# mycrazycracy/speaker-embedding-with-phonetic-information

Measured on AMD Instinct MI355X. Metric: utterance-embeddings/sec (400-frame chunks), higher is better.
Workload: dtype fp16mx; 1 GPU; v2_xvector TDNN, 256 chunks x 400 frames per GPU per step, utterance-sharded, weights broadcast once over RCCL; topology=v2_xvector, batch_chunks_per_gpu=256, frames_per_chunk=400, precision=default, arithmetic=fp16mx, lanes=2, output_node=embedding, chunk_lengths=400, library=xvec_hip 0.4 (gfx950; kernels 1123b5fc04a88fd3)

## Files before the change

### include/xvec_hip.h

```cpp
#ifndef XVEC_HIP_H_
#define XVEC_HIP_H_

#include <stddef.h>
#include <stdint.h>

#ifdef __cplusplus
extern "C" {
#endif

typedef enum {
  XV_OK = 0,
  XV_ERR_IO = 1,
  XV_ERR_MODEL = 2,
  XV_ERR_DEVICE = 3,
  XV_ERR_ARG = 4,
  XV_ERR_INTERNAL = 5
} xv_status;

typedef enum {
  XV_PREC_DEFAULT = -1,
  XV_PREC_BF16X3 = 0,
  XV_PREC_BF16 = 1,
  XV_PREC_FP16 = 2,
  XV_PREC_FP16X3 = 3,
// ... 118 lines not shown
  float sample_frequency, frame_length_ms, frame_shift_ms, dither, preemphasis_coefficient, blackman_coeff;
  int32_t remove_dc_offset, window_type, round_to_power_of_two, snip_edges;
  int32_t num_mel_bins;
  float low_freq, high_freq;
  int32_t num_ceps;
  float cepstral_lifter;
  int32_t use_energy, raw_energy;
  float energy_floor;
} xv_mfcc_options;
typedef struct {
  float vad_energy_threshold, vad_energy_mean_scale, vad_proportion_threshold;
  int32_t vad_frames_context;
} xv_vad_options;
void xv_mfcc_options_default(xv_mfcc_options* opts);
int64_t xv_mfcc_num_frames(const xv_mfcc_options* opts, int64_t n_samples);
uint64_t xv_mfcc_utt_seed(const char* key);
xv_status xv_mfcc_compute(int device, const xv_mfcc_options* opts, const float* samples, const int64_t* sample_offsets,
                          int32_t n_utts, const uint64_t* utt_seeds, float* out, int32_t* out_row_offsets);
xv_status xv_mfcc_compute_i16(int device, const xv_mfcc_options* opts, const int16_t* samples, const int64_t* sample_offsets,
                              int32_t n_utts, const uint64_t* utt_seeds, float* out, int32_t* out_row_offsets);
xv_status xv_mfcc_kernel_time(int device, const xv_mfcc_options* opts, const int16_t* samples, const int64_t* sample_offsets,
                              int32_t n_utts, int32_t reps, float* kernel_ms);
xv_status xv_vad_energy(int device, const xv_vad_options* vad_opts, const float* feats, const int32_t* row_offsets,
                        int32_t n_utts, int32_t dim, float* out);
xv_status xv_wave_read(const char* rxfilename, int32_t channel, int32_t* rate, int16_t** samples, int64_t* n);
void xv_wave_free(int16_t* samples);

typedef struct {
  int32_t shift_output, normalize_output;
  float duration, volume;
  int32_t input_wave_channel, rir_channel, noise_channel;
} xv_reverb_options;
void xv_reverb_options_default(xv_reverb_options* opts);
int64_t xv_reverb_output_length(const xv_reverb_options* opts, float sample_rate, int64_t n_samples, int64_t rir_len);
xv_status xv_wav_reverberate(int device, const xv_reverb_options* opts, float sample_rate, const void* samples,
                             int32_t samples_are_i16, const int64_t* sample_offsets, int32_t n_utts, const float* rirs,
                             const int64_t* rir_offsets, int32_t n_rirs, const int32_t* utt_rir, const float* noises,
                             const int64_t* noise_offsets, int32_t n_noises, const int32_t* utt_add_offsets,
                             const int32_t* add_noise, const float* add_snr, const float* add_start, int64_t* out_offsets,
                             float* out_f32, int16_t* out_i16, int64_t* clipped);
xv_status xv_reverb_kernel_time(int device, const xv_reverb_options* opts, float sample_rate, const void* samples,
                                int32_t samples_are_i16, const int64_t* sample_offsets, int32_t n_utts, const float* rirs,
                                const int64_t* rir_offsets, int32_t n_rirs, const int32_t* utt_rir, const float* noises,
                                const int64_t* noise_offsets, int32_t n_noises, const int32_t* utt_add_offsets,
                                const int32_t* add_noise, const float* add_snr, const float* add_start, int32_t reps,
                                float* kernel_ms);
xv_status xv_recognize_wav_pipeline(const char* rxfilename, int32_t* found, char* description, size_t description_cap);
xv_status xv_wave_write(const char* wxfilename, int32_t rate, const float* samples, int64_t n, int64_t* clipped);

typedef struct {
  const void* hi;
  const void* lo;
  int32_t ld;
  int32_t row_shift;
  int32_t k_len;
  const void* gmax;
  const void* lo4; const void* lo4_scale;
} xv_seg_desc;
typedef struct {
  int32_t precision, epilogue;
  int32_t nseg;
  xv_seg_desc seg[8];
  const void* w_hi; const void* w_lo; int32_t ldw;
  int32_t rows;
  int32_t n_pad;
  const float* bias; const float* scale; const float* offset;
  int32_t relu, bn;
  void* out_hi; void* out_lo; int32_t ldo;
  float* out_f32; int32_t ldf; int32_t m_valid;
  float* partial; int32_t ldp; const int8_t* grp_range;
  void* hip_stream;
  const void* w4; int32_t ldw4; const void* w4_scale;
  void* gmax_out;
  const void* w4b; int32_t ldw4b; const void* w4b_scale;
  void* out_lo4; void* out_lo4_scale;
  int32_t p8;
  const int8_t* out_range;
  int32_t ksplit;
} xv_gemm_desc;
xv_status xv_pack_mx_residual(const float* w, const uint16_t* w_hi_f16, int32_t n_pad, int32_t nseg,
                              const int32_t* seg_src, const int32_t* seg_shift, const int32_t* seg_klen, uint8_t* w4,
                              uint8_t* w4_scale);
xv_status xv_pack_mx_residual64(const float* w, const uint16_t* w_hi_f16, int32_t n_pad, int32_t nseg, const int32_t* seg_src,
                                const int32_t* seg_shift, const int32_t* seg_klen, uint8_t* w4, uint8_t* w4_scale);
xv_status xv_pack_mx_weights(const float* w, int32_t n_pad, int32_t nseg, const int32_t* seg_src, const int32_t* seg_shift,
                             const int32_t* seg_klen, uint8_t* w4b, uint8_t* w4b_scale);
xv_status xv_pack_mx_weights64(const float* w, int32_t n_pad, int32_t nseg, const int32_t* seg_src, const int32_t* seg_shift,
                               const int32_t* seg_klen, uint8_t* w4b, uint8_t* w4b_scale);
xv_status xv_tile_mx_scales(const uint8_t* natural, int32_t n_pad, int32_t k_len, int32_t epilogue, uint8_t* tiled);
xv_status xv_kernel_tdnn_gemm(const xv_gemm_desc* d);

xv_status xv_compressed_size(int32_t rows, int32_t cols, int32_t method, size_t* nbytes, const char** format);
xv_status xv_compress_matrices(int device, const float* feats, const int32_t* row_off, int32_t n, int32_t cols, int32_t method,
                               uint8_t* out_bytes, int64_t* out_off, int32_t* nonfinite_flags);
xv_status xv_compress_kernel_time(int device, const float* feats, const int32_t* row_off, int32_t n, int32_t cols, int32_t method,
                                  int32_t reps, float* kernel_ms);
xv_status xv_cmvn_sliding(int device, const float* raw, const int32_t* raw_off, int32_t n, int32_t cols, int32_t cmn_window,
                          int32_t min_cmn_window, int32_t center, float* out);

xv_status xv_cmvn_stats(int device, const float* feats, const int32_t* row_off, int32_t n_utts, int32_t cols, double* stats,
                        float* device_ms);
xv_status xv_cmvn_norm(const double* stats, int32_t cols, int32_t norm_means, int32_t norm_vars, int32_t reverse,
                       const int32_t* skip_dims, int32_t n_skip, float* norm, int32_t* num_floored);
xv_status xv_cmvn_apply(int device, const float* feats, const int32_t* row_off, int32_t n_utts, int32_t cols, const float* norms,
                        const int32_t* utt_norm, float* out);
xv_status xv_cmvn_kernel_time(int device, const float* feats, const int32_t* row_off, int32_t n_utts, int32_t cols, int32_t reps,
                              float* stats_ms, float* apply_ms);

typedef struct {
  const float* feats;
  const int32_t* row_offsets;
  const int32_t* dev_off;
  int32_t B;
  int32_t rows;
  int32_t pad_left, pad_right;
  int32_t dim, noff;
  int32_t off[8];
  const void* w_hi; const void* w_lo;
  int32_t ldw, seg_pad;
  int32_t n_pad;
  int32_t epi_prec;
  const float* bias; const float* scale; const float* offset;
  int32_t relu, bn;
  void* out_hi; void* out_lo; int32_t ldo;
  void* out_lo4; void* out_lo4_scale;
  void* gmax_out; const int8_t* out_range;
  int32_t row0, nrows;
  int32_t max_wgs;
  void* hip_stream;
} xv_first_layer_desc;
xv_status xv_kernel_first_layer(const xv_first_layer_desc* d);
typedef struct {
  int32_t precision;
  const float* feats; const int32_t* src_off; const int32_t* dev_off; const int32_t* grp_utt;
  int32_t rows;
  int32_t dim, ld;
  void* out_hi; void* out_lo;
  int32_t pad_left, pad_right;
  void* zero_words; int32_t n_zero_words;
  void* hip_stream;
} xv_prep_input_desc;
xv_status xv_kernel_prep_input(const xv_prep_input_desc* d);
typedef struct {
  int32_t precision;
  const float* partial; int32_t ldp;
  const int32_t* utt_grp0; const int32_t* utt_grp1; const int32_t* utt_count;
  int32_t B, dim;
  float var_floor;
  void* out_hi; void* out_lo; int32_t ld;
  void* hip_stream;
} xv_pool_finalise_desc;
xv_status xv_kernel_pool_finalise(const xv_pool_finalise_desc* d);
typedef struct {
  const float* src; const void* src16; int32_t ld;
  const int32_t* out_row; int32_t n_out;
  int32_t dim, log_softmax;
  float* out; int32_t out_ld;
  void* hip_stream;
} xv_frame_output_desc;
xv_status xv_kernel_frame_output(const xv_frame_output_desc* d);

#ifdef __cplusplus
}
#endif
#endif
```

### speaker-embedding-with-phonetic-information_amd/__init__.py

```python
import ctypes
import os
import subprocess
import sys

_HERE = os.path.dirname(os.path.abspath(__file__))
CSRC = os.path.join(_HERE, "csrc")
LIB_PATH = os.environ.get("XVEC_LIB") or os.path.join(_HERE, "libxvec_hip.so")
BIN_DIR = os.path.join(_HERE, "bin")

XV_OK = 0
XV_ERR_IO, XV_ERR_MODEL, XV_ERR_DEVICE, XV_ERR_ARG, XV_ERR_INTERNAL = 1, 2, 3, 4, 5
PREC_BF16X3, PREC_BF16, PREC_FP16, PREC_FP16X3, PREC_FP16X2, PREC_AUTO, PREC_FP16MX, PREC_FP16MX2, PREC_FP16X3E = range(9)
PREC_DEFAULT = -1
PRECISIONS = {"default": PREC_DEFAULT, "bf16x3": PREC_BF16X3, "bf16": PREC_BF16, "fp16": PREC_FP16, "fp16x3": PREC_FP16X3,
              "fp16x2": PREC_FP16X2, "auto": PREC_AUTO, "fp16mx": PREC_FP16MX, "fp16mx2": PREC_FP16MX2}
PRECISION_NAMES = {v: k for k, v in PRECISIONS.items()}
MFMA_PASSES = {"bf16x3": 3, "bf16": 1, "fp16": 1, "fp16x3": 3, "fp16x2": 2, "fp16mx": 1.25}
EPI_ACT, EPI_F32, EPI_STATS = 0, 1, 2


class XvError(RuntimeError):
    def __init__(self, status, msg):
        super().__init__("xvec_hip status %d: %s" % (status, msg))
        self.status = status


class ModelInfo(ctypes.Structure):
    _fields_ = [(n, ctypes.c_int32) for n in ("input_dim", "output_dim", "left_context", "right_context",
                                              "min_frames", "num_layers", "output_is_segment", "reserved")]


class SegDesc(ctypes.Structure):
    _fields_ = [("hi", ctypes.c_void_p), ("lo", ctypes.c_void_p), ("ld", ctypes.c_int32),
                ("row_shift", ctypes.c_int32), ("k_len", ctypes.c_int32), ("gmax", ctypes.c_void_p),
                ("lo4", ctypes.c_void_p), ("lo4_scale", ctypes.c_void_p)]


class GemmDesc(ctypes.Structure):
    _fields_ = [("precision", ctypes.c_int32), ("epilogue", ctypes.c_int32), ("nseg", ctypes.c_int32),
                ("seg", SegDesc * 8),
                ("w_hi", ctypes.c_void_p), ("w_lo", ctypes.c_void_p), ("ldw", ctypes.c_int32),
                ("rows", ctypes.c_int32), ("n_pad", ctypes.c_int32),
                ("bias", ctypes.c_void_p), ("scale", ctypes.c_void_p), ("offset", ctypes.c_void_p),
                ("relu", ctypes.c_int32), ("bn", ctypes.c_int32),
                ("out_hi", ctypes.c_void_p), ("out_lo", ctypes.c_void_p), ("ldo", ctypes.c_int32),
                ("out_f32", ctypes.c_void_p), ("ldf", ctypes.c_int32), ("m_valid", ctypes.c_int32),
                ("partial", ctypes.c_void_p), ("ldp", ctypes.c_int32), ("grp_range", ctypes.c_void_p),
                ("hip_stream", ctypes.c_void_p),
                ("w4", ctypes.c_void_p), ("ldw4", ctypes.c_int32), ("w4_scale", ctypes.c_void_p),
                ("gmax_out", ctypes.c_void_p),
                ("w4b", ctypes.c_void_p), ("ldw4b", ctypes.c_int32), ("w4b_scale", ctypes.c_void_p),
                ("out_lo4", ctypes.c_void_p), ("out_lo4_scale", ctypes.c_void_p),
                ("p8", ctypes.c_int32),
                ("out_range", ctypes.c_void_p), ("ksplit", ctypes.c_int32)]


class FirstLayerDesc(ctypes.Structure):
    _fields_ = [("feats", ctypes.c_void_p), ("row_offsets", ctypes.c_void_p), ("dev_off", ctypes.c_void_p), ("B", ctypes.c_int32),
                ("rows", ctypes.c_int32), ("pad_left", ctypes.c_int32), ("pad_right", ctypes.c_int32),
                ("dim", ctypes.c_int32), ("noff", ctypes.c_int32), ("off", ctypes.c_int32 * 8),
                ("w_hi", ctypes.c_void_p), ("w_lo", ctypes.c_void_p), ("ldw", ctypes.c_int32), ("seg_pad", ctypes.c_int32),
                ("n_pad", ctypes.c_int32), ("epi_prec", ctypes.c_int32),
                ("bias", ctypes.c_void_p), ("scale", ctypes.c_void_p), ("offset", ctypes.c_void_p),
                ("relu", ctypes.c_int32), ("bn", ctypes.c_int32),
                ("out_hi", ctypes.c_void_p), ("out_lo", ctypes.c_void_p), ("ldo", ctypes.c_int32),
                ("out_lo4", ctypes.c_void_p), ("out_lo4_scale", ctypes.c_void_p),
                ("gmax_out", ctypes.c_void_p), ("out_range", ctypes.c_void_p),
                ("row0", ctypes.c_int32), ("nrows", ctypes.c_int32), ("max_wgs", ctypes.c_int32),
                ("hip_stream", ctypes.c_void_p)]


class PrepInputDesc(ctypes.Structure):
    _fields_ = [("precision", ctypes.c_int32), ("feats", ctypes.c_void_p), ("src_off", ctypes.c_void_p), ("dev_off", ctypes.c_void_p),
                ("grp_utt", ctypes.c_void_p), ("rows", ctypes.c_int32), ("dim", ctypes.c_int32), ("ld", ctypes.c_int32),
                ("out_hi", ctypes.c_void_p), ("out_lo", ctypes.c_void_p), ("pad_left", ctypes.c_int32), ("pad_right", ctypes.c_int32),
                ("zero_words", ctypes.c_void_p), ("n_zero_words", ctypes.c_int32), ("hip_stream", ctypes.c_void_p)]


class PoolFinaliseDesc(ctypes.Structure):
    _fields_ = [("precision", ctypes.c_int32), ("partial", ctypes.c_void_p), ("ldp", ctypes.c_int32),
                ("utt_grp0", ctypes.c_void_p), ("utt_grp1", ctypes.c_void_p), ("utt_count", ctypes.c_void_p),
                ("B", ctypes.c_int32), ("dim", ctypes.c_int32), ("var_floor", ctypes.c_float),
                ("out_hi", ctypes.c_void_p), ("out_lo", ctypes.c_void_p), ("ld", ctypes.c_int32), ("hip_stream", ctypes.c_void_p)]


class FrameOutputDesc(ctypes.Structure):
    _fields_ = [("src", ctypes.c_void_p), ("src16", ctypes.c_void_p), ("ld", ctypes.c_int32),
                ("out_row", ctypes.c_void_p), ("n_out", ctypes.c_int32), ("dim", ctypes.c_int32), ("log_softmax", ctypes.c_int32),
                ("out", ctypes.c_void_p), ("out_ld", ctypes.c_int32), ("hip_stream", ctypes.c_void_p)]


class Calibration(ctypes.Structure):
    _fields_ = [("chosen", ctypes.c_int32), ("checked", ctypes.c_int32), ("err_mx", ctypes.c_float), ("err_mx2", ctypes.c_float),
                ("checked_mx", ctypes.c_int32), ("err_lite", ctypes.c_float), ("lite_mask", ctypes.c_uint64),
                ("err_holdout", ctypes.c_float), ("checked_holdout", ctypes.c_int32), ("lite_dropped", ctypes.c_int32),
                ("tail", ctypes.c_float)]

    def as_dict(self):
        d = {"chosen": PRECISION_NAMES.get(self.chosen, str(self.chosen)), "checked": self.checked, "checked_mx": self.checked_mx,
             "err_mx": self.err_mx, "err_mx2": self.err_mx2, "tail": self.tail}
        if self.lite_mask:
            d["lite_mask"] = int(self.lite_mask)
            d["err_lite"] = self.err_lite
            d["err_holdout"] = self.err_holdout
            d["checked_holdout"] = self.checked_holdout
        if self.lite_dropped:
            d["lite_dropped"] = self.lite_dropped
        return d


ABI_SYMBOLS = [
    "xv_last_error", "xv_version", "xv_model_load", "xv_model_load_rxfilename", "xv_model_free", "xv_model_info",
    "xv_model_macs", "xv_model_describe", "xv_model_pack", "xv_ctx_create", "xv_ctx_create_from_blob",
    "xv_ctx_create_from_device_blob", "xv_ctx_free",
    "xv_ctx_info", "xv_forward_batch", "xv_forward_batch_device", "xv_ctx_synchronize", "xv_ctx_set_profiling",
    "xv_ctx_profile_report", "xv_extract_utterances", "xv_ctx_calibrate", "xv_ctx_set_fast_mode", "xv_ctx_fast_mode",
    "xv_calibrate_table", "xv_ctx_set_calibration", "xv_ctx_model_fingerprint", "xv_ctx_share_calibration",
    "xv_ctx_set_calibration_file", "xv_calibration_file_read", "xv_calibration_file_publish", "xv_recognize_feature_pipeline", "xv_ctx_set_lite_layers", "xv_ctx_lite_layers",
    "xv_extract_table", "xv_frontend_cmvn_select", "xv_plan_chunks", "xv_ctx_create_broadcast", "xv_kernel_tdnn_gemm",
    "xv_backend_apply", "xv_segment_mean", "xv_scatter_stats", "xv_plda_transform", "xv_plda_score", "xv_lda_estimate",
    "xv_plda_estimate", "xv_plda_adapt",
    "xv_mfcc_options_default", "xv_mfcc_num_frames", "xv_mfcc_utt_seed", "xv_mfcc_compute", "xv_mfcc_compute_i16", "xv_mfcc_kernel_time", "xv_vad_energy",
    "xv_reverb_options_default", "xv_reverb_output_length", "xv_wav_reverberate", "xv_reverb_kernel_time", "xv_wave_write", "xv_recognize_wav_pipeline",
    "xv_compressed_size", "xv_compress_matrices", "xv_compress_kernel_time", "xv_cmvn_sliding",
    "xv_cmvn_stats", "xv_cmvn_norm", "xv_cmvn_apply", "xv_cmvn_kernel_time",
    "xv_kernel_first_layer", "xv_kernel_prep_input", "xv_kernel_pool_finalise", "xv_kernel_frame_output",
    "xv_wave_read", "xv_wave_free", "xv_pack_mx_residual", "xv_pack_mx_residual64", "xv_tile_mx_scales", "xv_pack_mx_weights", "xv_pack_mx_weights64",
]

_lib = None


def build(verbose=False):
    cmd = ["make", "-C", CSRC, "-j8"]
    res = subprocess.run(cmd, stdout=subprocess.PIPE, stderr=subprocess.STDOUT, text=True)
    if verbose or res.returncode != 0:
        print(res.stdout)
    if res.returncode != 0:
        raise RuntimeError("building libxvec_hip.so failed")
    return LIB_PATH


def lib():
    global _lib
    if _lib is not None:
        return _lib
    if not os.path.exists(LIB_PATH):
        raise ImportError("%s is missing - run `python -c 'import __graft_entry__ as g; g.build()'` "
                          "(there is no Python/CPU fallback for the HIP path)" % LIB_PATH)
    if os.environ.get("XVEC_NO_TORCH_PRELOAD", "") != "1":
        try:
            import torch
        except Exception:
            pass
    L = ctypes.CDLL(LIB_PATH)
    L.xv_last_error.restype = ctypes.c_char_p
    L.xv_version.restype = ctypes.c_char_p
    L.xv_model_macs.restype = ctypes.c_double
    L.xv_model_macs.argtypes = [ctypes.c_void_p, ctypes.c_int32]
    L.xv_model_describe.restype = ctypes.c_size_t
    L.xv_model_describe.argtypes = [ctypes.c_void_p, ctypes.c_char_p, ctypes.c_size_t]
    L.xv_model_load.argtypes = [ctypes.c_void_p, ctypes.c_size_t, ctypes.c_char_p, ctypes.c_char_p,
                                ctypes.POINTER(ctypes.c_void_p)]
    L.xv_model_load_rxfilename.argtypes = [ctypes.c_char_p, ctypes.c_char_p, ctypes.c_char_p,
                                           ctypes.POINTER(ctypes.c_void_p)]
    L.xv_model_free.argtypes = [ctypes.c_void_p]
    L.xv_model_free.restype = None
    L.xv_model_info.argtypes = [ctypes.c_void_p, ctypes.POINTER(ModelInfo)]
    L.xv_model_pack.argtypes = [ctypes.c_void_p, ctypes.c_int, ctypes.c_void_p, ctypes.POINTER(ctypes.c_size_t)]
    L.xv_ctx_create.argtypes = [ctypes.c_void_p, ctypes.c_int, ctypes.c_int, ctypes.POINTER(ctypes.c_void_p)]
    L.xv_ctx_create_from_blob.argtypes = [ctypes.c_void_p, ctypes.c_size_t, ctypes.c_int,
                                          ctypes.POINTER(ctypes.c_void_p)]
    L.xv_ctx_create_from_device_blob.argtypes = [ctypes.c_void_p, ctypes.c_size_t, ctypes.c_int,
                                                 ctypes.POINTER(ctypes.c_void_p)]
    L.xv_pack_mx_residual.argtypes = [ctypes.c_void_p, ctypes.c_void_p, ctypes.c_int32, ctypes.c_int32, ctypes.c_void_p,
                                      ctypes.c_void_p, ctypes.c_void_p, ctypes.c_void_p, ctypes.c_void_p]
    L.xv_pack_mx_residual64.argtypes = L.xv_pack_mx_residual.argtypes
    L.xv_pack_mx_weights.argtypes = [ctypes.c_void_p, ctypes.c_int32, ctypes.c_int32, ctypes.c_void_p, ctypes.c_void_p,
                                     ctypes.c_void_p, ctypes.c_void_p, ctypes.c_void_p]
    L.xv_pack_mx_weights64.argtypes = L.xv_pack_mx_weights.argtypes
    L.xv_tile_mx_scales.argtypes = [ctypes.c_void_p, ctypes.c_int32, ctypes.c_int32, ctypes.c_int32, ctypes.c_void_p]
    L.xv_ctx_free.argtypes = [ctypes.c_void_p]
    L.xv_ctx_free.restype = None
    L.xv_ctx_info.argtypes = [ctypes.c_void_p, ctypes.POINTER(ModelInfo), ctypes.POINTER(ctypes.c_int32),
                              ctypes.POINTER(ctypes.c_int32)]
    L.xv_forward_batch.argtypes = [ctypes.c_void_p, ctypes.c_void_p, ctypes.c_void_p, ctypes.c_int32, ctypes.c_void_p]
    L.xv_forward_batch_device.argtypes = [ctypes.c_void_p, ctypes.c_void_p, ctypes.c_void_p, ctypes.c_int32,
                                          ctypes.c_void_p, ctypes.c_int32, ctypes.c_void_p]
    L.xv_ctx_synchronize.argtypes = [ctypes.c_void_p]
    L.xv_ctx_set_profiling.argtypes = [ctypes.c_void_p, ctypes.c_int32]
    L.xv_ctx_profile_report.argtypes = [ctypes.c_void_p, ctypes.c_char_p, ctypes.c_size_t]
    L.xv_ctx_profile_report.restype = ctypes.c_size_t
    L.xv_extract_utterances.argtypes = [ctypes.c_void_p, ctypes.c_void_p, ctypes.c_void_p, ctypes.c_int32,
                                        ctypes.c_int32, ctypes.c_int32, ctypes.c_int32, ctypes.c_void_p, ctypes.c_void_p]
    L.xv_ctx_create_broadcast.argtypes = [ctypes.c_void_p, ctypes.POINTER(ctypes.c_int), ctypes.c_int, ctypes.c_int,
                                          ctypes.POINTER(ctypes.c_void_p)]
    L.xv_kernel_tdnn_gemm.argtypes = [ctypes.POINTER(GemmDesc)]
    L.xv_kernel_first_layer.argtypes = [ctypes.POINTER(FirstLayerDesc)]
    L.xv_kernel_prep_input.argtypes = [ctypes.POINTER(PrepInputDesc)]
    L.xv_kernel_pool_finalise.argtypes = [ctypes.POINTER(PoolFinaliseDesc)]
    L.xv_kernel_frame_output.argtypes = [ctypes.POINTER(FrameOutputDesc)]
    L.xv_ctx_calibrate.argtypes = [ctypes.c_void_p, ctypes.c_void_p, ctypes.c_void_p, ctypes.c_int32, ctypes.c_float,
                                   ctypes.POINTER(Calibration)]
    L.xv_ctx_set_fast_mode.argtypes = [ctypes.c_void_p, ctypes.c_int32]
    L.xv_ctx_fast_mode.argtypes = [ctypes.c_void_p, ctypes.POINTER(ctypes.c_int32)]
    L.xv_ctx_set_lite_layers.argtypes = [ctypes.c_void_p, ctypes.c_uint64]
    L.xv_ctx_lite_layers.argtypes = [ctypes.c_void_p, ctypes.POINTER(ctypes.c_uint64)]
    L.xv_calibrate_table.argtypes = [ctypes.c_void_p, ctypes.c_char_p, ctypes.c_int32, ctypes.c_int32, ctypes.c_int32,
                                     ctypes.c_int32, ctypes.c_float, ctypes.POINTER(Calibration)]
    L.xv_ctx_set_calibration.argtypes = [ctypes.c_void_p, ctypes.c_int32, ctypes.c_float]
    L.xv_ctx_model_fingerprint.argtypes = [ctypes.c_void_p, ctypes.POINTER(ctypes.c_uint64)]
    L.xv_ctx_share_calibration.argtypes = [ctypes.c_void_p, ctypes.c_char_p, ctypes.c_float, ctypes.c_char_p,
                                           ctypes.POINTER(ctypes.c_int32)]
    L.xv_ctx_set_calibration_file.argtypes = [ctypes.c_void_p, ctypes.c_char_p]
    L.xv_calibration_file_read.argtypes = [ctypes.c_char_p, ctypes.POINTER(ctypes.c_int32), ctypes.POINTER(ctypes.c_uint64),
                                           ctypes.POINTER(ctypes.c_int32), ctypes.POINTER(ctypes.c_uint64)]
    L.xv_calibration_file_publish.argtypes = [ctypes.c_char_p, ctypes.c_uint64, ctypes.c_int32, ctypes.c_uint64, ctypes.c_float,
                                              ctypes.c_char_p, ctypes.POINTER(ctypes.c_int32), ctypes.POINTER(ctypes.c_uint64),
                                              ctypes.POINTER(ctypes.c_int32), ctypes.POINTER(ctypes.c_uint64)]
    _lib = L
    return L


def _check(status):
    if status != XV_OK:
        raise XvError(status, lib().xv_last_error().decode(errors="replace"))


class Model:

    def __init__(self, raw=None, rxfilename=None, nnet_config=None, output_node=None):
        L = lib()
        self._h = ctypes.c_void_p()
        cfg = nnet_config.encode() if nnet_config else None
        node = output_node.encode() if output_node else None
        if raw is not None:
            buf = ctypes.create_string_buffer(bytes(raw), len(raw))
            _check(L.xv_model_load(buf, len(raw), cfg, node, ctypes.byref(self._h)))
        else:
            _check(L.xv_model_load_rxfilename(rxfilename.encode(), cfg, node, ctypes.byref(self._h)))

    def __del__(self):
        if getattr(self, "_h", None) and self._h.value and lib is not None:
            lib().xv_model_free(self._h)
            self._h = ctypes.c_void_p()

    @property
    def info(self):
        mi = ModelInfo()
        _check(lib().xv_model_info(self._h, ctypes.byref(mi)))
        return mi

    def macs(self, frames):
        return lib().xv_model_macs(self._h, int(frames))

    def describe(self):
        n = lib().xv_model_describe(self._h, None, 0)
        buf = ctypes.create_string_buffer(n)
        lib().xv_model_describe(self._h, buf, n)
        return buf.value.decode()

    def pack(self, precision=PREC_DEFAULT):
        n = ctypes.c_size_t(0)
        _check(lib().xv_model_pack(self._h, precision, None, ctypes.byref(n)))
        buf = ctypes.create_string_buffer(n.value)
        _check(lib().xv_model_pack(self._h, precision, buf, ctypes.byref(n)))
        return buf.raw[:n.value]


class Context:

    def __init__(self, model=None, blob=None, device=0, precision=PREC_DEFAULT, device_blob=None):
        L = lib()
        self._h = ctypes.c_void_p()
        if device_blob is not None:
            _check(L.xv_ctx_create_from_device_blob(ctypes.c_void_p(int(device_blob[0])), int(device_blob[1]), device,
                                                    ctypes.byref(self._h)))
        elif blob is not None:
            self._blob = ctypes.create_string_buffer(bytes(blob), len(blob))
            _check(L.xv_ctx_create_from_blob(self._blob, len(blob), device, ctypes.byref(self._h)))
        else:
            _check(L.xv_ctx_create(model._h, device, precision, ctypes.byref(self._h)))
        mi = ModelInfo()
        p, d = ctypes.c_int32(), ctypes.c_int32()
        _check(L.xv_ctx_info(self._h, ctypes.byref(mi), ctypes.byref(p), ctypes.byref(d)))
        self.info, self.precision, self.device = mi, p.value, d.value

    def close(self):
        if getattr(self, "_h", None) and self._h.value and lib is not None:
            lib().xv_ctx_free(self._h)
            self._h = ctypes.c_void_p()

    def __del__(self):
        self.close()

    def forward_batch(self, feats, row_offsets):
        import numpy as np
        feats = np.ascontiguousarray(feats, dtype=np.float32)
        offs = np.ascontiguousarray(row_offsets, dtype=np.int32)
        B = len(offs) - 1
        n_out = B if self.info.output_is_segment else int(offs[-1] - offs[0])
        out = np.empty((n_out, self.info.output_dim), dtype=np.float32)
        _check(lib().xv_forward_batch(self._h, feats.ctypes.data, offs.ctypes.data, B, out.ctypes.data))
        return out

    def forward_batch_device(self, feats_ptr, row_offsets, out_ptr, out_ld, stream=None):
        import numpy as np
        offs = np.ascontiguousarray(row_offsets, dtype=np.int32)
        _check(lib().xv_forward_batch_device(self._h, feats_ptr, offs.ctypes.data, len(offs) - 1, out_ptr, out_ld,
                                             stream))

    def synchronize(self):
        _check(lib().xv_ctx_synchronize(self._h))

    def set_profiling(self, on):
        _check(lib().xv_ctx_set_profiling(self._h, 1 if on else 0))

    def profile_report(self):
        buf = ctypes.create_string_buffer(1 << 18)
        lib().xv_ctx_profile_report(self._h, buf, len(buf))
        rows = []
        for line in buf.value.decode().splitlines():
            label, calls, ms = line.split("\t")
            rows.append((label, int(calls), float(ms)))
        return rows

    def frontend(self, raw, raw_offsets, vad=None, cmn_window=300, center=True):
        import numpy as np
        raw = np.ascontiguousarray(raw, dtype=np.float32)
        offs = np.ascontiguousarray(raw_offsets, dtype=np.int32)
        n = len(offs) - 1
        out = np.empty_like(raw)
        out_off = np.zeros(n + 1, dtype=np.int32)
        v = None if vad is None else np.ascontiguousarray(vad, dtype=np.float32)
        L = lib()
        L.xv_frontend_cmvn_select.argtypes = [ctypes.c_void_p, ctypes.c_void_p, ctypes.c_void_p, ctypes.c_int32, ctypes.c_void_p,
                                              ctypes.c_int32, ctypes.c_int32, ctypes.c_void_p, ctypes.c_void_p]
        _check(L.xv_frontend_cmvn_select(self._h, raw.ctypes.data, offs.ctypes.data, n, None if v is None else v.ctypes.data,
                                         cmn_window, 1 if center else 0, out.ctypes.data, out_off.ctypes.data))
        return out[:out_off[-1]], out_off

    def extract_table(self, feature_rspecifier, vector_wspecifier, chunk_size=-1, min_chunk_size=100, pad_input=True,
                      batch_frames=0):
        L = lib()
        L.xv_extract_table.argtypes = [ctypes.c_void_p, ctypes.c_char_p, ctypes.c_char_p, ctypes.c_int32, ctypes.c_int32,
                                       ctypes.c_int32, ctypes.c_int32, ctypes.POINTER(ctypes.c_int64),
                                       ctypes.POINTER(ctypes.c_int64)]
        done, failed = ctypes.c_int64(0), ctypes.c_int64(0)
        _check(L.xv_extract_table(self._h, feature_rspecifier.encode(), vector_wspecifier.encode(), chunk_size,
                                  min_chunk_size, 1 if pad_input else 0, batch_frames, ctypes.byref(done),
                                  ctypes.byref(failed)))
        return done.value, failed.value

    def calibrate(self, feats, row_offsets, tol=7.5e-5):
# ... 538 lines not shown
              rir_flat.ctypes.data, rir_off.ctypes.data, len(rir_list), utt_rir.ctypes.data,
              noise_flat.ctypes.data, noise_off.ctypes.data, len(noise_list), add_off.ctypes.data if additive is not None else None,
              add_noise.ctypes.data, add_snr.ctypes.data, add_start.ctypes.data)
    if kernel_time_reps > 0:
        L.xv_reverb_kernel_time.argtypes = _REVERB_ARGTYPES + [ctypes.c_int32, ctypes.POINTER(ctypes.c_float)]
        ms = ctypes.c_float(0)
        _check(L.xv_reverb_kernel_time(*common, int(kernel_time_reps), ctypes.byref(ms)))
        return ms.value
    out = np.empty(total, dtype=np.float32)
    out16 = np.empty(total, dtype=np.int16) if return_int16 else None
    clipped = np.zeros(max(1, n), dtype=np.int64)
    out_off = np.zeros(n + 1, dtype=np.int64)
    L.xv_wav_reverberate.argtypes = _REVERB_ARGTYPES + [ctypes.c_void_p, ctypes.c_void_p, ctypes.c_void_p, ctypes.c_void_p]
    _check(L.xv_wav_reverberate(*common, out_off.ctypes.data, out.ctypes.data, out16.ctypes.data if return_int16 else None,
                                clipped.ctypes.data))
    assert list(np.diff(out_off)) == [max(0, x) for x in lens]
    if return_int16:
        return [(out[out_off[u]:out_off[u + 1]].copy(), out16[out_off[u]:out_off[u + 1]].copy(), int(clipped[u])) for u in range(n)]
    return [out[out_off[u]:out_off[u + 1]].copy() for u in range(n)]


def _pack_matrices(mats, what):
    import numpy as np
    ms = [np.ascontiguousarray(m, dtype=np.float32) for m in mats]
    if any(m.ndim != 2 for m in ms):
        raise XvError(XV_ERR_ARG, "%s: every matrix must be two-dimensional" % what)
    widths = {m.shape[1] for m in ms if m.shape[0] > 0}
    if len(widths) > 1:
        raise XvError(XV_ERR_ARG, "%s: the matrices of one call share their column count" % what)
    cols = widths.pop() if widths else 0
    off = np.zeros(len(ms) + 1, dtype=np.int32)
    off[1:] = np.cumsum([m.shape[0] if cols else 0 for m in ms])
    rows = [m for m in ms if m.shape[0] > 0 and cols]
    packed = np.concatenate(rows, axis=0) if rows else np.zeros((0, max(cols, 1)), np.float32)
    return np.ascontiguousarray(packed), off, cols


def compressed_size(rows, cols, method=1):
    L = lib()
    n, fmt = ctypes.c_size_t(0), ctypes.c_char_p()
    L.xv_compressed_size.argtypes = [ctypes.c_int32, ctypes.c_int32, ctypes.c_int32, ctypes.POINTER(ctypes.c_size_t),
                                     ctypes.POINTER(ctypes.c_char_p)]
    _check(L.xv_compressed_size(rows, cols, method, ctypes.byref(n), ctypes.byref(fmt)))
    return int(n.value), fmt.value.decode()


def compress(mats, method=1, device=0, return_flags=False, kernel_time_reps=0):
    import numpy as np
    L = lib()
    packed, off, cols = _pack_matrices(mats, "compress")
    n = len(off) - 1
    common = [device, packed.ctypes.data if packed.size else None, off.ctypes.data, n, cols, method]
    types = [ctypes.c_int, ctypes.c_void_p, ctypes.c_void_p, ctypes.c_int32, ctypes.c_int32, ctypes.c_int32]
    if kernel_time_reps > 0:
        ms = ctypes.c_float(0)
        L.xv_compress_kernel_time.argtypes = types + [ctypes.c_int32, ctypes.POINTER(ctypes.c_float)]
        _check(L.xv_compress_kernel_time(*common, int(kernel_time_reps), ctypes.byref(ms)))
        return ms.value
    total = sum(compressed_size(int(off[u + 1] - off[u]), cols, method)[0] for u in range(n))
    out = np.zeros(max(1, total), dtype=np.uint8)
    out_off = np.zeros(n + 1, dtype=np.int64)
    flags = np.zeros(max(1, n), dtype=np.int32)
    L.xv_compress_matrices.argtypes = types + [ctypes.c_void_p, ctypes.c_void_p, ctypes.c_void_p]
    _check(L.xv_compress_matrices(*common, out.ctypes.data, out_off.ctypes.data, flags.ctypes.data))
    assert int(out_off[n]) == total
    objs = [out[out_off[u]:out_off[u + 1]].tobytes() for u in range(n)]
    return (objs, [bool(f) for f in flags[:n]]) if return_flags else objs


def cmvn_sliding(mats, cmn_window=600, min_cmn_window=100, center=False, device=0):
    import numpy as np
    L = lib()
    packed, off, cols = _pack_matrices(mats, "cmvn_sliding")
    n = len(off) - 1
    out = np.empty_like(packed)
    L.xv_cmvn_sliding.argtypes = [ctypes.c_int, ctypes.c_void_p, ctypes.c_void_p, ctypes.c_int32, ctypes.c_int32, ctypes.c_int32,
                                  ctypes.c_int32, ctypes.c_int32, ctypes.c_void_p]
    _check(L.xv_cmvn_sliding(device, packed.ctypes.data if packed.size else None, off.ctypes.data, n, max(cols, 1), cmn_window,
                             min_cmn_window, 1 if center else 0, out.ctypes.data if out.size else None))
    return [out[off[u]:off[u + 1]].copy() for u in range(n)]


def cmvn_stats(feats_list, device=0, kernel_time_reps=0):
    import numpy as np
    L = lib()
    packed, off, cols = _pack_matrices(feats_list, "cmvn_stats")
    n = len(off) - 1
    if cols < 1:
        raise XvError(XV_ERR_ARG, "cmvn_stats: no matrix with rows and columns")
    if kernel_time_reps > 0:
        a, b = ctypes.c_float(0), ctypes.c_float(0)
        L.xv_cmvn_kernel_time.argtypes = [ctypes.c_int, ctypes.c_void_p, ctypes.c_void_p, ctypes.c_int32, ctypes.c_int32, ctypes.c_int32,
                                          ctypes.POINTER(ctypes.c_float), ctypes.POINTER(ctypes.c_float)]
        _check(L.xv_cmvn_kernel_time(device, packed.ctypes.data, off.ctypes.data, n, cols, int(kernel_time_reps), ctypes.byref(a),
                                     ctypes.byref(b)))
        return a.value, b.value
    stats = np.zeros((n, 2, cols + 1), dtype=np.float64)
    L.xv_cmvn_stats.argtypes = [ctypes.c_int, ctypes.c_void_p, ctypes.c_void_p, ctypes.c_int32, ctypes.c_int32, ctypes.c_void_p,
                                ctypes.c_void_p]
    _check(L.xv_cmvn_stats(device, packed.ctypes.data if packed.size else None, off.ctypes.data, n, cols, stats.ctypes.data, None))
    return stats


def cmvn_norm(stats, norm_means=True, norm_vars=False, reverse=False, skip_dims=(), return_floored=False):
    import numpy as np
    L = lib()
    st = np.ascontiguousarray(stats, dtype=np.float64)
    if st.ndim != 2 or st.shape[0] != 2 or st.shape[1] < 2:
        raise XvError(XV_ERR_ARG, "cmvn_norm: the statistics are a [2][cols + 1] matrix")
    cols = st.shape[1] - 1
    skip = np.ascontiguousarray(list(skip_dims), dtype=np.int32)
    norm = np.zeros((2, cols), dtype=np.float32)
    floored = ctypes.c_int32(0)
    L.xv_cmvn_norm.argtypes = [ctypes.c_void_p, ctypes.c_int32, ctypes.c_int32, ctypes.c_int32, ctypes.c_int32, ctypes.c_void_p,
                               ctypes.c_int32, ctypes.c_void_p, ctypes.POINTER(ctypes.c_int32)]
    _check(L.xv_cmvn_norm(st.ctypes.data, cols, int(bool(norm_means)), int(bool(norm_vars)), int(bool(reverse)),
                          skip.ctypes.data if skip.size else None, int(skip.size), norm.ctypes.data, ctypes.byref(floored)))
    return (norm, int(floored.value)) if return_floored else norm


def apply_cmvn(feats_list, norms, utt_norm, device=0):
    import numpy as np
    L = lib()
    packed, off, cols = _pack_matrices(feats_list, "apply_cmvn")
    n = len(off) - 1
    nm = np.ascontiguousarray(norms, dtype=np.float32)
    un = np.ascontiguousarray(utt_norm, dtype=np.int32)
    if un.shape != (n,) or nm.ndim != 3 or nm.shape[1:] != (2, max(cols, 1)) or (n and (un.min() < 0 or un.max() >= nm.shape[0])):
        raise XvError(XV_ERR_ARG, "apply_cmvn: norms are [n_norms][2][cols] and utt_norm names one of them per matrix")
    out = np.empty_like(packed)
    L.xv_cmvn_apply.argtypes = [ctypes.c_int, ctypes.c_void_p, ctypes.c_void_p, ctypes.c_int32, ctypes.c_int32, ctypes.c_void_p,
                                ctypes.c_void_p, ctypes.c_void_p]
    _check(L.xv_cmvn_apply(device, packed.ctypes.data if packed.size else None, off.ctypes.data, n, max(cols, 1), nm.ctypes.data,
                           un.ctypes.data, out.ctypes.data if out.size else None))
    return [out[off[u]:off[u + 1]].copy() for u in range(n)]


def kernel_tdnn_gemm(desc):
    _check(lib().xv_kernel_tdnn_gemm(ctypes.byref(desc)))


def kernel_first_layer(desc):
    _check(lib().xv_kernel_first_layer(ctypes.byref(desc)))


def kernel_prep_input(desc):
    _check(lib().xv_kernel_prep_input(ctypes.byref(desc)))


def kernel_pool_finalise(desc):
    _check(lib().xv_kernel_pool_finalise(ctypes.byref(desc)))


def kernel_frame_output(desc):
    _check(lib().xv_kernel_frame_output(ctypes.byref(desc)))


def pack_mx_residual(w, w_hi_f16, segs, walk64=False):
    import numpy as np
    w = np.ascontiguousarray(w, dtype=np.float32)
    hi = np.ascontiguousarray(w_hi_f16, dtype=np.uint16)
    n_pad, K = w.shape
    src = np.array([s[0] for s in segs], dtype=np.int32)
    shift = np.array([s[1] for s in segs], dtype=np.int32)
    klen = np.array([s[2] for s in segs], dtype=np.int32)
    assert int(klen.sum()) == K and K % 128 == 0
    w4 = np.zeros((n_pad, K // 128 * 64), dtype=np.uint8)
    sc = np.zeros((n_pad, K // 32), dtype=np.uint8)
    fn = lib().xv_pack_mx_residual64 if walk64 else lib().xv_pack_mx_residual
    _check(fn(w.ctypes.data, hi.ctypes.data, n_pad, len(segs), src.ctypes.data, shift.ctypes.data,
              klen.ctypes.data, w4.ctypes.data, sc.ctypes.data))
    return w4, sc


def pack_mx_weights(w, segs, walk64=False):
    import numpy as np
    w = np.ascontiguousarray(w, dtype=np.float32)
    n_pad, K = w.shape
    src = np.array([s[0] for s in segs], dtype=np.int32)
    shift = np.array([s[1] for s in segs], dtype=np.int32)
    klen = np.array([s[2] for s in segs], dtype=np.int32)
    assert int(klen.sum()) == K and np.all(klen % (256 if walk64 else 128) == 0)
    w4b = np.zeros((n_pad, 2 * K if walk64 else K // 2), dtype=np.uint8)
    sc = np.zeros((n_pad, K // 32), dtype=np.uint8)
    fn = lib().xv_pack_mx_weights64 if walk64 else lib().xv_pack_mx_weights
    _check(fn(w.ctypes.data, n_pad, len(segs), src.ctypes.data, shift.ctypes.data, klen.ctypes.data, w4b.ctypes.data, sc.ctypes.data))
    return w4b, sc


def tile_mx_scales(scales, epilogue):
    import numpy as np
    sc = np.ascontiguousarray(scales, dtype=np.uint8)
    out = np.zeros(sc.size, dtype=np.uint8)
    _check(lib().xv_tile_mx_scales(sc.ctypes.data, sc.shape[0], sc.shape[1] * 32, int(epilogue), out.ctypes.data))
    return out
```

### speaker-embedding-with-phonetic-information_amd/csrc/capi.cc

```cpp
#include <dlfcn.h>
#include <stdlib.h>
#include <string.h>

#include <algorithm>
#include <memory>
#include <string>
#include <vector>

#include "../../include/xvec_hip.h"
#include "backend.h"
#include "cmvn.h"
#include "compress.h"
#include "engine.h"
#include "extractor.h"
#include "feat.h"
#include "reverb.h"
#include "wave.h"
#include "kernels.h"
#include "calib_file.h"
#include "fuse_pipe.h"
#include "fuse_wav.h"
#include "multi_gpu.h"
#include "nnet3_raw.h"
#include "plda.h"
// ... 1066 lines not shown
    if (p) (void)hipFree(p);
  }
  hipError_t Alloc(size_t n) { return hipMalloc(&p, n ? n : 1); }
};
}

xv_status xv_kernel_first_layer(const xv_first_layer_desc* d) {
  if (!d) return Fail(XV_ERR_ARG, "xv_kernel_first_layer: null descriptor");
  return Guard([&] {
    const char* who = "xv_kernel_first_layer: ";
    if (!d->feats || !d->row_offsets || !d->dev_off || !d->w_hi || !d->w_lo || !d->bias || !d->out_hi || (d->bn && (!d->scale || !d->offset)))
      return Fail(XV_ERR_ARG, std::string(who) + "a required pointer is null");
    const int p = d->epi_prec;
    if (p != xv::kPrecBf16x3 && p != xv::kPrecFp16x3 && p != xv::kPrecFp16x2 && p != xv::kPrecFp16x3E)
      return Fail(XV_ERR_ARG, std::string(who) + "epi_prec must be XV_PREC_BF16X3, XV_PREC_FP16X3, XV_PREC_FP16X2 or XV_PREC_FP16X3E");
    if ((p == xv::kPrecBf16x3 || p == xv::kPrecFp16x3) && !d->out_lo) return Fail(XV_ERR_ARG, std::string(who) + "the split planes need out_lo");
    if (p == xv::kPrecFp16x3E && (!d->out_lo4 || !d->out_lo4_scale))
      return Fail(XV_ERR_ARG, std::string(who) + "XV_PREC_FP16X3E needs out_lo4 and out_lo4_scale");
    if (d->B < 1 || d->rows < xv::kFirstRows || d->rows % xv::kFirstRows || d->n_pad < xv::kBN || d->n_pad % xv::kBN ||
        d->ldo < d->n_pad || d->ldo % 64 || d->pad_left < 0 || d->pad_right < 0)
      return Fail(XV_ERR_ARG, std::string(who) + "bad geometry (rows: multiple of 64, n_pad: multiple of 128, ldo: multiple of 64, >= n_pad)");
    if (d->nrows < xv::kFirstRows || d->nrows % xv::kFirstRows || d->row0 < 0 || d->row0 % xv::kFirstRows || d->row0 + (long)d->nrows > d->rows)
      return Fail(XV_ERR_ARG, std::string(who) + "row0 and nrows must be multiples of 64 inside [0, rows]");
    if (d->dim < 1 || d->noff < 1 || d->noff > 8) return Fail(XV_ERR_ARG, std::string(who) + "dim >= 1 and 1 .. 8 offsets");
    int off[8];
    for (int j = 0; j < d->noff; ++j) {
      off[j] = d->off[j];
      if (off[j] < -15 || off[j] > 15) return Fail(XV_ERR_ARG, std::string(who) + "time offsets beyond +-15 frames");
    }
    if (!xv::FirstLayerApplicable(d->dim, d->noff, off))
      return Fail(XV_ERR_ARG, std::string(who) + "tdnn_first_kernel cannot run this shape (dim rounded up to 8 must be <= 24, noff x that <= 128, "
                                                 "and (64 + offset span) x that <= 2048)");
    if (d->seg_pad < d->dim || (long)(d->noff - 1) * d->seg_pad + d->dim > d->ldw)
      return Fail(XV_ERR_ARG, std::string(who) + "the weight planes do not hold noff segments of dim columns");
    const int ngrp = d->rows / xv::kRowAlign;
    std::vector<int32_t> grp_utt(ngrp, -1);
    long next_free = 0;
    if (d->row_offsets[0] < 0) return Fail(XV_ERR_ARG, std::string(who) + "negative row offset");
    for (int b = 0; b < d->B; ++b) {
      const long len = (long)d->row_offsets[b + 1] - d->row_offsets[b];
      const long span = (len + d->pad_left + d->pad_right + xv::kRowAlign - 1) / xv::kRowAlign * xv::kRowAlign;
      if (len < 1 || d->dev_off[b] % xv::kRowAlign || d->dev_off[b] < next_free || d->dev_off[b] + span > d->rows)
        return Fail(XV_ERR_ARG, std::string(who) + "chunk " + std::to_string(b) + ": empty, not on a 16-row boundary, overlapping or beyond rows");
      next_free = d->dev_off[b] + span;
      for (long g = d->dev_off[b] / xv::kRowAlign; g < next_free / xv::kRowAlign; ++g) grp_utt[g] = b;
    }
    std::vector<int32_t> grp_src((size_t)ngrp * 4);
    xv::FillFirstGroupSources(ngrp, grp_utt.data(), d->dev_off, d->row_offsets, d->pad_left, d->pad_right, grp_src.data());
    hipStream_t s = (hipStream_t)d->hip_stream;
    DevMem tab, wch, wcl;
    const size_t wc_bytes = (size_t)d->n_pad * xv::kFirstK * 2;
    hipError_t e = tab.Alloc(grp_src.size() * 4);
    if (e == hipSuccess) e = wch.Alloc(wc_bytes);
    if (e == hipSuccess) e = wcl.Alloc(wc_bytes);
    if (e == hipSuccess) e = hipMemcpy(tab.p, grp_src.data(), grp_src.size() * 4, hipMemcpyHostToDevice);
    if (e != hipSuccess) return Fail(XV_ERR_DEVICE, std::string("first_layer tables: ") + hipGetErrorString(e));
    xv::FirstArgs fa;
    memset(&fa, 0, sizeof fa);
    fa.g.n_tiles = d->n_pad / xv::kBN;
    fa.g.m_tiles = d->rows / xv::kBM;
    fa.g.relu = d->relu;
    fa.g.bn = d->bn;
    fa.g.bias = d->bias;
    fa.g.scale = d->scale;
    fa.g.offset = d->offset;
    fa.g.out_hi = (uint16_t*)d->out_hi;
    fa.g.out_lo = (uint16_t*)d->out_lo;
    fa.g.ldo = d->ldo;
    fa.g.out_lo4 = (uint8_t*)d->out_lo4;
    fa.g.out_lo4s = (uint8_t*)d->out_lo4_scale;
    fa.g.gmax_out = (unsigned*)d->gmax_out;
    fa.g.out_range = d->out_range;
    fa.feats = d->feats;
    fa.feats_valid_idx = (long)d->row_offsets[0] * d->dim;
    fa.grp_src = (const int4*)tab.p;
    fa.rows = d->rows;
    fa.dim = d->dim;
    fa.row0 = d->row0;
    fa.nrows = d->nrows;
    fa.noff = d->noff;
    for (int j = 0; j < d->noff; ++j) fa.off[j] = off[j];
    fa.wc_hi = (const uint16_t*)wch.p;
    fa.wc_lo = (const uint16_t*)wcl.p;
    fa.max_wgs = d->max_wgs > 0 ? d->max_wgs : 0;
    e = xv::launch_compact_first((const uint16_t*)d->w_hi, d->ldw, d->seg_pad, d->n_pad, d->noff, d->dim, (uint16_t*)wch.p, s);
    if (e == hipSuccess) e = xv::launch_compact_first((const uint16_t*)d->w_lo, d->ldw, d->seg_pad, d->n_pad, d->noff, d->dim, (uint16_t*)wcl.p, s);
    if (e == hipSuccess) e = xv::launch_tdnn_first(fa, p, s);
    const hipError_t e2 = hipStreamSynchronize(s);
    if (e != hipSuccess || e2 != hipSuccess)
      return Fail(XV_ERR_DEVICE, std::string("tdnn_first launch: ") + hipGetErrorString(e != hipSuccess ? e : e2));
    return XV_OK;
  });
}

xv_status xv_kernel_prep_input(const xv_prep_input_desc* d) {
  if (!d) return Fail(XV_ERR_ARG, "xv_kernel_prep_input: null descriptor");
  return Guard([&] {
    if (d->precision < xv::kPrecBf16x3 || d->precision > xv::kPrecFp16x3) return Fail(XV_ERR_ARG, "xv_kernel_prep_input: precision must be 0 .. 3");
    const bool split = xv::PrecXPlanes(d->precision) == 2;
    if (!d->feats || !d->src_off || !d->dev_off || !d->grp_utt || !d->out_hi || (split && !d->out_lo))
      return Fail(XV_ERR_ARG, "xv_kernel_prep_input: a required pointer is null");
    if (d->rows < xv::kBM || d->rows % xv::kBM || d->ld < xv::kBK || d->ld % xv::kBK || d->dim < 1 || d->dim > d->ld || d->pad_left < 0 ||
        d->pad_right < 0 || d->n_zero_words < 0 || (d->n_zero_words > 0 && !d->zero_words))
      return Fail(XV_ERR_ARG, "xv_kernel_prep_input: bad geometry (rows: multiple of 128, ld: multiple of 32, >= dim)");
    xv::PrepArgs a;
    memset(&a, 0, sizeof a);
    a.feats = d->feats;
    a.src_off = d->src_off;
    a.dev_off = d->dev_off;
    a.grp_utt = d->grp_utt;
    a.rows = d->rows;
    a.dim = d->dim;
    a.ld = d->ld;
    a.out_hi = (uint16_t*)d->out_hi;
    a.out_lo = (uint16_t*)d->out_lo;
    a.pad_left = d->pad_left;
    a.pad_right = d->pad_right;
    a.zero_words = (unsigned*)d->zero_words;
    a.n_zero_words = d->n_zero_words;
    const hipError_t e = xv::launch_prep_input(a, d->precision, (hipStream_t)d->hip_stream);
    if (e != hipSuccess) return Fail(XV_ERR_DEVICE, std::string("prep_input launch: ") + hipGetErrorString(e));
    return XV_OK;
  });
}

xv_status xv_kernel_pool_finalise(const xv_pool_finalise_desc* d) {
  if (!d) return Fail(XV_ERR_ARG, "xv_kernel_pool_finalise: null descriptor");
  return Guard([&] {
    if (d->precision < xv::kPrecBf16x3 || d->precision > xv::kPrecFp16x3) return Fail(XV_ERR_ARG, "xv_kernel_pool_finalise: precision must be 0 .. 3");
    const bool split = xv::PrecXPlanes(d->precision) == 2;
    if (!d->partial || !d->utt_grp0 || !d->utt_grp1 || !d->utt_count || !d->out_hi || (split && !d->out_lo))
      return Fail(XV_ERR_ARG, "xv_kernel_pool_finalise: a required pointer is null");
    if (d->B < 1 || d->dim < 1 || d->ldp < d->dim || d->ld < 2 * d->dim)
      return Fail(XV_ERR_ARG, "xv_kernel_pool_finalise: bad geometry (ldp >= dim, ld >= 2 dim)");
    xv::PoolArgs a;
    memset(&a, 0, sizeof a);
    a.partial = d->partial;
    a.ldp = d->ldp;
    a.utt_grp0 = d->utt_grp0;
    a.utt_grp1 = d->utt_grp1;
    a.utt_count = d->utt_count;
    a.B = d->B;
    a.dim = d->dim;
    a.var_floor = d->var_floor;
    a.out_hi = (uint16_t*)d->out_hi;
    a.out_lo = (uint16_t*)d->out_lo;
    a.ld = d->ld;
    const hipError_t e = xv::launch_pool_finalise(a, d->precision, (hipStream_t)d->hip_stream);
    if (e != hipSuccess) return Fail(XV_ERR_DEVICE, std::string("pool_finalise launch: ") + hipGetErrorString(e));
    return XV_OK;
  });
}

xv_status xv_kernel_frame_output(const xv_frame_output_desc* d) {
  if (!d) return Fail(XV_ERR_ARG, "xv_kernel_frame_output: null descriptor");
  return Guard([&] {
    if ((!d->src && !d->src16) || !d->out) return Fail(XV_ERR_ARG, "xv_kernel_frame_output: a required pointer is null");
    if (d->n_out < 1 || d->dim < 1 || d->ld < d->dim || d->out_ld < d->dim) return Fail(XV_ERR_ARG, "xv_kernel_frame_output: bad geometry");
    if (d->src16 && (!d->log_softmax || d->dim > 256 * 64))
      return Fail(XV_ERR_ARG, "xv_kernel_frame_output: fp16 logits are read by the log-softmax kernels only, rows of up to 16384 columns");
    xv::FrameOutArgs a;
    memset(&a, 0, sizeof a);
    a.src = d->src;
    a.src16 = (const uint16_t*)d->src16;
    a.ld = d->ld;
    a.out_row = d->out_row;
    a.n_out = d->n_out;
    a.dim = d->dim;
    a.log_softmax = d->log_softmax;
    a.out = d->out;
    a.out_ld = d->out_ld;
    const hipError_t e = xv::launch_frame_output(a, (hipStream_t)d->hip_stream);
    if (e != hipSuccess) return Fail(XV_ERR_DEVICE, std::string("frame_output launch: ") + hipGetErrorString(e));
    return XV_OK;
  });
}

static xv_status PackMxResidualImpl(bool walk64, const float* w, const uint16_t* w_hi_f16, int32_t n_pad, int32_t nseg,
                                    const int32_t* seg_src, const int32_t* seg_shift, const int32_t* seg_klen, uint8_t* w4,
                                    uint8_t* w4_scale) {
  if (!w || !w_hi_f16 || !seg_src || !seg_shift || !seg_klen || !w4 || !w4_scale || nseg < 1 || nseg > xv::kMaxSeg || n_pad < 1)
    return Fail(XV_ERR_ARG, "xv_pack_mx_residual: bad argument");
  return Guard([&] {
    long key[xv::kMaxSeg];
    int shift[xv::kMaxSeg], ksteps[xv::kMaxSeg], k_pad = 0;
    for (int j = 0; j < nseg; ++j) {
      if (seg_klen[j] % xv::kBK) return Fail(XV_ERR_ARG, "xv_pack_mx_residual: k_len must be a multiple of 32");
      key[j] = seg_src[j];
      shift[j] = seg_shift[j];
      ksteps[j] = seg_klen[j] / xv::kBK;
      k_pad += seg_klen[j];
    }
    xv::WalkGroup wg[xv::kMaxSeg];
    const int ng = xv::PlanWalkGroups(nseg, key, shift, ksteps, wg);
    std::vector<int> step_wcol(k_pad / xv::kBK);
    bool ok = false;
    if (walk64) xv::PlanWalkSteps64(ng, wg, step_wcol.data(), (int)step_wcol.size(), &ok);
    else xv::PlanWalkSteps(ng, wg, step_wcol.data(), (int)step_wcol.size(), &ok);
    if (!ok) return Fail(XV_ERR_ARG, "xv_pack_mx_residual: a K group is not a multiple of four steps");
    const int ldw4 = k_pad / xv::kBK / 4 * 64;
    std::vector<float> res(k_pad);
    for (int n = 0; n < n_pad; ++n) {
      for (int k = 0; k < k_pad; ++k) res[k] = w[(size_t)n * k_pad + k] - xv::host_f16_to_f32(w_hi_f16[(size_t)n * k_pad + k]);
      xv::PackMxRow(res.data(), k_pad, step_wcol.data(), w4 + (size_t)n * ldw4, w4_scale + (size_t)n * (k_pad / xv::kBK));
    }
    return XV_OK;
  });
}

xv_status xv_pack_mx_residual(const float* w, const uint16_t* w_hi_f16, int32_t n_pad, int32_t nseg, const int32_t* seg_src,
                              const int32_t* seg_shift, const int32_t* seg_klen, uint8_t* w4, uint8_t* w4_scale) {
  return PackMxResidualImpl(false, w, w_hi_f16, n_pad, nseg, seg_src, seg_shift, seg_klen, w4, w4_scale);
}

xv_status xv_pack_mx_residual64(const float* w, const uint16_t* w_hi_f16, int32_t n_pad, int32_t nseg, const int32_t* seg_src,
                                const int32_t* seg_shift, const int32_t* seg_klen, uint8_t* w4, uint8_t* w4_scale) {
  return PackMxResidualImpl(true, w, w_hi_f16, n_pad, nseg, seg_src, seg_shift, seg_klen, w4, w4_scale);
}

static xv_status PackMxWeightsImpl(bool walk64, const float* w, int32_t n_pad, int32_t nseg, const int32_t* seg_src,
                                   const int32_t* seg_shift, const int32_t* seg_klen, uint8_t* w4b, uint8_t* w4b_scale) {
  if (!w || !seg_src || !seg_shift || !seg_klen || !w4b || !w4b_scale || nseg < 1 || nseg > xv::kMaxSeg || n_pad < 1)
    return Fail(XV_ERR_ARG, "xv_pack_mx_weights: bad argument");
  return Guard([&] {
    long key[xv::kMaxSeg];
    int shift[xv::kMaxSeg], ksteps[xv::kMaxSeg], k_pad = 0;
    for (int j = 0; j < nseg; ++j) {
      if (seg_klen[j] % (walk64 ? 256 : 128)) return Fail(XV_ERR_ARG, "xv_pack_mx_weights: k_len must be a multiple of 128 (256 for the p8 order)");
      key[j] = seg_src[j];
      shift[j] = seg_shift[j];
      ksteps[j] = seg_klen[j] / xv::kBK;
      k_pad += seg_klen[j];
    }
    xv::WalkGroup wg[xv::kMaxSeg];
    const int ng = xv::PlanWalkGroups(nseg, key, shift, ksteps, wg);
    std::vector<int> lo_wcol(k_pad / 128);
    const int n_lo = walk64 ? xv::PlanWalkLoSteps64(ng, wg, lo_wcol.data(), (int)lo_wcol.size())
                            : xv::PlanWalkLoSteps(ng, wg, lo_wcol.data(), (int)lo_wcol.size());
    if (n_lo != (int)lo_wcol.size()) return Fail(XV_ERR_ARG, "xv_pack_mx_weights: inconsistent walk");
    const size_t pitch = walk64 ? (size_t)k_pad * 2 : (size_t)n_lo * 64;
    if (walk64) memset(w4b, 0, pitch * n_pad);
    for (int n = 0; n < n_pad; ++n)
      xv::PackMxWeightsRow(w + (size_t)n * k_pad, lo_wcol.data(), n_lo, w4b + (size_t)n * pitch, w4b_scale + (size_t)n * n_lo * 4);
    return XV_OK;
  });
}

xv_status xv_pack_mx_weights(const float* w, int32_t n_pad, int32_t nseg, const int32_t* seg_src, const int32_t* seg_shift,
                             const int32_t* seg_klen, uint8_t* w4b, uint8_t* w4b_scale) {
  return PackMxWeightsImpl(false, w, n_pad, nseg, seg_src, seg_shift, seg_klen, w4b, w4b_scale);
}

xv_status xv_pack_mx_weights64(const float* w, int32_t n_pad, int32_t nseg, const int32_t* seg_src, const int32_t* seg_shift,
                               const int32_t* seg_klen, uint8_t* w4b, uint8_t* w4b_scale) {
  return PackMxWeightsImpl(true, w, n_pad, nseg, seg_src, seg_shift, seg_klen, w4b, w4b_scale);
}

xv_status xv_tile_mx_scales(const uint8_t* natural, int32_t n_pad, int32_t k_len, int32_t epilogue, uint8_t* tiled) {
  if (!natural || !tiled || n_pad < 1 || n_pad % xv::kBN || k_len < 128 || k_len % 128)
    return Fail(XV_ERR_ARG, "xv_tile_mx_scales: bad argument");
  return Guard([&] {
    xv::TileMxScales(natural, n_pad, k_len / xv::kBK, epilogue != xv::kEpiStats, tiled);
    return XV_OK;
  });
}

}
```

### speaker-embedding-with-phonetic-information_amd/csrc/engine.cc

```cpp
#include "engine.h"
#include "knobs.h"

#include <stddef.h>
#include <time.h>
#include <stdlib.h>
#include <string.h>

#include <algorithm>
#include <atomic>
#include <cmath>
#include <exception>
#include <sstream>
#include <thread>

namespace xv {

namespace {

constexpr int kDefaultFastMinPooledMx2 = 160;
constexpr int kHalo = 32;
constexpr uint32_t kBlobVersion = 8;
constexpr uint64_t kNone = ~0ull;

uint64_t Hash64(const uint8_t* p, size_t n) {
// ... 486 lines not shown
      if (b.w4p != kNone)
        ok = ok && b.w4 != kNone && b.n_pad % 256 == 0 && inside(b.w4p, (uint64_t)b.n_pad * b.ldw4) && b.w4p_scale != kNone &&
             inside(b.w4p_scale, sc_bytes);
      else
        ok = ok && b.w4p_scale == kNone;
      if (b.w4bp != kNone)
        ok = ok && b.w4p != kNone && b.w4b != kNone && inside(b.w4bp, (uint64_t)b.n_pad * b.k_pad * 2) && b.w4bp_scale != kNone &&
             inside(b.w4bp_scale, sc_bytes);
      else
        ok = ok && b.w4bp_scale == kNone;
      if (!ok) throw EngineError("model blob: layer " + std::to_string(i) + " is inconsistent");
    }
    BlobLayerInfo li;
    li.name = b.name;
    li.in_dim = b.in_dim;
    li.out_dim = b.out_dim;
    li.k_pad = b.k_pad;
    li.n_pad = b.n_pad;
    li.relu = b.relu;
    li.bn = b.bn;
    li.log_softmax = b.log_softmax;
    li.segment_level = b.segment_level;
    li.left = b.left;
    li.right = b.right;
    li.has_w4 = b.w4 != kNone;
    li.has_w4b = b.w4b != kNone;
    li.has_w4p = b.w4p != kNone;
    for (int j = 0; j < b.nsrc; ++j) {
      LayerSource s;
      s.layer = b.src_layer[j];
      s.offset = b.src_offset[j];
      s.dim = b.src_dim[j];
      li.src.push_back(s);
    }
    info.layers.push_back(li);
  }
  return info;
}

double BlobInfo::Macs(int T) const {
  const int n = (int)layers.size();
  std::vector<int> nl(n, 1 << 30), nr(n, 1 << 30);
  const int root = output_is_segment ? pooled_layer : output_layer;
  nl[root] = layers[root].left;
  nr[root] = layers[root].right;
  for (int i = n - 1; i >= 0; --i) {
    if (layers[i].segment_level || nl[i] == (1 << 30)) continue;
    for (const LayerSource& s : layers[i].src)
      if (s.layer >= 0) {
        nl[s.layer] = std::min(nl[s.layer], nl[i] + s.offset);
        nr[s.layer] = std::min(nr[s.layer], nr[i] - s.offset);
      }
  }
  double macs = 0;
  for (int i = 0; i < n; ++i) {
    if (layers[i].segment_level) macs += (double)layers[i].in_dim * layers[i].out_dim;
    else if (nl[i] != (1 << 30)) macs += (double)layers[i].in_dim * layers[i].out_dim * std::max(0, T - nl[i] - nr[i]);
  }
  return macs;
}

void Engine::Check(hipError_t e, const char* what) const {
  if (e != hipSuccess) {
    std::ostringstream m;
    m << what << ": " << hipGetErrorString(e) << " (HIP error " << (int)e << ", device " << device_ << ")";
    throw EngineError(m.str());
  }
}

Engine::Engine(const uint8_t* blob, size_t n, int device, const void* device_image) : device_(device) {
  info_ = ParseBlobInfo(blob, n);
  int count = 0;
  hipError_t e = hipGetDeviceCount(&count);
  if (e != hipSuccess || count <= 0)
    throw EngineError("no HIP device available: this library has no CPU path (hipGetDeviceCount: " +
                      std::string(hipGetErrorString(e)) + ")");
  if (device < 0 || device >= count) throw EngineError("HIP device index out of range");
  Check(hipSetDevice(device_), "hipSetDevice");
  hipDeviceProp_t prop;
  Check(hipGetDeviceProperties(&prop, device_), "hipGetDeviceProperties");
  if (strncmp(prop.gcnArchName, "gfx950", 6) != 0)
    throw EngineError(std::string("kernels are built for gfx950 (MI355X) only; device is ") + prop.gcnArchName);
  frame_mode_ = !info_.output_is_segment;
  if (frame_mode_) {
    if (info_.pooled_layer >= 0) throw EngineError("a frame-level output that depends on statistics pooling is not supported");
    pad_left_ = info_.left_context;
    pad_right_ = info_.right_context;
  } else {
    if (info_.pooled_layer < 0) throw EngineError("model has no statistics pooling");
    for (size_t i = 0; i < info_.layers.size(); ++i)
      for (const LayerSource& s : info_.layers[i].src)
        if (s.layer == info_.pooled_layer)
          throw EngineError("the pooled layer must feed only the statistics pooling");
  }
  nplanes_ = PrecWPlanes(info_.precision);
  fast_mode_ = info_.precision;
  if (info_.precision == kPrecAuto || info_.precision == kPrecFp16Mx2) {
    const char* e = getenv("XVEC_FAST_MIN_POOLED");
    fast_min_pooled_ = (e && *e) ? atoi(e) : (info_.precision == kPrecAuto ? kDefaultFastMinPooled : kDefaultFastMinPooledMx2);
    mx2_min_pooled_ = (e && *e) ? atoi(e) : kDefaultFastMinPooledMx2;
    mx_min_pooled_ = (e && *e) ? atoi(e) : kDefaultFastMinPooled;
  }
  Check(hipStreamCreateWithFlags(&stream_, hipStreamNonBlocking), "hipStreamCreate");
  {
    const char* e = getenv("XVEC_LANES");
    int nl = e && *e ? atoi(e) : 2;
    if (nl < 1) nl = 1;
    if (nl > kMaxLanes) nl = kMaxLanes;
    lanes_.resize(nl);
    for (Lane& L : lanes_) {
      Check(hipStreamCreateWithFlags(&L.stream, hipStreamNonBlocking), "hipStreamCreate(lane)");
      Check(hipEventCreateWithFlags(&L.done, hipEventDisableTiming), "hipEventCreate(lane)");
      L.act.resize(info_.layers.size());
    }
  }

  BlobHeader h;
  memcpy(&h, blob, sizeof h);
  blob_data_bytes_ = (size_t)(h.total_bytes - h.data_offset);
  Check(hipMalloc(&d_blob_, blob_data_bytes_), "hipMalloc(weights)");
  if (device_image)
    Check(hipMemcpy(d_blob_, (const uint8_t*)device_image + h.data_offset, blob_data_bytes_, hipMemcpyDeviceToDevice),
          "hipMemcpy(weights, device to device)");
  else
    Check(hipMemcpy(d_blob_, blob + h.data_offset, blob_data_bytes_, hipMemcpyHostToDevice), "hipMemcpy(weights)");
  layers_.resize(info_.layers.size());
  for (size_t i = 0; i < layers_.size(); ++i) {
    BlobLayer b;
    memcpy(&b, blob + sizeof h + i * sizeof(BlobLayer), sizeof b);
    const uint8_t* base = (const uint8_t*)d_blob_;
    layers_[i].w_hi = (const uint16_t*)(base + b.w_hi);
    layers_[i].w_lo = b.w_lo == kNone ? nullptr : (const uint16_t*)(base + b.w_lo);
    layers_[i].bias = (const float*)(base + b.bias);
    layers_[i].scale = (const float*)(base + b.scale);
    layers_[i].offset = (const float*)(base + b.offset);
    layers_[i].w4 = b.w4 == kNone ? nullptr : base + b.w4;
    layers_[i].w4_scale = b.w4_scale == kNone ? nullptr : base + b.w4_scale;
    layers_[i].ldw4 = b.ldw4;
    layers_[i].w4b = b.w4b == kNone ? nullptr : base + b.w4b;
    layers_[i].w4b_scale = b.w4b_scale == kNone ? nullptr : base + b.w4b_scale;
    layers_[i].ldw4b = b.ldw4b;
    layers_[i].w4p = b.w4p == kNone ? nullptr : base + b.w4p;
    layers_[i].w4p_scale = b.w4p_scale == kNone ? nullptr : base + b.w4p_scale;
    layers_[i].w4bp = b.w4bp == kNone ? nullptr : base + b.w4bp;
    layers_[i].w4bp_scale = b.w4bp_scale == kNone ? nullptr : base + b.w4bp_scale;
  }
  Check(hipStreamSynchronize(nullptr), "hipStreamSynchronize(weights)");
  {
    use_p8_ = DebugKnobInt("p8", 1) != 0;
    p8_whole_ = DebugKnobInt("p8_whole", 0);
  }
  in_ld_ = RoundUp(info_.input_dim, kBK);
  stats_ld_ = RoundUp(2 * info_.pool_dim, kBK);
  {
    const bool allow = DebugKnobInt("first_kernel", 1) != 0 && nplanes_ == 2;
    need_prep_ = false;
    for (size_t i = 0; i < layers_.size(); ++i) {
      const BlobLayerInfo& li = info_.layers[i];
      bool reads_input = false, only_input = !li.segment_level && !li.src.empty();
      int off[kMaxSeg] = {0};
      for (size_t j = 0; j < li.src.size(); ++j) {
        if (li.src[j].layer == kSrcInput) reads_input = true;
        if (li.src[j].layer != kSrcInput || li.src[j].dim != info_.input_dim) only_input = false;
        off[j] = li.src[j].offset;
      }
      const bool planes_out = (int)i != info_.pooled_layer && !(frame_mode_ && (int)i == info_.output_layer);
      if (allow && only_input && planes_out && layers_[i].w_lo && FirstLayerApplicable(info_.input_dim, (int)li.src.size(), off)) {
        first_buf_.emplace_back();
        first_buf_.emplace_back();
        Buf& bh = first_buf_[first_buf_.size() - 2];
        Buf& bl = first_buf_[first_buf_.size() - 1];
        Ensure(&bh, (size_t)li.n_pad * kFirstK * 2, false);
        Ensure(&bl, (size_t)li.n_pad * kFirstK * 2, false);
        const int seg_pad = SrcKPad(info_.input_dim, kSrcInput, false, info_.precision);
        Check(launch_compact_first(layers_[i].w_hi, li.k_pad, seg_pad, li.n_pad, (int)li.src.size(), info_.input_dim, (uint16_t*)bh.p, stream_),
              "compact_first launch");
        Check(launch_compact_first(layers_[i].w_lo, li.k_pad, seg_pad, li.n_pad, (int)li.src.size(), info_.input_dim, (uint16_t*)bl.p, stream_),
              "compact_first launch");
        layers_[i].first = true;
        layers_[i].wc_hi = (const uint16_t*)bh.p;
        layers_[i].wc_lo = (const uint16_t*)bl.p;
      } else if (reads_input) {
        need_prep_ = true;
      }
    }
    Check(hipStreamSynchronize(stream_), "hipStreamSynchronize(compact_first)");
  }
}

Engine::~Engine() {
  (void)hipSetDevice(device_);
  if (stream_) (void)hipStreamSynchronize(stream_);
  plan_cache_.clear();
  auto fr = [](Buf& b) {
    if (b.p) (void)hipFree(b.p);
    b.p = nullptr;
  };
  if (stream_) release_stream_workspace(stream_);
  for (Lane& L : lanes_) {
    if (L.stream) (void)hipStreamSynchronize(L.stream);
    if (L.stream) release_stream_workspace(L.stream);
    fr(L.gmax);
    for (ActBuf& a : L.act) {
      fr(a.act_hi);
      fr(a.act_lo);
      fr(a.act_lo4);
      fr(a.act_lo4s);
    }
    fr(L.in_hi);
    fr(L.in_lo);
    fr(L.partial);
    fr(L.stats_hi);
    fr(L.stats_lo);
    fr(L.out_f32);
    fr(L.splitk_ws);
    fr(L.frame_f32);
    if (L.done) (void)hipEventDestroy(L.done);
    if (L.stream) (void)hipStreamDestroy(L.stream);
  }
  for (HostSlot& S : host_slots_) {
    if (S.done) {
      (void)hipEventSynchronize(S.done);
      (void)hipEventDestroy(S.done);
    }
    if (S.h2d_done) (void)hipEventDestroy(S.h2d_done);
    S.plan.reset();
    fr(S.d_feats);
    fr(S.d_out);
    fr(S.d_tables);
    fr(S.d_raw);
    fr(S.d_prefix);
    fr(S.d_fetab);
    fr(S.d_cm);
    if (S.h_fetab) (void)hipHostFree(S.h_fetab);
    if (S.h_feats) (void)hipHostFree(S.h_feats);
    if (S.h_out) (void)hipHostFree(S.h_out);
    if (S.h_tables) (void)hipHostFree(S.h_tables);
  }
  for (Buf& b : first_buf_) fr(b);
  fr(feats_stage_);
  fr(fe_raw_);
  fr(fe_tab_);
  fr(fe_prefix_);
  fr(fe_out_);
  fr(out_stage_);
  if (d_blob_) (void)hipFree(d_blob_);
  if (copy_stream_) (void)hipStreamDestroy(copy_stream_);
  if (stream_) (void)hipStreamDestroy(stream_);
}

void Engine::Ensure(Buf* b, size_t bytes, bool zero, hipStream_t consumer) {
  if (b->bytes >= bytes && b->p) return;
  if (b->p) Check(hipFree(b->p), "hipFree");
  b->p = nullptr;
  Check(hipMalloc(&b->p, bytes), "hipMalloc");
  b->bytes = bytes;
  if (zero) {
    Check(hipMemsetAsync(b->p, 0, bytes, consumer), "hipMemsetAsync");
  }
}

void Engine::EnsureCapacity(Lane& L, int rows, int b_pad, hipStream_t s) {
  bool grew = false;
  if (rows > L.cap_rows) {
    grew = true;
    if (L.busy) Check(hipEventSynchronize(L.done), "hipEventSynchronize(lane)");
    const size_t r = (size_t)rows + 2 * kHalo;
    Ensure(&L.in_hi, r * in_ld_ * 2, true, s);
    if (nplanes_ == 2) Ensure(&L.in_lo, r * in_ld_ * 2, true, s);
    for (size_t i = 0; i < layers_.size(); ++i) {
      const BlobLayerInfo& li = info_.layers[i];
      if (li.segment_level) continue;
      if ((int)i == info_.pooled_layer) {
        Ensure(&L.partial, (size_t)(rows / kRowAlign) * 2 * li.n_pad * 4, true, s);
        continue;
      }
      if (frame_mode_ && (int)i == info_.output_layer) {
        Ensure(&L.frame_f32, (size_t)rows * li.n_pad * (logits16() ? 2 : 4), false);
        continue;
      }
      Ensure(&L.act[i].act_hi, r * li.n_pad * 2, true, s);
      if (nplanes_ == 2) Ensure(&L.act[i].act_lo, r * li.n_pad * 2, true, s);
      if (info_.precision == kPrecFp16Mx2 && !frame_mode_) {
        Ensure(&L.act[i].act_lo4, r * (li.n_pad / 2), true, s);
        Ensure(&L.act[i].act_lo4s, r * Lo4ScalePitch(li.n_pad), true, s);
      }
    }
    if (fast_mx() || can_switch_fast_mode()) Ensure(&L.gmax, layers_.size() * (size_t)(rows / kRowAlign) * 4, true, s);
    L.gmax_stride = rows / kRowAlign;
    L.cap_rows = rows;
  }
  if (!frame_mode_ && b_pad > L.cap_b) {
    if (L.busy) Check(hipEventSynchronize(L.done), "hipEventSynchronize(lane)");
    Ensure(&L.stats_hi, (size_t)b_pad * stats_ld_ * 2, true, s);
    if (nplanes_ == 2) Ensure(&L.stats_lo, (size_t)b_pad * stats_ld_ * 2, true, s);
    for (size_t i = 0; i < layers_.size(); ++i) {
      const BlobLayerInfo& li = info_.layers[i];
      if (!li.segment_level) continue;
      if ((int)i == info_.output_layer) {
        Ensure(&L.out_f32, (size_t)b_pad * li.n_pad * 4, true, s);
      } else {
        Ensure(&L.act[i].act_hi, (size_t)b_pad * li.n_pad * 2, true, s);
        if (nplanes_ == 2) Ensure(&L.act[i].act_lo, (size_t)b_pad * li.n_pad * 2, true, s);
      }
    }
    L.cap_b = b_pad;
    grew = true;
  }
  if (grew) Check(hipStreamSynchronize(s), "hipStreamSynchronize(fills)");
}

uint16_t* Engine::ActBase(const Buf& b, int ld) const {
  return b.p ? (uint16_t*)b.p + (size_t)kHalo * ld : nullptr;
}

Engine::Plan::~Plan() {
  if (d_tables && !borrowed_tables) (void)hipFree(d_tables);
}

void Engine::FillPlan(const int32_t* row_offsets, int B, Plan* plan, std::vector<uint8_t>* tables) const {
  if (B <= 0) throw EngineError("empty batch");
  std::vector<int32_t> key(B);
  for (int b = 0; b < B; ++b) {
    key[b] = row_offsets[b + 1] - row_offsets[b];
    if (frame_mode_ ? key[b] < 1 : key[b] < info_.min_frames) {
      std::ostringstream m;
      m << "chunk " << b << " has " << key[b] << " frames; the network needs at least " << info_.min_frames;
      throw EngineError(m.str());
    }
  }
  plan->B = B;
  plan->b_pad = RoundUp(B, kBM);
  plan->src_off.assign(row_offsets, row_offsets + B + 1);
  plan->src_rows = row_offsets[B];
  const BlobLayerInfo& pl = info_.layers[frame_mode_ ? 0 : info_.pooled_layer];
  const int pool_first = std::max(pl.left, -info_.pool_left);
  std::vector<int32_t> dev_off(B), cnt(B, 0);
  std::vector<char> fast(B, 0);
  for (int b = 0; b < B && !frame_mode_; ++b) {
    const int last = std::min(key[b] - 1 - pl.right, info_.pool_right);
    if (last < pool_first) throw EngineError("chunk has no frame inside the pooling window");
    cnt[b] = last - pool_first + 1;
    fast[b] = has_fast() && cnt[b] >= fast_min_pooled_;
  }
  long off = 0;
  for (int pass = 0; pass < 2; ++pass) {
    for (int b = 0; b < B; ++b) {
      if ((pass == 0) != (fast[b] != 0)) continue;
      dev_off[b] = (int32_t)off;
      off += RoundUp(key[b] + pad_left_ + pad_right_, kRowAlign);
      if (off > (1l << 30)) throw EngineError("batch too large (more than 2^30 device rows)");
    }
    off = RoundUp((int)off, (pass == 0 && has_fast()) ? 4 * kBM : 2 * kBM);
    if (pass == 0) plan->rows_fast = (int)off;
  }
  plan->rows = (int)off;
  const int ngrp = plan->rows / kRowAlign;
  std::vector<int32_t> grp_utt(ngrp, -1), g0(B), g1(B);
  std::vector<int8_t> grp_range((size_t)ngrp * 2, 0);
  std::vector<int32_t> out_row;
  if (frame_mode_) {
    plan->out_off.assign(1, 0);
    for (int b = 0; b < B; ++b) {
      const int Td = key[b] + pad_left_ + pad_right_;
      const int ga = dev_off[b] / kRowAlign, gb = (dev_off[b] + RoundUp(Td, kRowAlign)) / kRowAlign;
      for (int g = ga; g < gb; ++g) grp_utt[g] = b;
      for (int i = 0; i < key[b]; ++i) out_row.push_back(dev_off[b] + pad_left_ + i);
      plan->out_off.push_back((int32_t)out_row.size());
    }
    plan->n_out = (int)out_row.size();
  }
  for (int b = 0; b < B && !frame_mode_; ++b) {
    const int T = key[b];
    const int first = pool_first;
    const int last = first + cnt[b] - 1;
    g0[b] = dev_off[b] / kRowAlign;
    g1[b] = (dev_off[b] + RoundUp(T, kRowAlign)) / kRowAlign;
    for (int g = g0[b]; g < g1[b]; ++g) {
      grp_utt[g] = b;
      const int t0 = (g - g0[b]) * kRowAlign;
      grp_range[2 * g] = (int8_t)std::min(std::max(first - t0, 0), kRowAlign);
      grp_range[2 * g + 1] = (int8_t)std::min(std::max(last + 1 - t0, 0), kRowAlign);
    }
  }
  const int nlay = (int)info_.layers.size();
  std::vector<int8_t> act_range;
  if (fast_mx() && !frame_mode_) {
    act_range.assign((size_t)nlay * ngrp * 2, 0);
    for (int i = 0; i < nlay; ++i) {
      const BlobLayerInfo& li = info_.layers[i];
      if (li.segment_level) continue;
      int8_t* t = act_range.data() + (size_t)i * ngrp * 2;
      for (int b = 0; b < B; ++b) {
        const int lo = li.left, hi = key[b] - li.right;
        for (int g = g0[b]; g < g1[b]; ++g) {
          const int t0 = (g - g0[b]) * kRowAlign;
          t[2 * g] = (int8_t)std::min(std::max(lo - t0, 0), kRowAlign);
          t[2 * g + 1] = (int8_t)std::min(std::max(hi - t0, 0), kRowAlign);
        }
      }
    }
  }
  plan->ngrp = ngrp;
  plan->o_src = 0;
  plan->o_dev = Align256(plan->o_src + (size_t)(B + 1) * 4);
  plan->o_gu = Align256(plan->o_dev + (size_t)B * 4);
  plan->o_gr = Align256(plan->o_gu + (size_t)ngrp * 4);
  plan->o_g0 = Align256(plan->o_gr + (size_t)ngrp * 2);
  plan->o_g1 = Align256(plan->o_g0 + (size_t)B * 4);
  plan->o_cn = Align256(plan->o_g1 + (size_t)B * 4);
  plan->o_or = Align256(plan->o_cn + (size_t)B * 4);
  plan->o_ar = Align256(plan->o_or + out_row.size() * 4);
  plan->o_gs = Align256(plan->o_ar + act_range.size());
  std::vector<int32_t> grp_src((size_t)ngrp * 4, 0);
  FillFirstGroupSources(ngrp, grp_utt.data(), dev_off.data(), row_offsets, pad_left_, pad_right_, grp_src.data());
  const size_t total = Align256(plan->o_gs + grp_src.size() * 4);
  std::vector<uint8_t>& host = *tables;
  host.assign(total, 0);
  if (!act_range.empty()) memcpy(host.data() + plan->o_ar, act_range.data(), act_range.size());
  memcpy(host.data() + plan->o_gs, grp_src.data(), grp_src.size() * 4);
  if (!out_row.empty()) memcpy(host.data() + plan->o_or, out_row.data(), out_row.size() * 4);
  memcpy(host.data() + plan->o_src, plan->src_off.data(), (size_t)(B + 1) * 4);
  memcpy(host.data() + plan->o_dev, dev_off.data(), (size_t)B * 4);
  memcpy(host.data() + plan->o_gu, grp_utt.data(), (size_t)ngrp * 4);
  memcpy(host.data() + plan->o_gr, grp_range.data(), (size_t)ngrp * 2);
  memcpy(host.data() + plan->o_g0, g0.data(), (size_t)B * 4);
  memcpy(host.data() + plan->o_g1, g1.data(), (size_t)B * 4);
  memcpy(host.data() + plan->o_cn, cnt.data(), (size_t)B * 4);
}

void Engine::BindPlan(Plan* plan, const void* device_tables) {
  const uint8_t* d = (const uint8_t*)device_tables;
  plan->d_src_off = (const int32_t*)(d + plan->o_src);
  plan->d_dev_off = (const int32_t*)(d + plan->o_dev);
  plan->d_grp_utt = (const int32_t*)(d + plan->o_gu);
  plan->d_grp_range = (const int8_t*)(d + plan->o_gr);
  plan->d_utt_grp0 = (const int32_t*)(d + plan->o_g0);
  plan->d_utt_grp1 = (const int32_t*)(d + plan->o_g1);
  plan->d_utt_count = (const int32_t*)(d + plan->o_cn);
  plan->d_out_row = (const int32_t*)(d + plan->o_or);
  plan->d_act_range = (const int8_t*)(d + plan->o_ar);
  plan->d_grp_src = d + plan->o_gs;
}

std::shared_ptr<Engine::Plan> Engine::MakePlan(const int32_t* row_offsets, int B) {
  if (B <= 0) throw EngineError("empty batch");
  std::vector<int32_t> key(B + 1);
// ... 102 lines not shown
      ga.ldo = li.n_pad;
      if (fast_mx2()) {
        ga.out_lo4 = (uint8_t*)L.act[i].act_lo4.p + (size_t)kHalo * (li.n_pad / 2);
        ga.out_lo4s = (uint8_t*)L.act[i].act_lo4s.p + (size_t)kHalo * Lo4ScalePitch(li.n_pad);
      }
      if (mx_pass) {
        ga.gmax_out = gmax_of((int)i);
        ga.out_range = plan.d_act_range + (size_t)i * plan.ngrp * 2;
      }
    }
  } else {
    ga.m_tiles = plan.b_pad / kBM;
    const int per = SplitKStepsPerSlice(ksteps);
    ga.ksteps_per_slice = per;
    ga.ksplit = (ksteps + per - 1) / per;
    if (ga.ksplit > 1) {
      Ensure(&L.splitk_ws, (size_t)ga.ksplit * plan.b_pad * li.n_pad * 4, false);
      ga.splitk_ws = (float*)L.splitk_ws.p;
    }
    if ((int)i == info_.output_layer) {
      epi = kEpiF32;
      ga.out_f32 = direct_out ? out_dev : (float*)L.out_f32.p;
      ga.ldf = direct_out ? out_ld : li.n_pad;
      ga.m_valid = plan.B;
    } else {
      epi = kEpiAct;
      ga.out_hi = (uint16_t*)L.act[i].act_hi.p;
      ga.out_lo = (uint16_t*)L.act[i].act_lo.p;
      ga.ldo = li.n_pad;
    }
  }
  if (ga.w4_scale && epi == kEpiStats) ga.w4_scale += (size_t)li.n_pad * (li.k_pad / kBK);
  if (ga.w4b_scale && epi == kEpiStats) ga.w4b_scale += (size_t)li.n_pad * (li.k_pad / kBK);
  return epi;
}

FirstArgs Engine::FirstLayerArgs(const Plan& plan, size_t i, const GemmArgs& ga, const float* feats_dev, int r0, int r1) const {
  const BlobLayerInfo& li = info_.layers[i];
  FirstArgs fa;
  memset(&fa, 0, sizeof fa);
  fa.g = ga;
  fa.feats = feats_dev;
  fa.feats_valid_idx = (long)plan.src_off[0] * info_.input_dim;
  fa.grp_src = (const int4*)plan.d_grp_src;
  fa.rows = plan.rows;
  fa.dim = info_.input_dim;
  fa.noff = (int)li.src.size();
  for (int j = 0; j < fa.noff; ++j) fa.off[j] = li.src[j].offset;
  fa.wc_hi = layers_[i].wc_hi;
  fa.wc_lo = layers_[i].wc_lo;
  fa.row0 = r0;
  fa.nrows = r1 - r0;
  return fa;
}

static GemmArgs SliceRows(GemmArgs g, long r0, long r1) {
  g.m_tiles = (int)((r1 - r0) / kBM);
  g.m_valid = (int)(r1 - r0);
  for (int j = 0; j < g.nseg; ++j) {
    Seg& sg = g.seg[j];
    sg.hi += r0 * sg.ld;
    if (sg.lo) sg.lo += r0 * sg.ld;
    if (sg.lo4) sg.lo4 += r0 * (sg.ld / 2);
    if (sg.lo4s) sg.lo4s += r0 * Lo4ScalePitch(sg.ld);
  }
  if (g.out_hi) g.out_hi += r0 * g.ldo;
  if (g.out_lo) g.out_lo += r0 * g.ldo;
  if (g.out_lo4) g.out_lo4 += r0 * (g.ldo / 2);
  if (g.out_lo4s) g.out_lo4s += r0 * Lo4ScalePitch(g.ldo);
  if (g.out_f32) g.out_f32 += r0 * g.ldf;
  if (g.partial) g.partial += (r0 / kRowAlign) * 2 * g.ldp;
  if (g.grp_range) g.grp_range += (r0 / kRowAlign) * 2;
  return g;
}

int Engine::LaunchPrec(size_t i, int epi, bool fast, GemmArgs* g) const {
  const BlobLayerInfo& li = info_.layers[i];
  const DevLayer& dl = layers_[i];
  int p = slow_prec();
  if (!fast) {
    g->gmax_out = nullptr;
    g->out_range = nullptr;
    for (int j = 0; j < g->nseg; ++j) g->seg[j].gmax = nullptr;
    if (dl.first || p != kPrecFp16 || li.segment_level) return p;
  } else if (dl.first) {
    return (fast_mx2() && (!lite_mask_ || lite_emits_[i])) ? (int)kPrecFp16x3E : (int)kPrecFp16x2;
  } else if (fast_mx2() && lite_mask_ && lite_[i] && gemm_mx_applicable(*g)) {
    p = (lite_emits_[i] && epi == kEpiAct) ? (int)kPrecFp16MxE : (int)kPrecFp16Mx;
    if (p == kPrecFp16Mx) {
      g->out_lo4 = nullptr;
      g->out_lo4s = nullptr;
    }
  } else if (fast_mx2()) {
    p = gemm_mx2_applicable(*g) ? (int)kPrecFp16Mx2 : (int)kPrecFp16x3E;
    if (p == kPrecFp16x3E && epi != kEpiAct) throw EngineError("fp16mx2: layer " + li.name + " cannot run the mode");
    if (p == kPrecFp16x3E) return p;
  } else {
    p = (fast_mx() && gemm_mx_applicable(*g)) ? (int)kPrecFp16Mx : (int)kPrecFp16x2;
    if (p == kPrecFp16x2) return p;
  }
  const bool mx = p != kPrecFp16, mx2 = p == kPrecFp16Mx2;
  if (!use_p8_ || (epi != kEpiAct && epi != kEpiStats) || (mx && !dl.w4p) || (mx2 && !dl.w4bp)) return p;
  const size_t so = epi == kEpiStats ? (size_t)li.n_pad * (li.k_pad / kBK) : 0;
  GemmArgs g8 = *g;
  g8.p8 = 1;
  g8.p8_whole = p8_whole_;
  if (mx) {
    g8.w4 = dl.w4p;
    g8.w4_scale = dl.w4p_scale + so;
  }
  if (mx2) {
    g8.w4b = dl.w4bp;
    g8.ldw4b = li.k_pad * 2;
    g8.w4b_scale = dl.w4bp_scale + so;
  }
  if (gemm_p8_applicable(g8, p)) *g = g8;
  return p;
}

PrepArgs Engine::PrepInputArgs(const Lane& L, const Plan& plan, const float* feats_dev, bool mx_pass) const {
  PrepArgs pa;
  pa.feats = feats_dev;
  pa.src_off = plan.d_src_off;
  pa.dev_off = plan.d_dev_off;
  pa.grp_utt = plan.d_grp_utt;
  pa.rows = plan.rows;
  pa.dim = info_.input_dim;
  pa.ld = in_ld_;
  pa.out_hi = ActBase(L.in_hi, in_ld_);
  pa.out_lo = ActBase(L.in_lo, in_ld_);
  pa.pad_left = pad_left_;
  pa.pad_right = pad_right_;
  pa.zero_words = mx_pass ? (unsigned*)L.gmax.p : nullptr;
  pa.n_zero_words = mx_pass ? (int)(layers_.size() * (size_t)L.gmax_stride) : 0;
  return pa;
}

PoolArgs Engine::PoolingArgs(const Lane& L, const Plan& plan) const {
  PoolArgs po;
  po.partial = (const float*)L.partial.p;
  po.ldp = info_.layers[info_.pooled_layer].n_pad;
  po.utt_grp0 = plan.d_utt_grp0;
  po.utt_grp1 = plan.d_utt_grp1;
  po.utt_count = plan.d_utt_count;
  po.B = plan.B;
  po.dim = info_.pool_dim;
  po.var_floor = info_.variance_floor;
  po.out_hi = (uint16_t*)L.stats_hi.p;
  po.out_lo = (uint16_t*)L.stats_lo.p;
  po.ld = stats_ld_;
  return po;
}

FrameOutArgs Engine::OutputArgs(const Lane& L, const Plan& plan, float* out_dev, int out_ld) const {
  const BlobLayerInfo& ol = info_.layers[info_.output_layer];
  FrameOutArgs fo;
  fo.src = logits16() ? nullptr : (const float*)(frame_mode_ ? L.frame_f32.p : L.out_f32.p);
  fo.src16 = logits16() ? (const uint16_t*)L.frame_f32.p : nullptr;
  fo.ld = ol.n_pad;
  fo.out_row = frame_mode_ ? plan.d_out_row : nullptr;
  fo.n_out = frame_mode_ ? plan.n_out : plan.B;
  fo.dim = info_.output_dim;
  fo.log_softmax = ol.log_softmax;
  fo.out = out_dev;
  fo.out_ld = out_ld;
  return fo;
}

void Engine::ForwardOnLane(size_t lane, const Plan& plan, const float* feats_dev, float* out_dev, int out_ld,
                           hipStream_t stream) {
  Check(hipSetDevice(device_), "hipSetDevice");
  Lane& L = lanes_[lane % lanes_.size()];
  hipStream_t s = stream ? stream : L.stream;
  if (stream && stream != stream_ && std::find(ext_streams_.begin(), ext_streams_.end(), stream) == ext_streams_.end()) {
    bool own = false;
    for (const Lane& l : lanes_) own = own || l.stream == stream;
    if (!own) ext_streams_.push_back(stream);
  }
  if (L.busy) Check(hipStreamWaitEvent(s, L.done, 0), "hipStreamWaitEvent(lane)");
  EnsureCapacity(L, plan.rows, plan.b_pad, s);
  const bool mx_pass = fast_mx() && plan.rows_fast > 0;
  std::vector<hipEvent_t> prof_run;
  const bool first_prof = prof_on_ && prof_labels_.empty();
  auto arm = [&](const std::string& label) {
    if (!prof_on_) return;
    hipEvent_t e0, e1;
    Check(hipEventCreate(&e0), "hipEventCreate");
    Check(hipEventCreate(&e1), "hipEventCreate");
    prof_run.push_back(e0);
    prof_run.push_back(e1);
    if (first_prof) prof_labels_.push_back(label);
    set_launch_events(e0, e1);
  };
  auto disarm = [&]() {
    if (prof_on_) set_launch_events(nullptr, nullptr);
  };
  const PrepArgs pa = PrepInputArgs(L, plan, feats_dev, mx_pass);
  if (need_prep_) {
    arm("prep_input");
    Check(launch_prep_input(pa, slow_prec(), s), "prep_input launch");
    disarm();
  } else if (pa.n_zero_words > 0) {
    Check(hipMemsetAsync(pa.zero_words, 0, (size_t)pa.n_zero_words * 4, s), "hipMemsetAsync(group maxima)");
  }

  const BlobLayerInfo& ol = info_.layers[info_.output_layer];
  const bool direct_out = ol.segment_level && !ol.log_softmax && ol.n_pad == info_.output_dim && (out_ld & 3) == 0 &&
                          out_ld >= ol.n_pad && ((uintptr_t)out_dev & 15) == 0;
  for (size_t i = 0; i < layers_.size(); ++i) {
    const BlobLayerInfo& li = info_.layers[i];
    GemmArgs ga;
    const int epi = LayerArgs(L, plan, i, mx_pass, out_dev, out_ld, direct_out, &ga);
    arm(std::string("tdnn_gemm<") + (epi == kEpiAct ? "act" : epi == kEpiF32 ? "f32" : "stats") + ">:" + li.name);
    if (!layers_[i].first && (li.segment_level || plan.rows_fast == 0)) {
      const int p = LaunchPrec(i, epi, false, &ga);
      Check(launch_tdnn_gemm(ga, p, epi, s), "tdnn_gemm launch");
      if (first_prof) prof_labels_.back() += std::string(" ") + last_gemm_kernel();
    } else {
      for (int region = 0; region < 2; ++region) {
        const int r0 = region == 0 ? 0 : plan.rows_fast, r1 = region == 0 ? plan.rows_fast : plan.rows;
        if (r1 <= r0) continue;
        if (layers_[i].first) {
          FirstArgs fa = FirstLayerArgs(plan, i, ga, feats_dev, r0, r1);
          const int p = LaunchPrec(i, epi, region == 0, &fa.g);
          Check(launch_tdnn_first(fa, p, s), "tdnn_first launch");
        } else {
          GemmArgs gr = SliceRows(ga, r0, r1);
          const int p = LaunchPrec(i, epi, region == 0, &gr);
          Check(launch_tdnn_gemm(gr, p, epi, s), "tdnn_gemm launch");
        }
        if (first_prof) prof_labels_.back() += std::string(" ") + last_gemm_kernel();
      }
    }
    disarm();

    if ((int)i == info_.pooled_layer) {
      arm("pool_finalise");
      Check(launch_pool_finalise(PoolingArgs(L, plan), slow_prec(), s), "pool_finalise launch");
      disarm();
    }
  }
  if (frame_mode_ || ol.log_softmax) {
    arm("frame_output");
    Check(launch_frame_output(OutputArgs(L, plan, out_dev, out_ld), s), "frame_output launch");
    disarm();
  } else if (!direct_out) {
    Check(hipMemcpy2DAsync(out_dev, (size_t)out_ld * 4, L.out_f32.p, (size_t)ol.n_pad * 4, (size_t)info_.output_dim * 4,
                           (size_t)plan.B, hipMemcpyDeviceToDevice, s),
          "hipMemcpy2DAsync(out)");
  }
  Check(hipEventRecord(L.done, s), "hipEventRecord(lane)");
  L.busy = true;
  if (prof_on_) prof_runs_.push_back(std::move(prof_run));
}

void Engine::SetFastMode(int mode) {
  if (!can_switch_fast_mode()) throw EngineError("this context cannot switch its arithmetic (it was not packed as fp16mx2 with a pooled output)");
  if (mode != kPrecFp16Mx2 && mode != kPrecFp16Mx && mode != kPrecFp16x3) throw EngineError("SetFastMode: fp16mx2, fp16mx or fp16x3");
  if (mode == fast_mode_ && lite_mask_ == 0) return;
  Check(hipSetDevice(device_), "hipSetDevice");
  Check(hipDeviceSynchronize(), "hipDeviceSynchronize");
  for (const HostSlot& S : host_slots_)
    if (S.pending) throw EngineError("SetFastMode with a batch in flight");
  fast_mode_ = mode;
  fast_min_pooled_ = mode == kPrecFp16Mx2 ? mx2_min_pooled_ : mx_min_pooled_;
  lite_mask_ = 0;
  lite_.assign(layers_.size(), 0);
  lite_emits_.assign(layers_.size(), 0);
  plan_cache_.clear();
}

void Engine::SetLiteMask(uint64_t mask) {
  if (!can_switch_fast_mode() || fast_mode_ != kPrecFp16Mx2) throw EngineError("SetLiteMask: the context must be running fp16mx2");
  Check(hipSetDevice(device_), "hipSetDevice");
  Check(hipDeviceSynchronize(), "hipDeviceSynchronize");
  for (const HostSlot& S : host_slots_)
    if (S.pending) throw EngineError("SetLiteMask with a batch in flight");
  const size_t nl = layers_.size();
  lite_.assign(nl, 0);
  lite_emits_.assign(nl, 0);
  uint64_t kept = 0;
  for (size_t i = 0; i < nl && i < (size_t)kMaxLiteLayers; ++i) {
    const BlobLayerInfo& li = info_.layers[i];
    bool ok = ((mask >> i) & 1) && !li.segment_level && li.has_w4 && !layers_[i].first;
    for (const LayerSource& src : li.src) ok = ok && src.layer >= 0 && !info_.layers[src.layer].segment_level;
    if (ok) {
      lite_[i] = 1;
      kept |= 1ull << i;
    }
  }
  for (size_t c = 0; c < nl; ++c) {
    if (info_.layers[c].segment_level || lite_[c]) continue;
    for (const LayerSource& src : info_.layers[c].src)
      if (src.layer >= 0) lite_emits_[src.layer] = 1;
  }
  lite_mask_ = kept;
  fast_min_pooled_ = kept ? std::max(mx2_min_pooled_, mx_min_pooled_) : mx2_min_pooled_;
  plan_cache_.clear();
}

Engine::Calibration Engine::Calibrate(const float* feats, const int32_t* row_offsets, int B, float tol) {
  Calibration c;
  c.chosen = fast_mode();
  if (!can_switch_fast_mode() || B <= 0) return c;
  {
    static std::atomic<int> calls{0};
    const int inject = DebugKnobInt("calib_fail", 0);
    if ((inject == 1 && calls.fetch_add(1) == 0) || inject == 2) throw EngineError("injected failure (XVEC_DEBUG=calib_fail)");
  }
  static std::atomic<int> perturb_calls{0};
  const bool perturb = DebugKnobInt("calib_fail", 0) == 3 && perturb_calls.fetch_add(1) == 0;
  const BlobLayerInfo& pl = info_.layers[info_.pooled_layer];
  const int pool_first = std::max(pl.left, -info_.pool_left);
  std::vector<int32_t> offs(1, row_offsets[0]);
  std::vector<int> pick;
  std::vector<char> runs_mx;
  for (int b = 0; b < B; ++b) {
    const int T = row_offsets[b + 1] - row_offsets[b];
    const int cnt = std::min(T - 1 - pl.right, info_.pool_right) - pool_first + 1;
    if (T >= info_.min_frames && cnt >= std::min(mx_min_pooled_, mx2_min_pooled_)) {
      pick.push_back(b);
      runs_mx.push_back(cnt >= mx_min_pooled_);
    }
  }
  if (pick.empty()) return c;
  const int D = info_.input_dim, E = info_.output_dim;
  std::vector<float> f;
  offs.assign(1, 0);
  for (int b : pick) {
    f.insert(f.end(), feats + (size_t)row_offsets[b] * D, feats + (size_t)row_offsets[b + 1] * D);
    offs.push_back(offs.back() + (row_offsets[b + 1] - row_offsets[b]));
  }
  const int n = (int)pick.size();
  const int before = fast_mode_;
  const uint64_t lite_before = lite_mask_;
  std::vector<float> ref((size_t)n * E), mx((size_t)n * E), mx2((size_t)n * E);
  try {
    SetFastMode(kPrecFp16x3);
    ForwardHost(f.data(), offs.data(), n, ref.data());
    SetFastMode(kPrecFp16Mx);
    ForwardHost(f.data(), offs.data(), n, mx.data());
    SetFastMode(kPrecFp16Mx2);
    ForwardHost(f.data(), offs.data(), n, mx2.data());
    if (perturb) mx2[0] = std::nextafterf(mx2[0], INFINITY);
    std::vector<float> again((size_t)n * E);
    for (int pass = 0; pass < 2; ++pass) {
      const std::vector<float>& first = pass == 0 ? mx2 : ref;
      if (pass == 1) SetFastMode(kPrecFp16x3);
      ForwardHost(f.data(), offs.data(), n, again.data());
      if (memcmp(again.data(), first.data(), again.size() * sizeof(float)) != 0) {
        int bad = 0;
        double worst = 0.0;
        for (int i = 0; i < n; ++i) {
          bool differs = false;
          for (int k = 0; k < E; ++k) {
            const float a = again[(size_t)i * E + k], b = first[(size_t)i * E + k];
            if (memcmp(&a, &b, 4) != 0) {
              differs = true;
              const double r = std::fabs((double)a - b) / std::max(1e-30, (double)std::fabs(b));
              if (!(r <= worst)) worst = r;
            }
          }
          bad += differs ? 1 : 0;
        }
        std::ostringstream m;
        m << "calibration: two runs of the " << PrecisionName(pass == 0 ? (int)kPrecFp16Mx2 : (int)kPrecFp16x3) << " arithmetic on the same "
          << n << " chunks differ in " << bad << " of them (largest relative difference of an element " << worst
          << "): the device does not reproduce its own results";
        throw EngineError(m.str());
      }
    }
  } catch (...) {
    SetFastMode(before);
    if (before == kPrecFp16Mx2 && lite_before) SetLiteMask(lite_before);
    throw;
  }
  struct ErrStat {
    float worst = 0.f, tail = 0.f;
    int n = 0;
  };
  auto stat = [&](const std::vector<float>& got, bool only_mx, int half) {
    ErrStat st;
    double sum = 0.0, sum2 = 0.0;
    for (int i = 0; i < n; ++i) {
      if (only_mx && !runs_mx[i]) continue;
      if (half >= 0 && (i & 1) != half) continue;
      float d = 0.f, m = 0.f;
      for (int k = 0; k < E; ++k) {
        d = std::max(d, std::fabs(got[(size_t)i * E + k] - ref[(size_t)i * E + k]));
// ... 362 lines not shown
```

### speaker-embedding-with-phonetic-information_amd/csrc/engine.h

```cpp
#pragma once
#include <hip/hip_runtime_api.h>
#include <stdint.h>

#include <map>
#include <memory>
#include <stdexcept>
#include <string>
#include <vector>

#include "kernels.h"
#include "program.h"

namespace xv {

struct EngineError : public std::runtime_error {
  explicit EngineError(const std::string& m) : std::runtime_error(m) {}
};

std::vector<uint8_t> PackModel(const TdnnProgram& prog, int precision);
constexpr int kPrecDefault = -1;
std::vector<uint8_t> PackModelPolicy(const TdnnProgram& prog, int precision, int* resolved = nullptr);
const char* PrecisionName(int precision);

void PackMxRow(const float* res, int k_pad, const int* step_wcol, uint8_t* row, uint8_t* scales);
void PackMxWeightsRow(const float* w, const int* lo_wcol, int n_lo, uint8_t* row, uint8_t* scales);
void TileMxScales(const uint8_t* natural, int n_pad, int nsteps, bool weights_are_operand_a, uint8_t* tiled);

struct BlobLayerInfo {
  std::string name;
  int in_dim, out_dim, k_pad, n_pad, relu, bn, log_softmax, segment_level, left, right;
  bool has_w4 = false;
  bool has_w4b = false;
  bool has_w4p = false;
  std::vector<LayerSource> src;
};

struct BlobInfo {
  int precision, input_dim, pooled_layer, pool_dim, pool_left, pool_right, output_layer, output_dim,
      output_is_segment, left_context, right_context, min_frames;
  float variance_floor;
  uint64_t fingerprint = 0;
  std::vector<BlobLayerInfo> layers;
  double Macs(int T) const;
};
BlobInfo ParseBlobInfo(const uint8_t* blob, size_t n);
std::vector<uint8_t> ReadBlobHead(const void* device_blob, size_t n);

class Engine {
 public:
  struct Plan;
  Engine(const uint8_t* blob, size_t n, int device, const void* device_image = nullptr);
  ~Engine();
  Engine(const Engine&) = delete;
  Engine& operator=(const Engine&) = delete;

  const BlobInfo& info() const { return info_; }
  int device() const { return device_; }

  std::shared_ptr<Plan> MakePlan(const int32_t* row_offsets, int B);
  void Forward(const Plan& plan, const float* feats_dev, float* out_dev, int out_ld, hipStream_t stream);
  void ForwardHost(const float* feats, const int32_t* row_offsets, int B, float* out);
  static constexpr int kNumHostSlots = 3;
  float* HostFeats(int slot, size_t rows);
  struct FrontEndJob {
    const int32_t* raw_off;
    int n_utts;
    const int32_t* sel_row;
    const int32_t* sel_utt;
    int n_out;
    int cmn_window;
    bool center;
    int min_window;
    const int64_t* cm_off = nullptr;
    size_t cm_bytes = 0;
    int max_rows = 0;
  };
  void SubmitHost(int slot, long seq, const int32_t* row_offsets, int B, const FrontEndJob* fe = nullptr);
  const float* WaitHost(int slot);
  bool frame_mode() const { return frame_mode_; }
  void FrontEndHost(const float* raw, const int32_t* raw_off, int n_utts, const int32_t* sel_row, const int32_t* sel_utt,
                    int n_out, int cmn_window, bool center, int min_window, float* out);

  struct Calibration {
    int chosen = 0;
    int checked = 0;
    float err_mx = 0.f;
    float err_mx2 = 0.f;
    int checked_mx = 0;
    uint64_t lite_mask = 0;
    float err_lite = 0.f;
    int checked_holdout = 0;
    float err_holdout = 0.f;
    int lite_dropped = 0;
    float tail = 0.f;
    float tail_mx = 0.f;
  };
  static constexpr int kCalibMinChunks = 16;
  static constexpr double kTailSigmas = 6.0;
  static constexpr float kTailOverTol = 1.10f;
  static constexpr float kTailOverTolPacked = 1.20f;
  static constexpr int kMaxLanes = 4;
  static constexpr int kMaxLiteLayers = 64;
  bool can_switch_fast_mode() const { return info_.precision == kPrecFp16Mx2 && !frame_mode_; }
  int fast_mode() const { return can_switch_fast_mode() ? fast_mode_ : info_.precision; }
  void SetFastMode(int mode);
  void SetLiteMask(uint64_t mask);
  uint64_t lite_mask() const { return lite_mask_; }
  Calibration Calibrate(const float* feats, const int32_t* row_offsets, int B, float tol);

  hipStream_t stream() const { return stream_; }
  int num_lanes() const { return (int)lanes_.size(); }
  size_t weight_bytes() const { return blob_data_bytes_; }
  void SetProfiling(bool on) { prof_on_ = on; }
  std::string ProfileReport();

 private:
  struct Buf {
    void* p = nullptr;
    size_t bytes = 0;
  };
  struct DevLayer {
    const uint16_t* w_hi;
    const uint16_t* w_lo;
    const float* bias;
    const float* scale;
    const float* offset;
    const uint8_t* w4;
    const uint8_t* w4_scale;
    int ldw4;
    const uint8_t* w4b;
    const uint8_t* w4b_scale;
    int ldw4b;
    const uint8_t* w4p = nullptr;
    const uint8_t* w4p_scale = nullptr;
    const uint8_t* w4bp = nullptr;
    const uint8_t* w4bp_scale = nullptr;
    bool first = false;
    const uint16_t* wc_hi = nullptr;
    const uint16_t* wc_lo = nullptr;
  };
  struct ActBuf {
    Buf act_hi, act_lo;
    Buf act_lo4, act_lo4s;
  };
  struct Lane {
    hipStream_t stream = nullptr;
    hipEvent_t done = nullptr;
    bool busy = false;
    std::vector<ActBuf> act;
    Buf in_hi, in_lo, partial, stats_hi, stats_lo, out_f32, splitk_ws, frame_f32;
    Buf gmax;
    int gmax_stride = 0;
    int cap_rows = 0, cap_b = 0;
  };
  struct HostSlot {
    void* h_feats = nullptr;
    size_t h_feats_bytes = 0;
    void* h_out = nullptr;
    size_t h_out_bytes = 0;
    void* h_tables = nullptr;
    size_t h_tables_bytes = 0;
    Buf d_feats, d_out, d_tables;
    Buf d_raw, d_prefix, d_fetab;
    Buf d_cm;
    void* h_fetab = nullptr;
    size_t h_fetab_bytes = 0;
    hipEvent_t done = nullptr;
    hipEvent_t h2d_done = nullptr;
    bool pending = false;
    int lane = 0;
    std::unique_ptr<Plan> plan;
  };
  HostSlot host_slots_[kNumHostSlots];
  void EnsurePinned(void** p, size_t* have, size_t bytes);
  void FillPlan(const int32_t* row_offsets, int B, Plan* plan, std::vector<uint8_t>* tables) const;
  static void BindPlan(Plan* plan, const void* device_tables);
  void ForwardOnLane(size_t lane, const Plan& plan, const float* feats_dev, float* out_dev, int out_ld, hipStream_t stream);
  int LayerArgs(Lane& L, const Plan& plan, size_t i, bool mx_pass, float* out_dev, int out_ld, bool direct_out, GemmArgs* args);
  FirstArgs FirstLayerArgs(const Plan& plan, size_t i, const GemmArgs& ga, const float* feats_dev, int r0, int r1) const;
  int LaunchPrec(size_t i, int epi, bool fast, GemmArgs* g) const;
  PrepArgs PrepInputArgs(const Lane& L, const Plan& plan, const float* feats_dev, bool mx_pass) const;
  PoolArgs PoolingArgs(const Lane& L, const Plan& plan) const;
  FrameOutArgs OutputArgs(const Lane& L, const Plan& plan, float* out_dev, int out_ld) const;
  void Check(hipError_t e, const char* what) const;
 public:
  void CheckKernelFaults(int lane = -1) const;
  mutable unsigned fault_mask_ = 0;
  std::vector<hipStream_t> ext_streams_;
 private:
  void Ensure(Buf* b, size_t bytes, bool zero, hipStream_t consumer = nullptr);
  void EnsureCapacity(Lane& L, int rows, int b_pad, hipStream_t s);
  uint16_t* ActBase(const Buf& b, int ld) const;

  BlobInfo info_;
  int device_ = 0;
  bool frame_mode_ = false;
  int pad_left_ = 0, pad_right_ = 0;
  int nplanes_ = 1;
  static constexpr int kDefaultFastMinPooled = 300;
  static bool fast_family(int p) { return p == kPrecFp16x2 || p == kPrecAuto || p == kPrecFp16Mx || p == kPrecFp16Mx2; }
  int slow_prec() const { return fast_family(info_.precision) ? (int)kPrecFp16x3 : info_.precision; }
  bool has_fast() const { return !frame_mode_ && fast_family(fast_mode_); }
  bool fast_mx() const { return has_fast() && fast_mode_ != kPrecFp16x2; }
  bool fast_mx2() const { return has_fast() && fast_mode_ == kPrecFp16Mx2; }
  int p8_whole_ = 0;
  bool use_p8_ = true;
  bool logits16() const { return frame_mode_ && info_.precision == kPrecFp16 && info_.layers[info_.output_layer].log_softmax; }
  int fast_min_pooled_ = 0;
  int fast_mode_ = 0;
  uint64_t lite_mask_ = 0;
  std::vector<char> lite_, lite_emits_;
  int mx2_min_pooled_ = 0, mx_min_pooled_ = 0;
  hipStream_t stream_ = nullptr;
  hipStream_t copy_stream_ = nullptr;
  void* d_blob_ = nullptr;
  size_t blob_data_bytes_ = 0;
  std::vector<DevLayer> layers_;
  std::vector<Buf> first_buf_;
  bool need_prep_ = true;
  int in_ld_ = 0;
  int stats_ld_ = 0;
  std::vector<Lane> lanes_;
  size_t next_lane_ = 0;
  Buf feats_stage_, out_stage_;
  Buf fe_raw_, fe_tab_, fe_prefix_, fe_out_;
  std::map<std::vector<int32_t>, std::shared_ptr<Plan>> plan_cache_;
  bool prof_on_ = false;
  std::vector<std::string> prof_labels_;
  std::vector<std::vector<hipEvent_t>> prof_runs_;
};

struct Engine::Plan {
  int B = 0, b_pad = 0, rows = 0, src_rows = 0;
  int rows_fast = 0;
  std::vector<int32_t> src_off;
  void* d_tables = nullptr;
  bool borrowed_tables = false;
  size_t o_src = 0, o_dev = 0, o_gu = 0, o_gr = 0, o_g0 = 0, o_g1 = 0, o_cn = 0, o_or = 0, o_ar = 0, o_gs = 0;
  int ngrp = 0;
  const int8_t* d_act_range = nullptr;
  const int32_t* d_src_off = nullptr;
  const int32_t* d_dev_off = nullptr;
  const int32_t* d_grp_utt = nullptr;
  const void* d_grp_src = nullptr;
  const int8_t* d_grp_range = nullptr;
  const int32_t* d_utt_grp0 = nullptr;
  const int32_t* d_utt_grp1 = nullptr;
  const int32_t* d_utt_count = nullptr;
  const int32_t* d_out_row = nullptr;
  std::vector<int32_t> out_off;
  int n_out = 0;
  ~Plan();
};

struct FrontEndBuffers {
  void* raw;
  void* prefix;
  void* out;
  void* tab;
};
struct FrontEndBytes {
  size_t raw, prefix, out, tab;
};
FrontEndBytes FrontEndSizes(long raw_rows, int n_utts, int n_out, int dim);
void FrontEndRun(hipStream_t s, const FrontEndBuffers& b, int dim, const float* raw, const int32_t* raw_off, int n_utts,
                 const int32_t* sel_row, const int32_t* sel_utt, int n_out, int cmn_window, bool center, int min_window, float* out);

}
```

### speaker-embedding-with-phonetic-information_amd/csrc/kernels.h

```cpp
#pragma once
#include <hip/hip_runtime.h>
#include <stdint.h>

namespace xv {

constexpr int kBM = 128;
constexpr int kBN = 128;
constexpr int kBK = 32;
constexpr int kMaxSeg = 8;
constexpr int kRowAlign = 16;

enum Precision : int {
  kPrecBf16x3 = 0,
  kPrecBf16 = 1,
  kPrecFp16 = 2,
  kPrecFp16x3 = 3,
  kPrecFp16x2 = 4,
  kPrecAuto = 5,
  kPrecFp16Mx = 6,
  kPrecFp16Mx2 = 7,
  kPrecFp16x3E = 8,
  kPrecFp16MxE = 9,
};
constexpr bool PrecF16(int p) { return p == kPrecFp16 || p == kPrecFp16x3 || p == kPrecFp16x2 || p == kPrecAuto || p == kPrecFp16Mx || p == kPrecFp16Mx2 || p == kPrecFp16x3E || p == kPrecFp16MxE; }
// ... 117 lines not shown
    for (int kq = 0; kq < g[i].ksteps / 4; ++kq)
      for (int ij = 0; ij < g[i].nshift; ++ij) {
        if (n < cap) lo_wcol[n] = g[i].wcol0 + ij * g[i].wstride + kq * 4 * kBK;
        ++n;
      }
  return n;
}

struct GemmArgs {
  Seg seg[kMaxSeg];
  int nseg;
  Grp grp[2 * kMaxSeg];
  int ngrp;
  int total_ksteps;
  int ngrp_lo;
  int lo_ksteps;
  const uint16_t* w_hi;
  const uint16_t* w_lo;
  int ldw;
  const uint8_t* w4;
  int ldw4;
  const uint8_t* w4_scale;
  const uint8_t* w4b;
  int ldw4b;
  const uint8_t* w4b_scale;
  int m_tiles;
  int n_tiles;
  int relu;
  int bn;
  const float* bias;
  const float* scale;
  const float* offset;
  uint16_t* out_hi;
  uint16_t* out_lo;
  int ldo;
  uint8_t* out_lo4;
  uint8_t* out_lo4s;
  unsigned* gmax_out;
  const int8_t* out_range;
  float* out_f32;
  int ldf;
  int m_valid;
  float* partial;
  int ldp;
  const int8_t* grp_range;
  int ksplit;
  int ksteps_per_slice;
  float* splitk_ws;
  int stagger_wgs, stagger_units;
  int sk_mtiles;
  int sk_lanes;
  float* sk_ws;
  unsigned* sk_flags;
  unsigned sk_epoch;
  unsigned* sk_error;
  int p8;
  int p8_ktiles;
  int p8_whole;
  int p8_ktiles_lo;
};

inline int SplitKStepsPerSlice(int ksteps) {
  const int per = (ksteps + 23) / 24;
  return per < 4 ? 4 : per;
}

void set_launch_events(hipEvent_t start, hipEvent_t stop);

hipError_t launch_tdnn_gemm(const GemmArgs& a, int precision, int epilogue, hipStream_t s);
const char* last_gemm_kernel();
bool gemm_mx_applicable(const GemmArgs& a);
bool gemm_mx2_applicable(const GemmArgs& a);
constexpr bool kP8Mx2Built = true;
bool gemm_p8_applicable(const GemmArgs& a, int precision);
void release_stream_workspace(hipStream_t s);
unsigned sk_take_error(hipStream_t s);

constexpr int kFirstK = 128;
constexpr int kFirstRows = 64;
constexpr int kFirstMaxSlots = 4;
inline bool FirstLayerApplicable(int dim, int noff, const int* off) {
  if (noff < 1 || noff > 8 || dim < 1) return false;
  const int dp = (dim + 7) / 8 * 8;
  int lo = off[0], hi = off[0];
  for (int j = 1; j < noff; ++j) {
    lo = off[j] < lo ? off[j] : lo;
    hi = off[j] > hi ? off[j] : hi;
  }
  return dp <= 24 && noff * dp <= kFirstK && hi - lo <= 30 && (kFirstRows + hi - lo) * dp <= 512 * kFirstMaxSlots;
}
struct FirstArgs {
  GemmArgs g;
  const float* feats;
  long feats_valid_idx;
  const int4* grp_src;
  int rows;
  int dim;
  int row0, nrows;
  int noff;
  int off[8];
  const uint16_t* wc_hi;
  const uint16_t* wc_lo;
  int max_wgs;
};
inline void FillFirstGroupSources(int ngrp, const int32_t* grp_utt, const int32_t* dev_off, const int32_t* row_offsets, int pad_left,
                                  int pad_right, int32_t* grp_src) {
  for (int g = 0; g < ngrp; ++g) {
    int32_t* e = grp_src + 4 * (size_t)g;
    e[0] = e[1] = e[2] = e[3] = 0;
    const int b = grp_utt[g];
    if (b < 0) continue;
    const int t0 = g * kRowAlign - dev_off[b];
    const int s0 = row_offsets[b], len = row_offsets[b + 1] - row_offsets[b];
    e[0] = s0 + t0 - pad_left;
    e[1] = len + pad_left + pad_right - t0;
    e[2] = s0;
    e[3] = s0 + len - 1;
  }
}
hipError_t launch_tdnn_first(const FirstArgs& a, int epi_prec, hipStream_t s);
hipError_t launch_compact_first(const uint16_t* src, int ldw, int seg_pad, int n_pad, int noff, int dim, uint16_t* dst, hipStream_t s);

struct PrepArgs {
  const float* feats;
  const int32_t* src_off;
  const int32_t* dev_off;
  const int32_t* grp_utt;
  int rows;
  int dim;
  int ld;
  uint16_t* out_hi;
  uint16_t* out_lo;
  int pad_left, pad_right;
  unsigned* zero_words;
  int n_zero_words;
};
hipError_t launch_prep_input(const PrepArgs& a, int precision, hipStream_t s);

struct PoolArgs {
  const float* partial;
  int ldp;
  const int32_t* utt_grp0;
  const int32_t* utt_grp1;
  const int32_t* utt_count;
  int B;
  int dim;
  float var_floor;
  uint16_t* out_hi;
  uint16_t* out_lo;
  int ld;
};
hipError_t launch_pool_finalise(const PoolArgs& a, int precision, hipStream_t s);

struct FrameOutArgs {
  const float* src;
  const uint16_t* src16;
  int ld;
  const int32_t* out_row;
  int n_out;
  int dim;
  int log_softmax;
  float* out;
  int out_ld;
};
hipError_t launch_frame_output(const FrameOutArgs& a, hipStream_t s);

struct FrontEndArgs {
  const float* raw;
  const int32_t* raw_off;
  double* prefix;
  int n_utts;
  int dim;
  const int32_t* sel_row;
  const int32_t* sel_utt;
  int n_out;
  int cmn_window;
  int center;
  int min_window;
  float* out;
};
hipError_t launch_frontend(const FrontEndArgs& a, hipStream_t s);

struct CmExpandArgs {
  const uint8_t* cm;
  const int64_t* cm_off;
  const int32_t* raw_off;
  int n_utts, dim, max_rows;
  float* out;
};
hipError_t launch_cm_expand(const CmExpandArgs& a, hipStream_t s);

struct BackendArgs {
  const float* x;
  int n, dim, ldx;
  const float* mean;
  const float* t;
  int t_rows, t_cols;
  int normalize, scaleup;
  float* out;
  int ldo;
  float* ratio;
};
hipError_t launch_backend(const BackendArgs& a, hipStream_t s);

struct SegMeanArgs {
  const float* x;
  int dim, ldx;
  const int32_t* seg_off;
  const int32_t* idx;
  int n_seg;
  int acc64;
  float* out;
};
hipError_t launch_segment_mean(const SegMeanArgs& a, hipStream_t s);

uint16_t host_f32_to_bf16(float x);
float host_bf16_to_f32(uint16_t h);
uint16_t host_f32_to_f16(float x);
float host_f16_to_f32(uint16_t h);

}
```

### speaker-embedding-with-phonetic-information_amd/csrc/kernels.hip

```cpp
#include "kernels.h"
#include "knobs.h"

#include <hip/hip_ext.h>

#include <stdlib.h>
#include <string.h>

#include <algorithm>
#include <atomic>
#include <map>
#include <mutex>
#include <type_traits>
#include <utility>

namespace xv {

typedef __attribute__((ext_vector_type(8))) __bf16 bf16x8;
typedef __attribute__((ext_vector_type(8))) _Float16 f16x8;
typedef __attribute__((ext_vector_type(8))) short s16x8;
typedef __attribute__((ext_vector_type(4))) float f32x4;
typedef __attribute__((ext_vector_type(2))) float f32x2;
typedef __attribute__((ext_vector_type(4))) unsigned int u32x4;

#define XV_AS1 __attribute__((address_space(1)))
// ... 2704 lines not shown
    b.sk_mtiles = a.m_tiles * kBM / (64 * MF);
    {
      static const int max_lanes = [] {
        const int x = DebugKnobInt("sk_lanes", 4);
        return (x != 1 && x != 2 && x != 4) ? 4 : x;
      }();
      int l = max_lanes;
      while (l > 1 && (a.n_tiles % l || (grid / 8) % l)) l >>= 1;
      b.sk_lanes = l;
      grid = 8 * l * sk_groups<MF>(a, grid, l);
    }
    SkWorkspace w;
    hipError_t e = sk_workspace(s, grid, (size_t)grid * 64 * MF * kBN * sizeof(float), &w, &b.sk_epoch, &b.sk_error);
    if (e != hipSuccess) return e;
    b.sk_ws = w.ws;
    b.sk_flags = w.flags;
    note_kernel("_sk", PREC, EPI, MF);
    XV_LAUNCH((tdnn_gemm_kernel_sk<PREC, EPI, MF>), dim3(grid), dim3(512), lds, s, b);
    return hipGetLastError();
  }
}


bool gemm_p8_applicable(const GemmArgs& a, int precision) {
  if (precision == kPrecFp16MxE) precision = kPrecFp16Mx;
  if (precision != kPrecFp16 && precision != kPrecFp16Mx && precision != kPrecFp16Mx2) return false;
  if ((a.m_tiles & 1) || (a.n_tiles & 1) || a.ksplit > 1) return false;
  const bool mx = precision != kPrecFp16, mx2 = precision == kPrecFp16Mx2;
  GemmArgs b = a;
  build_groups(&b);
  int t = 0;
  for (int i = 0; i < b.ngrp; ++i) {
    if (b.grp[i].ksteps % (mx2 ? 8 : mx ? 4 : 2) || b.grp[i].ld % (mx2 ? 256 : 64)) return false;
    if (mx && !b.grp[i].gmax) return false;
    t += (b.grp[i].ksteps >> 1) * b.grp[i].nshift;
  }
  if (t < 2 || (t & 1)) return false;
  if (mx && (!a.w4 || !a.w4_scale || a.ldw4 <= 0)) return false;
  if (mx2) {
    if (!a.w4b || !a.w4b_scale || a.ldw4b <= 0) return false;
    for (int j = 0; j < a.nseg; ++j)
      if (!a.seg[j].lo4 || !a.seg[j].lo4s) return false;
  }
  return true;
}

template <int PREC, int EPI>
static hipError_t launch_one_p8(const GemmArgs& a, hipStream_t s) {
  if (!gemm_p8_applicable(a, PREC)) return hipErrorInvalidValue;
  static std::atomic<unsigned long long> attr_done{0};
  int attr_dev = 0;
  if (lds_attr_needed(&attr_done, &attr_dev)) {
    hipError_t e = hipFuncSetAttribute((const void*)tdnn_gemm_kernel_p8<PREC, EPI>, hipFuncAttributeMaxDynamicSharedMemorySize, kP8Lds);
    if (e != hipSuccess) return e;
    attr_done.fetch_or(1ull << (attr_dev & 63), std::memory_order_release);
  }
  GemmArgs b = a;
  build_groups(&b);
  b.p8_ktiles = 0;
  for (int i = 0; i < b.ngrp; ++i) b.p8_ktiles += (b.grp[i].ksteps >> 1) * b.grp[i].nshift;
  b.p8_ktiles_lo = 0;
  if constexpr (PrecMx2(PREC)) {
    build_lo_groups(&b);
    for (int i = 0; i < b.ngrp_lo; ++i) b.p8_ktiles_lo += (b.grp[b.ngrp + i].ksteps >> 1) * b.grp[b.ngrp + i].nshift;
  }
  b.p8 = 1;
  b.p8_whole = (a.p8_whole == 1 || (a.p8_whole == 2 && b.p8_ktiles + b.p8_ktiles_lo <= 8)) ? 1 : 0;
  b.sk_mtiles = a.m_tiles >> 1;
  const int nt = a.n_tiles >> 1;
  int grid = device_cu_count() / 8 * 8;
  if (grid < 8) return hipErrorInvalidValue;
  int l = 4;
  while (l > 1 && (nt % l || (grid / 8) % l)) l >>= 1;
  if (nt % 3 == 0 && nt <= 6 && grid / 8 >= nt) l = nt;
  b.sk_lanes = l;
  const int tiles_min = std::max(1, (b.sk_mtiles / 8) * (nt / l));
  grid = 8 * l * std::min(grid / 8 / l, tiles_min);
  SkWorkspace w;
  hipError_t e = sk_workspace(s, grid, (size_t)grid * 256 * 256 * sizeof(float), &w, &b.sk_epoch, &b.sk_error);
  if (e != hipSuccess) return e;
  b.sk_ws = w.ws;
  b.sk_flags = w.flags;
  note_kernel("_p8", PREC, EPI, 0);
  XV_LAUNCH((tdnn_gemm_kernel_p8<PREC, EPI>), dim3(grid), dim3(512), kP8Lds, s, b);
  return hipGetLastError();
}

template <int PREC, int EPI>
static hipError_t launch_one_v2(const GemmArgs& a, hipStream_t s) {
  constexpr int lds = 3 * (PrecXPlanes(PREC) * (256 + 16) * kBK * 2 + PrecWPlanes(PREC) * kTileBytes) + (PrecMx(PREC) ? 1536 : 0) + (PrecMx2(PREC) ? 3 * (256 + 16) * 4 : 0);
  static std::atomic<unsigned long long> attr_done{0};
  int attr_dev = 0;
  if (lds_attr_needed(&attr_done, &attr_dev)) {
    hipError_t e = hipFuncSetAttribute((const void*)tdnn_gemm_kernel_v2<PREC, EPI>,
                                       hipFuncAttributeMaxDynamicSharedMemorySize, lds);
    if (e != hipSuccess) return e;
    attr_done.fetch_or(1ull << (attr_dev & 63), std::memory_order_release);
  }
  const int mt = a.m_tiles >> 1;
  const int mt8 = (mt + 7) / 8 * 8;
  dim3 grid(mt8 * a.n_tiles), block(512);
  GemmArgs b = a;
  build_groups(&b);
  if constexpr (PrecMx2(PREC)) build_lo_groups(&b);
  {
    static const int pct = DebugKnobInt("gemm_stagger", 85);
    const int cus = device_cu_count();
    b.stagger_wgs = cus;
    b.stagger_units = ((int)grid.x > 2 * cus) ? (int)(((long)b.total_ksteps * (400 + 600 * PrecPasses(PREC)) + 14000) * pct / 100 / 2048) : 0;
  }
  note_kernel("_v2", PREC, EPI, 0);
  XV_LAUNCH((tdnn_gemm_kernel_v2<PREC, EPI>), grid, block, lds, s, b);
  return hipGetLastError();
}

template <int PREC, int EPI>
static hipError_t launch_one(const GemmArgs& a, hipStream_t s) {
  if (a.p8) {
    if constexpr (((PREC == kPrecFp16 || PREC == kPrecFp16Mx || PREC == kPrecFp16Mx2) && (EPI == kEpiAct || EPI == kEpiStats)) ||
                  (PREC == kPrecFp16MxE && EPI == kEpiAct))
      return launch_one_p8<PREC, EPI>(a, s);
    else return hipErrorInvalidValue;
  }
  const int variant = gemm_variant();
  const bool sk_default = PREC == kPrecFp16x2 || PREC == kPrecFp16Mx || a.total_ksteps >= 32;
  if constexpr (PrecMx(PREC)) {
    if (PrecMx2(PREC) ? !gemm_mx2_applicable(a) : !gemm_mx_applicable(a)) return hipErrorInvalidValue;
    if (variant != 2 && variant != 1 && sk_max_mf() == 8 && sk_applicable<PREC, 8>(a)) return launch_one_sk<PREC, EPI, 8>(a, s);
    return launch_one_v2<PREC, EPI>(a, s);
  } else {
    if (variant == 4 || (variant == 0 && sk_default)) {
      if (sk_max_mf() == 8 && sk_applicable<PREC, 8>(a)) return launch_one_sk<PREC, EPI, 8>(a, s);
      if ((variant == 4 || PrecXPlanes(PREC) == 2) && sk_applicable<PREC, 4>(a)) return launch_one_sk<PREC, EPI, 4>(a, s);
    }
    if (variant != 1 && (a.m_tiles & 1) == 0) return launch_one_v2<PREC, EPI>(a, s);
    constexpr int lds = kTileBytes * (PrecXPlanes(PREC) + PrecWPlanes(PREC)) * 2;
    static std::atomic<unsigned long long> attr_done{0};
    int attr_dev = 0;
    if (lds_attr_needed(&attr_done, &attr_dev)) {
      hipError_t e = hipFuncSetAttribute((const void*)tdnn_gemm_kernel<PREC, EPI>,
                                         hipFuncAttributeMaxDynamicSharedMemorySize, lds);
      if (e != hipSuccess) return e;
      attr_done.fetch_or(1ull << (attr_dev & 63), std::memory_order_release);
    }
    const int mt8 = (a.m_tiles + 7) / 8 * 8;
    dim3 grid(mt8 * a.n_tiles), block(256);
    note_kernel("", PREC, EPI, 0);
    XV_LAUNCH((tdnn_gemm_kernel<PREC, EPI>), grid, block, lds, s, a);
    return hipGetLastError();
  }
}

template <int PREC, int EPI>
__global__ __launch_bounds__(256) void splitk_reduce_kernel(const GemmArgs a) {
  constexpr bool SPLIT = PrecXPlanes(PREC) == 2;
  constexpr bool F16 = PrecF16(PREC);
  const int n_pad = a.n_tiles * kBN;
  const int rows = a.m_tiles * kBM;
  const long idx = (long)blockIdx.x * blockDim.x + threadIdx.x;
  const int per_row = n_pad >> 2;
  if (idx >= (long)rows * per_row) return;
  const int row = (int)(idx / per_row);
  const int col = (int)(idx - (long)row * per_row) * 4;
  f32x4 v = {0.f, 0.f, 0.f, 0.f};
  const long slab = (long)rows * n_pad;
  const float* src = a.splitk_ws + (long)row * n_pad + col;
  int k = 0;
  for (; k + 8 <= a.ksplit; k += 8) {
    f32x4 t[8];
#pragma unroll
    for (int j = 0; j < 8; ++j) t[j] = *(const f32x4*)(src + (k + j) * slab);
#pragma unroll
    for (int j = 0; j < 8; ++j) v += t[j];
  }
  {
    f32x4 t[8];
#pragma unroll
    for (int j = 0; j < 8; ++j) t[j] = (k + j < a.ksplit) ? *(const f32x4*)(src + (k + j) * slab) : f32x4{0.f, 0.f, 0.f, 0.f};
#pragma unroll
    for (int j = 0; j < 8; ++j)
      if (k + j < a.ksplit) v += t[j];
  }
  const f32x4 b = *(const f32x4*)(a.bias + col);
  float y[4];
#pragma unroll
  for (int r = 0; r < 4; ++r) {
    float z = v[r] + b[r];
    if (a.relu) z = (z < 0.f) ? 0.f : z;
    if (a.bn) z = __builtin_fmaf(z, a.scale[col + r], a.offset[col + r]);
    y[r] = z;
  }
  if constexpr (EPI == kEpiF32) {
    if (row < a.m_valid) *(f32x4*)(a.out_f32 + (long)row * a.ldf + col) = f32x4{y[0], y[1], y[2], y[3]};
  } else {
    const uint16_t h0 = to16<F16>(y[0]), h1 = to16<F16>(y[1]), h2 = to16<F16>(y[2]), h3 = to16<F16>(y[3]);
    unsigned int* dh = (unsigned int*)(a.out_hi + (long)row * a.ldo + col);
    dh[0] = (unsigned int)h0 | ((unsigned int)h1 << 16);
    dh[1] = (unsigned int)h2 | ((unsigned int)h3 << 16);
    if constexpr (SPLIT) {
      const uint16_t l0 = to16<F16>(y[0] - from16<F16>(h0)), l1 = to16<F16>(y[1] - from16<F16>(h1));
      const uint16_t l2 = to16<F16>(y[2] - from16<F16>(h2)), l3 = to16<F16>(y[3] - from16<F16>(h3));
      unsigned int* dl = (unsigned int*)(a.out_lo + (long)row * a.ldo + col);
      dl[0] = (unsigned int)l0 | ((unsigned int)l1 << 16);
      dl[1] = (unsigned int)l2 | ((unsigned int)l3 << 16);
    }
  }
}

template <int PREC, int EPI>
static hipError_t launch_splitk(const GemmArgs& a, hipStream_t s) {
  constexpr int lds = kTileBytes * (PrecXPlanes(PREC) + PrecWPlanes(PREC)) * kSplitKStages;
  static std::atomic<unsigned long long> attr_done{0};
  int attr_dev = 0;
  if (lds_attr_needed(&attr_done, &attr_dev)) {
    hipError_t e = hipFuncSetAttribute((const void*)tdnn_gemm_kernel<PREC, kEpiSplitK>,
                                       hipFuncAttributeMaxDynamicSharedMemorySize, lds);
    if (e != hipSuccess) return e;
    attr_done.fetch_or(1ull << (attr_dev & 63), std::memory_order_release);
  }
  dim3 grid(a.m_tiles * a.n_tiles, a.ksplit), block(256);
  note_kernel("", PREC, kEpiSplitK, 0);
  XV_LAUNCH((tdnn_gemm_kernel<PREC, kEpiSplitK>), grid, block, lds, s, a);
  hipError_t e = hipGetLastError();
  if (e != hipSuccess) return e;
  const long total = (long)a.m_tiles * kBM * (a.n_tiles * kBN / 4);
  XV_LAUNCH((splitk_reduce_kernel<PREC, EPI>), dim3((unsigned)((total + 255) / 256)), dim3(256), 0, s, a);
  return hipGetLastError();
}

template <int PREC>
static hipError_t launch_prec(const GemmArgs& a, int epi, hipStream_t s) {
  if constexpr (PREC == kPrecFp16x3E) {
    if (a.ksplit > 1 || epi != kEpiAct || !a.out_lo4 || !a.out_lo4s) return hipErrorInvalidValue;
    return launch_one<PREC, kEpiAct>(a, s);
  } else if constexpr (PREC == kPrecFp16MxE) {
    if (a.ksplit > 1 || epi != kEpiAct || !a.out_lo4 || !a.out_lo4s) return hipErrorInvalidValue;
    return launch_one<PREC, kEpiAct>(a, s);
  } else if constexpr (PrecMx(PREC)) {
    if (a.ksplit > 1) return hipErrorInvalidValue;
    if (epi == kEpiAct) return launch_one<PREC, kEpiAct>(a, s);
    if (epi == kEpiStats) return launch_one<PREC, kEpiStats>(a, s);
    return hipErrorInvalidValue;
  } else {
    if (a.ksplit > 1 && a.splitk_ws) {
      if (epi == kEpiAct) return launch_splitk<PREC, kEpiAct>(a, s);
      if (epi == kEpiF32) return launch_splitk<PREC, kEpiF32>(a, s);
      return hipErrorInvalidValue;
    }
    switch (epi) {
      case kEpiAct: return launch_one<PREC, kEpiAct>(a, s);
      case kEpiF32: return launch_one<PREC, kEpiF32>(a, s);
      case kEpiStats: return launch_one<PREC, kEpiStats>(a, s);
      default: return hipErrorInvalidValue;
    }
  }
}

hipError_t launch_tdnn_gemm(const GemmArgs& a, int precision, int epilogue, hipStream_t s) {
  if (a.nseg < 1 || a.nseg > kMaxSeg || a.m_tiles < 1 || a.n_tiles < 1) return hipErrorInvalidValue;
  switch (precision) {
    case kPrecBf16x3: return launch_prec<kPrecBf16x3>(a, epilogue, s);
    case kPrecBf16: return launch_prec<kPrecBf16>(a, epilogue, s);
    case kPrecFp16: return launch_prec<kPrecFp16>(a, epilogue, s);
    case kPrecFp16x3: return launch_prec<kPrecFp16x3>(a, epilogue, s);
    case kPrecFp16x2: return launch_prec<kPrecFp16x2>(a, epilogue, s);
    case kPrecFp16Mx: return launch_prec<kPrecFp16Mx>(a, epilogue, s);
    case kPrecFp16Mx2: return launch_prec<kPrecFp16Mx2>(a, epilogue, s);
    case kPrecFp16x3E: return launch_prec<kPrecFp16x3E>(a, epilogue, s);
    case kPrecFp16MxE: return launch_prec<kPrecFp16MxE>(a, epilogue, s);
    default: return hipErrorInvalidValue;
  }
}

template <int EPREC>
__global__ __launch_bounds__(512) void tdnn_first_kernel(const FirstArgs fa) {
  const GemmArgs& a = fa.g;
  constexpr bool F16 = PrecF16(EPREC);
  constexpr int XR = kFirstRows + 32;
  extern __shared__ __attribute__((aligned(16))) char smem[];
  float* par_all = (float*)smem;
  const int tid = threadIdx.x;
  const int lane = tid & 63;
  const int wave = __builtin_amdgcn_readfirstlane(tid >> 6);
  const int fr_i = lane & 15, fr_g = lane >> 4;
  const int dp = (fa.dim + 7) & ~7;
  int min_off = fa.off[0], max_off = fa.off[0];
  for (int j = 1; j < fa.noff; ++j) {
    min_off = min(min_off, fa.off[j]);
    max_off = max(max_off, fa.off[j]);
  }
  const int span = max_off - min_off;
  const int plane_bytes = XR * dp * 2;
  char* wlo_s = smem + 4 * 384 * 4;
  char* xbuf = wlo_s + 512 * 256;
  auto wkey = [](int r) __attribute__((always_inline)) { return ((r >> 1) & 12) | (r & 3); };

  const int n_pad = a.n_tiles * kBN;
  const int nrb = fa.nrows / kFirstRows, ncg = (n_pad + 511) / 512;
  const int cg = blockIdx.x % ncg, wg = blockIdx.x / ncg, nwg = gridDim.x / ncg;
  const int rb0 = (int)((long)nrb * wg / nwg), rb1 = (int)((long)nrb * (wg + 1) / nwg);
  if (rb0 >= rb1 || wg >= nwg) return;
  const int n0w = cg * 512 + wave * 64;
  const bool cols_valid = n0w < n_pad;
  XV_FUZZ_INIT();

  int xo[4];
#pragma unroll
  for (int s = 0; s < 4; ++s) {
    const int k = 32 * s + 8 * fr_g;
    int j = k / dp, d0 = k - j * dp;
    if (j >= fa.noff) {
      j = fa.noff - 1;
      d0 = dp - 8;
    }
    xo[s] = ((fa.off[j] - min_off + fr_i) * dp + d0) * 2;
  }

  constexpr int kTabUnits = 96;
  constexpr int kTabGroups = kTabUnits * 4 + 8;
  int4* gtab = (int4*)(xbuf + 4 * plane_bytes);
  int tab_rb0 = -(1 << 30), tab_g0 = 0;
  auto build_table = [&](int rb_first) __attribute__((always_inline)) {
    tab_rb0 = rb_first;
    tab_g0 = ((fa.row0 + rb_first * kFirstRows) >> 4) - 4;
    for (int i = tid; i < kTabGroups; i += 512) {
      const int g = tab_g0 + i;
      gtab[i] = (g >= 0 && g * 16 < fa.rows) ? fa.grp_src[g] : int4{0, 0, 0, 0};
    }
  };
  const int n_slots = (kFirstRows + span) * dp;
  int slot_fd[kFirstMaxSlots];
#pragma unroll
  for (int i = 0; i < kFirstMaxSlots; ++i) {
    const int slot = tid + 512 * i;
    const int fr = slot / dp;
    slot_fd[i] = slot < n_slots ? (fr << 8) | (slot - fr * dp) : -1;
  }
  float pv[kFirstMaxSlots] = {0.f, 0.f, 0.f, 0.f};
  unsigned pv_ok = 0u;
  auto prefetch = [&](int rb) __attribute__((always_inline)) {
    const int r_first = fa.row0 + rb * kFirstRows + min_off;
    pv_ok = 0u;
#pragma unroll
    for (int i = 0; i < kFirstMaxSlots; ++i) {
      long idx = fa.feats_valid_idx;
      if (slot_fd[i] >= 0) {
        const int d = slot_fd[i] & 255;
        const int r = r_first + (slot_fd[i] >> 8);
        const int4 e = gtab[(r >> 4) - tab_g0];
        const int t = r & 15;
        if (d < fa.dim && t < e.y) {
          idx = (long)min(max(e.x + t, e.z), e.w) * fa.dim + d;
          pv_ok |= 1u << i;
        }
      }
      pv[i] = fa.feats[idx];
    }
    __builtin_amdgcn_sched_barrier(0);
  };
// ... 388 lines not shown
}

hipError_t launch_cm_expand(const CmExpandArgs& a, hipStream_t s) {
  if (a.dim < 1 || a.dim > 64 || a.n_utts < 1 || a.max_rows < 1) return hipErrorInvalidValue;
  XV_LAUNCH(cm_expand_kernel, dim3((unsigned)((a.max_rows + 63) / 64), (unsigned)a.n_utts), dim3(256), 0, s, a);
  return hipGetLastError();
}

hipError_t launch_frontend(const FrontEndArgs& a, hipStream_t s) {
  if (a.dim > 64) return hipErrorInvalidValue;
  if (a.cmn_window > 0 && a.n_utts > 0) XV_LAUNCH(cmn_prefix_kernel, dim3(a.n_utts), dim3(1024), 0, s, a);
  if (a.n_out > 0) {
    const long total = (long)a.n_out * a.dim;
    XV_LAUNCH(cmn_select_kernel, dim3((unsigned)((total + 255) / 256)), dim3(256), 0, s, a);
  }
  return hipGetLastError();
}

template <int N, bool VEC, bool IN16 = false>
__global__ __launch_bounds__(256) void frame_output_lsm_kernel(const FrameOutArgs a) {
  const int o = blockIdx.x;
  const long srow = a.out_row ? a.out_row[o] : o;
  const float* src = IN16 ? nullptr : a.src + srow * a.ld;
  const _Float16* src16 = IN16 ? (const _Float16*)a.src16 + srow * a.ld : nullptr;
  float* dst = a.out + (long)o * a.out_ld;
  const int tid = threadIdx.x;
  __shared__ float red[8];
  float v[N];
  float m = -INFINITY;
  if constexpr (VEC) {
#pragma unroll
    for (int i = 0; i < N / 4; ++i) {
      const int c = (tid + 256 * i) * 4;
      f32x4 x = {-INFINITY, -INFINITY, -INFINITY, -INFINITY};
      if (c < a.dim) {
        if constexpr (IN16) {
          typedef _Float16 f16x4 __attribute__((ext_vector_type(4)));
          x = __builtin_convertvector(*(const f16x4*)(src16 + c), f32x4);
        } else {
          x = *(const f32x4*)(src + c);
        }
      }
#pragma unroll
      for (int k = 0; k < 4; ++k) {
        v[4 * i + k] = x[k];
        m = fmaxf(m, x[k]);
      }
    }
  } else {
#pragma unroll
    for (int i = 0; i < N; ++i) {
      const int c = tid + 256 * i;
      v[i] = c < a.dim ? (IN16 ? (float)src16[c] : src[c]) : -INFINITY;
      m = fmaxf(m, v[i]);
    }
  }
#pragma unroll
  for (int d = 32; d >= 1; d >>= 1) m = fmaxf(m, __shfl_xor(m, d));
  if ((tid & 63) == 0) red[tid >> 6] = m;
  __syncthreads();
  m = fmaxf(fmaxf(red[0], red[1]), fmaxf(red[2], red[3]));
  float sum = 0.f;
#pragma unroll
  for (int i = 0; i < N; ++i) sum += expf(v[i] - m);
#pragma unroll
  for (int d = 32; d >= 1; d >>= 1) sum += __shfl_xor(sum, d);
  if ((tid & 63) == 0) red[4 + (tid >> 6)] = sum;
  __syncthreads();
  const float lse = m + logf((red[4] + red[5]) + (red[6] + red[7]));
  if constexpr (VEC) {
#pragma unroll
    for (int i = 0; i < N / 4; ++i) {
      const int c = (tid + 256 * i) * 4;
      if (c < a.dim) *(f32x4*)(dst + c) = f32x4{v[4 * i] - lse, v[4 * i + 1] - lse, v[4 * i + 2] - lse, v[4 * i + 3] - lse};
    }
  } else {
#pragma unroll
    for (int i = 0; i < N; ++i) {
      const int c = tid + 256 * i;
      if (c < a.dim) dst[c] = v[i] - lse;
    }
  }
}

__global__ __launch_bounds__(256) void frame_output_kernel(const FrameOutArgs a) {
  const int o = blockIdx.x;
  const long srow = a.out_row ? a.out_row[o] : o;
  const float* src = a.src + srow * a.ld;
  float* dst = a.out + (long)o * a.out_ld;
  const int tid = threadIdx.x;
  if (!a.log_softmax) {
    for (int c = tid; c < a.dim; c += 256) dst[c] = src[c];
    return;
  }
  __shared__ float red[4];
  float m = -INFINITY;
  for (int c = tid; c < a.dim; c += 256) m = fmaxf(m, src[c]);
#pragma unroll
  for (int d = 32; d >= 1; d >>= 1) m = fmaxf(m, __shfl_xor(m, d));
  if ((tid & 63) == 0) red[tid >> 6] = m;
  __syncthreads();
  m = fmaxf(fmaxf(red[0], red[1]), fmaxf(red[2], red[3]));
  __syncthreads();
  float sum = 0.f;
  for (int c = tid; c < a.dim; c += 256) sum += expf(src[c] - m);
#pragma unroll
  for (int d = 32; d >= 1; d >>= 1) sum += __shfl_xor(sum, d);
  if ((tid & 63) == 0) red[tid >> 6] = sum;
  __syncthreads();
  const float lse = m + logf((red[0] + red[1]) + (red[2] + red[3]));
  for (int c = tid; c < a.dim; c += 256) dst[c] = src[c] - lse;
}

hipError_t launch_frame_output(const FrameOutArgs& a, hipStream_t s) {
  if (a.n_out <= 0) return hipSuccess;
  const dim3 grid(a.n_out), block(256);
  if (a.src16) {
    if (!a.log_softmax || a.dim > 256 * 64) return hipErrorInvalidValue;
    const bool vec = ((a.dim | a.out_ld | a.ld) & 3) == 0 && ((uintptr_t)a.out & 15) == 0 && ((uintptr_t)a.src16 & 7) == 0;
    const int n = (a.dim + 255) / 256;
    if (vec) {
      if (n <= 8) XV_LAUNCH((frame_output_lsm_kernel<8, true, true>), grid, block, 0, s, a);
      else if (n <= 16) XV_LAUNCH((frame_output_lsm_kernel<16, true, true>), grid, block, 0, s, a);
      else if (n <= 32) XV_LAUNCH((frame_output_lsm_kernel<32, true, true>), grid, block, 0, s, a);
      else XV_LAUNCH((frame_output_lsm_kernel<64, true, true>), grid, block, 0, s, a);
    } else {
      if (n <= 8) XV_LAUNCH((frame_output_lsm_kernel<8, false, true>), grid, block, 0, s, a);
      else if (n <= 16) XV_LAUNCH((frame_output_lsm_kernel<16, false, true>), grid, block, 0, s, a);
      else if (n <= 32) XV_LAUNCH((frame_output_lsm_kernel<32, false, true>), grid, block, 0, s, a);
      else XV_LAUNCH((frame_output_lsm_kernel<64, false, true>), grid, block, 0, s, a);
    }
    return hipGetLastError();
  }
  if (a.log_softmax && a.dim <= 256 * 64) {
    const bool vec = ((a.dim | a.out_ld | a.ld) & 3) == 0 && (((uintptr_t)a.out | (uintptr_t)a.src) & 15) == 0;
    const int n = (a.dim + 255) / 256;
    if (vec) {
      if (n <= 8) XV_LAUNCH((frame_output_lsm_kernel<8, true>), grid, block, 0, s, a);
      else if (n <= 16) XV_LAUNCH((frame_output_lsm_kernel<16, true>), grid, block, 0, s, a);
      else if (n <= 32) XV_LAUNCH((frame_output_lsm_kernel<32, true>), grid, block, 0, s, a);
      else XV_LAUNCH((frame_output_lsm_kernel<64, true>), grid, block, 0, s, a);
    } else {
      if (n <= 8) XV_LAUNCH((frame_output_lsm_kernel<8, false>), grid, block, 0, s, a);
      else if (n <= 16) XV_LAUNCH((frame_output_lsm_kernel<16, false>), grid, block, 0, s, a);
      else if (n <= 32) XV_LAUNCH((frame_output_lsm_kernel<32, false>), grid, block, 0, s, a);
      else XV_LAUNCH((frame_output_lsm_kernel<64, false>), grid, block, 0, s, a);
    }
    return hipGetLastError();
  }
  XV_LAUNCH(frame_output_kernel, grid, block, 0, s, a);
  return hipGetLastError();
}

template <int PREC>
__global__ __launch_bounds__(256) void pool_finalise_kernel(const PoolArgs a) {
  constexpr bool SPLIT = PrecXPlanes(PREC) == 2;
  constexpr bool F16 = PrecF16(PREC);
  const int b = blockIdx.y;
  const int col = blockIdx.x * blockDim.x + threadIdx.x;
  if (col >= a.dim) return;
  const int g0 = a.utt_grp0[b], g1 = a.utt_grp1[b];
  double s1 = 0.0, s2 = 0.0;
  for (int g = g0; g < g1; ++g) {
    const float* p = a.partial + (long)g * 2 * a.ldp + col;
    s1 += (double)p[0];
    s2 += (double)p[a.ldp];
  }
  const float n = (float)a.utt_count[b];
  const float mu = __fdiv_rn((float)s1, n);
  const float ex2 = __fdiv_rn((float)s2, n);
  float m2 = mu * mu;
  asm volatile("" : "+v"(m2));
  float var = ex2 - m2;
  var = fmaxf(var, a.var_floor);
  const float sd = sqrtf(var);
  const long base = (long)b * a.ld;
  const uint16_t mh = to16<F16>(mu), sh = to16<F16>(sd);
  a.out_hi[base + col] = mh;
  a.out_hi[base + a.dim + col] = sh;
  if constexpr (SPLIT) {
    a.out_lo[base + col] = to16<F16>(mu - from16<F16>(mh));
    a.out_lo[base + a.dim + col] = to16<F16>(sd - from16<F16>(sh));
  }
}

hipError_t launch_pool_finalise(const PoolArgs& a, int precision, hipStream_t s) {
  dim3 grid((a.dim + 255) / 256, a.B), block(256);
  switch (precision) {
    case kPrecBf16x3: XV_LAUNCH(pool_finalise_kernel<kPrecBf16x3>, grid, block, 0, s, a); break;
    case kPrecBf16: XV_LAUNCH(pool_finalise_kernel<kPrecBf16>, grid, block, 0, s, a); break;
    case kPrecFp16: XV_LAUNCH(pool_finalise_kernel<kPrecFp16>, grid, block, 0, s, a); break;
    case kPrecFp16x3: XV_LAUNCH(pool_finalise_kernel<kPrecFp16x3>, grid, block, 0, s, a); break;
    default: return hipErrorInvalidValue;
  }
  return hipGetLastError();
}

typedef __attribute__((ext_vector_type(4))) float f32x4_t;
constexpr int kBkVB = 64, kBkKT = 32, kBkLD = 36, kBkMaxRF = 16;

template <int RF>
__global__ __launch_bounds__(256) void backend_gemm_kernel(const BackendArgs a) {
  __shared__ float ts[RF * 16 * kBkLD];
  __shared__ float xs[kBkVB * kBkLD];
  const int tid = threadIdx.x, lane = tid & 63, wave = tid >> 6;
  const int v0 = blockIdx.x * kBkVB;
  const int fi = lane & 15, fk = lane >> 4;
  f32x4_t acc[RF];
#pragma unroll
  for (int r = 0; r < RF; ++r) acc[r] = f32x4_t{0.f, 0.f, 0.f, 0.f};
  constexpr int NT = RF * 16 / 8, NX = kBkVB / 8;
  float tr[NT], xr[NX];
  const int kk = tid & 31, r8 = tid >> 5;
  auto fetch = [&](int k0) {
#pragma unroll
    for (int i = 0; i < NT; ++i) {
      const int r = r8 + 8 * i;
      tr[i] = (r < a.t_rows && k0 + kk < a.dim) ? a.t[(long)r * a.t_cols + k0 + kk] : 0.f;
    }
#pragma unroll
    for (int i = 0; i < NX; ++i) {
      const int v = r8 + 8 * i;
      float x = 0.f;
      if (v0 + v < a.n && k0 + kk < a.dim) {
        x = a.x[(long)(v0 + v) * a.ldx + k0 + kk];
        if (a.mean) x -= a.mean[k0 + kk];
      }
      xr[i] = x;
    }
  };
  fetch(0);
  for (int k0 = 0; k0 < a.dim; k0 += kBkKT) {
    __syncthreads();
#pragma unroll
    for (int i = 0; i < NT; ++i) ts[(r8 + 8 * i) * kBkLD + kk] = tr[i];
#pragma unroll
    for (int i = 0; i < NX; ++i) xs[(r8 + 8 * i) * kBkLD + kk] = xr[i];
    __syncthreads();
    if (k0 + kBkKT < a.dim) fetch(k0 + kBkKT);
#pragma unroll
    for (int k4 = 0; k4 < kBkKT / 4; ++k4) {
      const float b = xs[(wave * 16 + fi) * kBkLD + k4 * 4 + fk];
#pragma unroll
      for (int r = 0; r < RF; ++r) {
        const float w = ts[(r * 16 + fi) * kBkLD + k4 * 4 + fk];
        acc[r] = __builtin_amdgcn_mfma_f32_16x16x4f32(w, b, acc[r], 0, 0, 0);
      }
    }
  }
  const int v = v0 + wave * 16 + fi;
  const int out_dim = a.t_rows;
  float ss = 0.f;
#pragma unroll
  for (int r = 0; r < RF; ++r) {
    {
#pragma unroll
      for (int q = 0; q < 4; ++q) {
        const int row = r * 16 + fk * 4 + q;
        float y = acc[r][q];
        if (row < out_dim) {
          if (a.t_cols == a.dim + 1) y += a.t[(long)row * a.t_cols + a.dim];
        } else {
          y = 0.f;
        }
        acc[r][q] = y;
        ss = fmaf(y, y, ss);
      }
    }
  }
  ss += __shfl_xor(ss, 16);
  ss += __shfl_xor(ss, 32);
  float scale = 1.f;
  if (a.normalize || a.ratio) {
    const float norm = sqrtf(ss);
    const float ratio = a.scaleup ? norm / sqrtf((float)out_dim) : norm;
    if (a.ratio && fk == 0 && v < a.n) a.ratio[v] = ratio;
    if (a.normalize && ratio != 0.f) scale = 1.f / ratio;
  }
  if (v < a.n) {
    float* dst = a.out + (long)v * a.ldo;
#pragma unroll
    for (int r = 0; r < RF; ++r) {
      {
        const int row = r * 16 + fk * 4;
        if (row + 3 < out_dim && (a.ldo & 3) == 0 && (out_dim & 3) == 0) {
          *(f32x4_t*)(dst + row) = acc[r] * scale;
        } else {
#pragma unroll
          for (int q = 0; q < 4; ++q)
            if (row + q < out_dim) dst[row + q] = acc[r][q] * scale;
        }
      }
    }
  }
}

__global__ __launch_bounds__(256) void backend_rowwise_kernel(const BackendArgs a) {
  const int lane = threadIdx.x & 63;
  const int v = blockIdx.x * 4 + (threadIdx.x >> 6);
  if (v >= a.n) return;
  const float* src = a.x + (long)v * a.ldx;
  float ss = 0.f;
  for (int k = lane; k < a.dim; k += 64) {
    float x = src[k];
    if (a.mean) x -= a.mean[k];
    ss = fmaf(x, x, ss);
  }
#pragma unroll
  for (int d = 32; d >= 1; d >>= 1) ss += __shfl_xor(ss, d);
  float scale = 1.f;
  if (a.normalize || a.ratio) {
    const float norm = sqrtf(ss);
    const float ratio = a.scaleup ? norm / sqrtf((float)a.dim) : norm;
    if (a.ratio && lane == 0) a.ratio[v] = ratio;
    if (a.normalize && ratio != 0.f) scale = 1.f / ratio;
  }
  float* dst = a.out + (long)v * a.ldo;
  for (int k = lane; k < a.dim; k += 64) {
    float x = src[k];
    if (a.mean) x -= a.mean[k];
    dst[k] = x * scale;
  }
}

static hipError_t launch_backend_gemm(const BackendArgs& a, hipStream_t s) {
  const dim3 grid((a.n + kBkVB - 1) / kBkVB), block(256);
  const int rf = (a.t_rows + 15) / 16;
  if (rf <= 2) XV_LAUNCH(backend_gemm_kernel<2>, grid, block, 0, s, a);
  else if (rf <= 4) XV_LAUNCH(backend_gemm_kernel<4>, grid, block, 0, s, a);
  else if (rf <= 7) XV_LAUNCH(backend_gemm_kernel<7>, grid, block, 0, s, a);
  else if (rf <= 10) XV_LAUNCH(backend_gemm_kernel<10>, grid, block, 0, s, a);
  else if (rf <= 13) XV_LAUNCH(backend_gemm_kernel<13>, grid, block, 0, s, a);
  else XV_LAUNCH(backend_gemm_kernel<16>, grid, block, 0, s, a);
  return hipGetLastError();
}

hipError_t launch_backend(const BackendArgs& a, hipStream_t s) {
  if (a.n <= 0) return hipSuccess;
  if (a.dim < 1 || (a.t && a.t_cols != a.dim && a.t_cols != a.dim + 1)) return hipErrorInvalidValue;
  if (!a.t) {
    XV_LAUNCH(backend_rowwise_kernel, dim3((a.n + 3) / 4), dim3(256), 0, s, a);
    return hipGetLastError();
  }
  if (a.t_rows <= kBkMaxRF * 16) return launch_backend_gemm(a, s);
  for (int r0 = 0; r0 < a.t_rows; r0 += kBkMaxRF * 16) {
    BackendArgs b = a;
// ... 71 lines not shown
```

Measured before the change: 358,600 utt/s.

## Fuse stats pooling finalise into the first segment-level split-K GEMM

Adds a tdnn_gemm_kernel_pool kernel that computes the pooled mean/std per utterance group directly into LDS. It feeds them into a three-pass split-K MFMA GEMM for the layer after pooling, and the last-arriving block, chosen by an atomic ticket, does the split-K reduction and the epilogue. This removes the separate pool_finalise and splitk_reduce launches and the round trip of the stats buffer. It also moves the group-max zeroing into this kernel, so the standalone memset is skipped when it is not needed. The path is only enabled for the fp16x3/bf16x3 slow precision with a small K per slice. It relies on the ticket counters being reset correctly between runs.

```diff
diff --git a/include/xvec_hip.h b/include/xvec_hip.h
--- a/include/xvec_hip.h
+++ b/include/xvec_hip.h
@@ -294,6 +294,24 @@
 } xv_pool_finalise_desc;
 xv_status xv_kernel_pool_finalise(const xv_pool_finalise_desc* d);
 typedef struct {
+  int32_t precision;
+  int32_t epilogue;
+  const float* partial; int32_t ldp;
+  const int32_t* utt_grp0; const int32_t* utt_grp1; const int32_t* utt_count;
+  int32_t B, dim;
+  float var_floor;
+  void* stats_hi; void* stats_lo; int32_t ld;
+  const void* w_hi; const void* w_lo; int32_t ldw;
+  int32_t n_pad;
+  const float* bias; const float* scale; const float* offset;
+  int32_t relu, bn;
+  void* out_hi; void* out_lo; int32_t ldo;
+  float* out_f32; int32_t ldf;
+  void* zero_words; int32_t n_zero_words;
+  void* hip_stream;
+} xv_pool_affine_desc;
+xv_status xv_kernel_pool_affine(const xv_pool_affine_desc* d);
+typedef struct {
   const float* src; const void* src16; int32_t ld;
   const int32_t* out_row; int32_t n_out;
   int32_t dim, log_softmax;
diff --git a/speaker-embedding-with-phonetic-information_amd/__init__.py b/speaker-embedding-with-phonetic-information_amd/__init__.py
--- a/speaker-embedding-with-phonetic-information_amd/__init__.py
+++ b/speaker-embedding-with-phonetic-information_amd/__init__.py
@@ -84,6 +84,19 @@
                 ("out_hi", ctypes.c_void_p), ("out_lo", ctypes.c_void_p), ("ld", ctypes.c_int32), ("hip_stream", ctypes.c_void_p)]
 
 
+class PoolAffineDesc(ctypes.Structure):
+    _fields_ = [("precision", ctypes.c_int32), ("epilogue", ctypes.c_int32), ("partial", ctypes.c_void_p), ("ldp", ctypes.c_int32),
+                ("utt_grp0", ctypes.c_void_p), ("utt_grp1", ctypes.c_void_p), ("utt_count", ctypes.c_void_p),
+                ("B", ctypes.c_int32), ("dim", ctypes.c_int32), ("var_floor", ctypes.c_float),
+                ("stats_hi", ctypes.c_void_p), ("stats_lo", ctypes.c_void_p), ("ld", ctypes.c_int32),
+                ("w_hi", ctypes.c_void_p), ("w_lo", ctypes.c_void_p), ("ldw", ctypes.c_int32), ("n_pad", ctypes.c_int32),
+                ("bias", ctypes.c_void_p), ("scale", ctypes.c_void_p), ("offset", ctypes.c_void_p),
+                ("relu", ctypes.c_int32), ("bn", ctypes.c_int32),
+                ("out_hi", ctypes.c_void_p), ("out_lo", ctypes.c_void_p), ("ldo", ctypes.c_int32),
+                ("out_f32", ctypes.c_void_p), ("ldf", ctypes.c_int32),
+                ("zero_words", ctypes.c_void_p), ("n_zero_words", ctypes.c_int32), ("hip_stream", ctypes.c_void_p)]
+
+
 class FrameOutputDesc(ctypes.Structure):
     _fields_ = [("src", ctypes.c_void_p), ("src16", ctypes.c_void_p), ("ld", ctypes.c_int32),
                 ("out_row", ctypes.c_void_p), ("n_out", ctypes.c_int32), ("dim", ctypes.c_int32), ("log_softmax", ctypes.c_int32),
@@ -125,6 +138,7 @@
     "xv_compressed_size", "xv_compress_matrices", "xv_compress_kernel_time", "xv_cmvn_sliding",
     "xv_cmvn_stats", "xv_cmvn_norm", "xv_cmvn_apply", "xv_cmvn_kernel_time",
     "xv_kernel_first_layer", "xv_kernel_prep_input", "xv_kernel_pool_finalise", "xv_kernel_frame_output",
+    "xv_kernel_pool_affine",
     "xv_wave_read", "xv_wave_free", "xv_pack_mx_residual", "xv_pack_mx_residual64", "xv_tile_mx_scales", "xv_pack_mx_weights", "xv_pack_mx_weights64",
 ]
 
@@ -200,6 +214,7 @@
     L.xv_kernel_prep_input.argtypes = [ctypes.POINTER(PrepInputDesc)]
     L.xv_kernel_pool_finalise.argtypes = [ctypes.POINTER(PoolFinaliseDesc)]
     L.xv_kernel_frame_output.argtypes = [ctypes.POINTER(FrameOutputDesc)]
+    L.xv_kernel_pool_affine.argtypes = [ctypes.POINTER(PoolAffineDesc)]
     L.xv_ctx_calibrate.argtypes = [ctypes.c_void_p, ctypes.c_void_p, ctypes.c_void_p, ctypes.c_int32, ctypes.c_float,
                                    ctypes.POINTER(Calibration)]
     L.xv_ctx_set_fast_mode.argtypes = [ctypes.c_void_p, ctypes.c_int32]
@@ -1044,6 +1059,10 @@
     _check(lib().xv_kernel_pool_finalise(ctypes.byref(desc)))
 
 
+def kernel_pool_affine(desc):
+    _check(lib().xv_kernel_pool_affine(ctypes.byref(desc)))
+
+
 def kernel_frame_output(desc):
     _check(lib().xv_kernel_frame_output(ctypes.byref(desc)))
 
diff --git a/speaker-embedding-with-phonetic-information_amd/csrc/capi.cc b/speaker-embedding-with-phonetic-information_amd/csrc/capi.cc
--- a/speaker-embedding-with-phonetic-information_amd/csrc/capi.cc
+++ b/speaker-embedding-with-phonetic-information_amd/csrc/capi.cc
@@ -1242,6 +1242,74 @@
   });
 }
 
+xv_status xv_kernel_pool_affine(const xv_pool_affine_desc* d) {
+  if (!d) return Fail(XV_ERR_ARG, "xv_kernel_pool_affine: null descriptor");
+  return Guard([&] {
+    if (d->B < 1 || d->dim < 1 || d->n_pad < xv::kBN || d->n_pad % xv::kBN || d->n_zero_words < 0)
+      return Fail(XV_ERR_ARG, "xv_kernel_pool_affine: bad geometry (n_pad: multiple of 128)");
+    xv::PoolAffineArgs a;
+    memset(&a, 0, sizeof a);
+    a.pool.partial = d->partial;
+    a.pool.ldp = d->ldp;
+    a.pool.utt_grp0 = d->utt_grp0;
+    a.pool.utt_grp1 = d->utt_grp1;
+    a.pool.utt_count = d->utt_count;
+    a.pool.B = d->B;
+    a.pool.dim = d->dim;
+    a.pool.var_floor = d->var_floor;
+    a.pool.out_hi = (uint16_t*)d->stats_hi;
+    a.pool.out_lo = (uint16_t*)d->stats_lo;
+    a.pool.ld = d->ld;
+    xv::GemmArgs& g = a.g;
+    g.nseg = 1;
+    g.total_ksteps = (2 * d->dim + xv::kBK - 1) / xv::kBK;
+    g.seg[0].ksteps = g.total_ksteps;
+    g.w_hi = (const uint16_t*)d->w_hi;
+    g.w_lo = (const uint16_t*)d->w_lo;
+    g.ldw = d->ldw;
+    g.n_tiles = d->n_pad / xv::kBN;
+    g.relu = d->relu;
+    g.bn = d->bn;
+    g.bias = d->bias;
+    g.scale = d->scale;
+    g.offset = d->offset;
+    g.out_hi = (uint16_t*)d->out_hi;
+    g.out_lo = (uint16_t*)d->out_lo;
+    g.ldo = d->ldo;
+    g.out_f32 = d->out_f32;
+    g.ldf = d->ldf;
+    g.m_valid = d->B;
+    g.ksteps_per_slice = xv::SplitKStepsPerSlice(g.total_ksteps);
+    g.ksplit = (g.total_ksteps + g.ksteps_per_slice - 1) / g.ksteps_per_slice;
+    const int groups = (d->B + xv::kPoolAffineRows - 1) / xv::kPoolAffineRows;
+    a.ws_rows = groups * xv::kPoolAffineRows;
+    a.zero_words = (unsigned*)d->zero_words;
+    a.n_zero_words = d->n_zero_words;
+    if ((d->bn && (!d->scale || !d->offset)) || (d->epilogue == xv::kEpiF32 ? d->ldf < d->n_pad : d->ldo < d->n_pad))
+      return Fail(XV_ERR_ARG, "xv_kernel_pool_affine: BatchNorm needs scale and offset, output rows hold n_pad columns");
+    DevMem ws, tickets;
+    hipError_t e = ws.Alloc((size_t)g.ksplit * a.ws_rows * d->n_pad * 4);
+    if (e == hipSuccess) e = tickets.Alloc((size_t)groups * 4);
+    if (e == hipSuccess) e = hipMemset(tickets.p, 0, (size_t)groups * 4);
+    if (e != hipSuccess) return Fail(XV_ERR_DEVICE, std::string("hipMalloc(pool_affine workspace): ") + hipGetErrorString(e));
+    g.splitk_ws = (float*)ws.p;
+    a.tickets = (unsigned*)tickets.p;
+    if (!xv::pool_affine_applicable(a, d->precision, d->epilogue))
+      return Fail(XV_ERR_ARG, "xv_kernel_pool_affine: XV_PREC_BF16X3 or XV_PREC_FP16X3, epilogue 0 or 1, ldp >= dim, ld >= 2 dim, ldw >= K, "
+                              "a K of at least two slices of at most 8 steps, and every pointer of the epilogue");
+    e = xv::launch_pool_affine(a, d->precision, d->epilogue, (hipStream_t)d->hip_stream);
+    const hipError_t e2 = hipStreamSynchronize((hipStream_t)d->hip_stream);
+    if (e != hipSuccess || e2 != hipSuccess)
+      return Fail(XV_ERR_DEVICE, std::string("pool_affine launch: ") + hipGetErrorString(e != hipSuccess ? e : e2));
+    std::vector<unsigned> left(groups, 1u);
+    e = hipMemcpy(left.data(), tickets.p, (size_t)groups * 4, hipMemcpyDeviceToHost);
+    if (e != hipSuccess) return Fail(XV_ERR_DEVICE, std::string("hipMemcpy(tickets): ") + hipGetErrorString(e));
+    for (unsigned t : left)
+      if (t) return Fail(XV_ERR_DEVICE, "pool_affine: an arrival counter was not reset");
+    return XV_OK;
+  });
+}
+
 xv_status xv_kernel_frame_output(const xv_frame_output_desc* d) {
   if (!d) return Fail(XV_ERR_ARG, "xv_kernel_frame_output: null descriptor");
   return Guard([&] {
diff --git a/speaker-embedding-with-phonetic-information_amd/csrc/engine.cc b/speaker-embedding-with-phonetic-information_amd/csrc/engine.cc
--- a/speaker-embedding-with-phonetic-information_amd/csrc/engine.cc
+++ b/speaker-embedding-with-phonetic-information_amd/csrc/engine.cc
@@ -662,6 +662,15 @@
   }
   in_ld_ = RoundUp(info_.input_dim, kBK);
   stats_ld_ = RoundUp(2 * info_.pool_dim, kBK);
+  fused_tail_ = false;
+  if (!frame_mode_ && info_.pooled_layer >= 0 && (size_t)info_.pooled_layer + 1 < info_.layers.size() &&
+      DebugKnobInt("fused_tail", 1) != 0 && (slow_prec() == kPrecFp16x3 || slow_prec() == kPrecBf16x3)) {
+    const BlobLayerInfo& c = info_.layers[info_.pooled_layer + 1];
+    const int ksteps = stats_ld_ / kBK;
+    fused_tail_ = c.segment_level && c.src.size() == 1 && c.src[0].layer == kSrcPooled && c.src[0].offset == 0 &&
+                  c.src[0].dim == 2 * info_.pool_dim && SplitKStepsPerSlice(ksteps) <= kPoolAffineMaxSteps &&
+                  ksteps > SplitKStepsPerSlice(ksteps);
+  }
   {
     const bool allow = DebugKnobInt("first_kernel", 1) != 0 && nplanes_ == 2;
     need_prep_ = false;
@@ -724,6 +733,7 @@
     fr(L.stats_lo);
     fr(L.out_f32);
     fr(L.splitk_ws);
+    fr(L.tail_tickets);
     fr(L.frame_f32);
     if (L.done) (void)hipEventDestroy(L.done);
     if (L.stream) (void)hipStreamDestroy(L.stream);
@@ -803,6 +813,7 @@
   if (!frame_mode_ && b_pad > L.cap_b) {
     if (L.busy) Check(hipEventSynchronize(L.done), "hipEventSynchronize(lane)");
     Ensure(&L.stats_hi, (size_t)b_pad * stats_ld_ * 2, true, s);
+    if (fused_tail_) Ensure(&L.tail_tickets, (size_t)(b_pad / kPoolAffineRows) * 4, true, s);
     if (nplanes_ == 2) Ensure(&L.stats_lo, (size_t)b_pad * stats_ld_ * 2, true, s);
     for (size_t i = 0; i < layers_.size(); ++i) {
       const BlobLayerInfo& li = info_.layers[i];
@@ -1211,6 +1222,18 @@
   return po;
 }
 
+PoolAffineArgs Engine::TailArgs(const Lane& L, const Plan& plan, const GemmArgs& affine, const PrepArgs& pa) const {
+  PoolAffineArgs t;
+  memset(&t, 0, sizeof t);
+  t.pool = PoolingArgs(L, plan);
+  t.g = affine;
+  t.ws_rows = plan.b_pad;
+  t.tickets = (unsigned*)L.tail_tickets.p;
+  t.zero_words = pa.zero_words;
+  t.n_zero_words = pa.n_zero_words;
+  return t;
+}
+
 FrameOutArgs Engine::OutputArgs(const Lane& L, const Plan& plan, float* out_dev, int out_ld) const {
   const BlobLayerInfo& ol = info_.layers[info_.output_layer];
   FrameOutArgs fo;
@@ -1259,15 +1282,17 @@
     arm("prep_input");
     Check(launch_prep_input(pa, slow_prec(), s), "prep_input launch");
     disarm();
-  } else if (pa.n_zero_words > 0) {
+  } else if (pa.n_zero_words > 0 && L.gmax_dirty) {
     Check(hipMemsetAsync(pa.zero_words, 0, (size_t)pa.n_zero_words * 4, s), "hipMemsetAsync(group maxima)");
   }
+  if (pa.n_zero_words > 0) L.gmax_dirty = true;
 
   const BlobLayerInfo& ol = info_.layers[info_.output_layer];
   const bool direct_out = ol.segment_level && !ol.log_softmax && ol.n_pad == info_.output_dim && (out_ld & 3) == 0 &&
                           out_ld >= ol.n_pad && ((uintptr_t)out_dev & 15) == 0;
   for (size_t i = 0; i < layers_.size(); ++i) {
     const BlobLayerInfo& li = info_.layers[i];
+    if (fused_tail_ && (int)i == info_.pooled_layer + 1) continue;
     GemmArgs ga;
     const int epi = LayerArgs(L, plan, i, mx_pass, out_dev, out_ld, direct_out, &ga);
     arm(std::string("tdnn_gemm<") + (epi == kEpiAct ? "act" : epi == kEpiF32 ? "f32" : "stats") + ">:" + li.name);
@@ -1293,7 +1318,16 @@
     }
     disarm();
 
-    if ((int)i == info_.pooled_layer) {
+    if ((int)i == info_.pooled_layer && fused_tail_) {
+      GemmArgs gb;
+      const int epi_b = LayerArgs(L, plan, i + 1, mx_pass, out_dev, out_ld, direct_out, &gb);
+      const int p = LaunchPrec(i + 1, epi_b, false, &gb);
+      arm(std::string("tdnn_gemm<") + (epi_b == kEpiAct ? "act" : "f32") + ">:" + info_.layers[i + 1].name);
+      Check(launch_pool_affine(TailArgs(L, plan, gb, pa), p, epi_b, s), "pool_affine launch");
+      if (first_prof) prof_labels_.back() += std::string(" ") + last_gemm_kernel();
+      disarm();
+      L.gmax_dirty = false;
+    } else if ((int)i == info_.pooled_layer) {
       arm("pool_finalise");
       Check(launch_pool_finalise(PoolingArgs(L, plan), slow_prec(), s), "pool_finalise launch");
       disarm();
diff --git a/speaker-embedding-with-phonetic-information_amd/csrc/engine.h b/speaker-embedding-with-phonetic-information_amd/csrc/engine.h
--- a/speaker-embedding-with-phonetic-information_amd/csrc/engine.h
+++ b/speaker-embedding-with-phonetic-information_amd/csrc/engine.h
@@ -151,6 +151,8 @@
     Buf in_hi, in_lo, partial, stats_hi, stats_lo, out_f32, splitk_ws, frame_f32;
     Buf gmax;
     int gmax_stride = 0;
+    bool gmax_dirty = false;
+    Buf tail_tickets;
     int cap_rows = 0, cap_b = 0;
   };
   struct HostSlot {
@@ -181,6 +183,7 @@
   int LaunchPrec(size_t i, int epi, bool fast, GemmArgs* g) const;
   PrepArgs PrepInputArgs(const Lane& L, const Plan& plan, const float* feats_dev, bool mx_pass) const;
   PoolArgs PoolingArgs(const Lane& L, const Plan& plan) const;
+  PoolAffineArgs TailArgs(const Lane& L, const Plan& plan, const GemmArgs& affine, const PrepArgs& pa) const;
   FrameOutArgs OutputArgs(const Lane& L, const Plan& plan, float* out_dev, int out_ld) const;
   void Check(hipError_t e, const char* what) const;
  public:
@@ -205,6 +208,7 @@
   bool fast_mx2() const { return has_fast() && fast_mode_ == kPrecFp16Mx2; }
   int p8_whole_ = 0;
   bool use_p8_ = true;
+  bool fused_tail_ = false;
   bool logits16() const { return frame_mode_ && info_.precision == kPrecFp16 && info_.layers[info_.output_layer].log_softmax; }
   int fast_min_pooled_ = 0;
   int fast_mode_ = 0;
diff --git a/speaker-embedding-with-phonetic-information_amd/csrc/kernels.h b/speaker-embedding-with-phonetic-information_amd/csrc/kernels.h
--- a/speaker-embedding-with-phonetic-information_amd/csrc/kernels.h
+++ b/speaker-embedding-with-phonetic-information_amd/csrc/kernels.h
@@ -293,6 +293,19 @@
 };
 hipError_t launch_pool_finalise(const PoolArgs& a, int precision, hipStream_t s);
 
+constexpr int kPoolAffineRows = 16;
+constexpr int kPoolAffineMaxSteps = 8;
+struct PoolAffineArgs {
+  PoolArgs pool;
+  GemmArgs g;
+  int ws_rows;
+  unsigned* tickets;
+  unsigned* zero_words;
+  int n_zero_words;
+};
+bool pool_affine_applicable(const PoolAffineArgs& a, int precision, int epilogue);
+hipError_t launch_pool_affine(const PoolAffineArgs& a, int precision, int epilogue, hipStream_t s);
+
 struct FrameOutArgs {
   const float* src;
   const uint16_t* src16;
diff --git a/speaker-embedding-with-phonetic-information_amd/csrc/kernels.hip b/speaker-embedding-with-phonetic-information_amd/csrc/kernels.hip
--- a/speaker-embedding-with-phonetic-information_amd/csrc/kernels.hip
+++ b/speaker-embedding-with-phonetic-information_amd/csrc/kernels.hip
@@ -2880,9 +2880,37 @@
 }
 
 template <int PREC, int EPI>
-__global__ __launch_bounds__(256) void splitk_reduce_kernel(const GemmArgs a) {
+__device__ __forceinline__ void splitk_finish(const GemmArgs& a, const f32x4 v, const int row, const int col) {
   constexpr bool SPLIT = PrecXPlanes(PREC) == 2;
   constexpr bool F16 = PrecF16(PREC);
+  const f32x4 b = *(const f32x4*)(a.bias + col);
+  float y[4];
+#pragma unroll
+  for (int r = 0; r < 4; ++r) {
+    float z = v[r] + b[r];
+    if (a.relu) z = (z < 0.f) ? 0.f : z;
+    if (a.bn) z = __builtin_fmaf(z, a.scale[col + r], a.offset[col + r]);
+    y[r] = z;
+  }
+  if constexpr (EPI == kEpiF32) {
+    if (row < a.m_valid) *(f32x4*)(a.out_f32 + (long)row * a.ldf + col) = f32x4{y[0], y[1], y[2], y[3]};
+  } else {
+    const uint16_t h0 = to16<F16>(y[0]), h1 = to16<F16>(y[1]), h2 = to16<F16>(y[2]), h3 = to16<F16>(y[3]);
+    unsigned int* dh = (unsigned int*)(a.out_hi + (long)row * a.ldo + col);
+    dh[0] = (unsigned int)h0 | ((unsigned int)h1 << 16);
+    dh[1] = (unsigned int)h2 | ((unsigned int)h3 << 16);
+    if constexpr (SPLIT) {
+      const uint16_t l0 = to16<F16>(y[0] - from16<F16>(h0)), l1 = to16<F16>(y[1] - from16<F16>(h1));
+      const uint16_t l2 = to16<F16>(y[2] - from16<F16>(h2)), l3 = to16<F16>(y[3] - from16<F16>(h3));
+      unsigned int* dl = (unsigned int*)(a.out_lo + (long)row * a.ldo + col);
+      dl[0] = (unsigned int)l0 | ((unsigned int)l1 << 16);
+      dl[1] = (unsigned int)l2 | ((unsigned int)l3 << 16);
+    }
+  }
+}
+
+template <int PREC, int EPI>
+__global__ __launch_bounds__(256) void splitk_reduce_kernel(const GemmArgs a) {
   const int n_pad = a.n_tiles * kBN;
   const int rows = a.m_tiles * kBM;
   const long idx = (long)blockIdx.x * blockDim.x + threadIdx.x;
@@ -2909,30 +2937,7 @@
     for (int j = 0; j < 8; ++j)
       if (k + j < a.ksplit) v += t[j];
   }
-  const f32x4 b = *(const f32x4*)(a.bias + col);
-  float y[4];
-#pragma unroll
-  for (int r = 0; r < 4; ++r) {
-    float z = v[r] + b[r];
-    if (a.relu) z = (z < 0.f) ? 0.f : z;
-    if (a.bn) z = __builtin_fmaf(z, a.scale[col + r], a.offset[col + r]);
-    y[r] = z;
-  }
-  if constexpr (EPI == kEpiF32) {
-    if (row < a.m_valid) *(f32x4*)(a.out_f32 + (long)row * a.ldf + col) = f32x4{y[0], y[1], y[2], y[3]};
-  } else {
-    const uint16_t h0 = to16<F16>(y[0]), h1 = to16<F16>(y[1]), h2 = to16<F16>(y[2]), h3 = to16<F16>(y[3]);
-    unsigned int* dh = (unsigned int*)(a.out_hi + (long)row * a.ldo + col);
-    dh[0] = (unsigned int)h0 | ((unsigned int)h1 << 16);
-    dh[1] = (unsigned int)h2 | ((unsigned int)h3 << 16);
-    if constexpr (SPLIT) {
-      const uint16_t l0 = to16<F16>(y[0] - from16<F16>(h0)), l1 = to16<F16>(y[1] - from16<F16>(h1));
-      const uint16_t l2 = to16<F16>(y[2] - from16<F16>(h2)), l3 = to16<F16>(y[3] - from16<F16>(h3));
-      unsigned int* dl = (unsigned int*)(a.out_lo + (long)row * a.ldo + col);
-      dl[0] = (unsigned int)l0 | ((unsigned int)l1 << 16);
-      dl[1] = (unsigned int)l2 | ((unsigned int)l3 << 16);
-    }
-  }
+  splitk_finish<PREC, EPI>(a, v, row, col);
 }
 
 template <int PREC, int EPI>
@@ -3627,6 +3632,17 @@
   return hipGetLastError();
 }
 
+__device__ __forceinline__ void pool_moments(const double s1, const double s2, const float n, const float var_floor, float& mu,
+                                             float& sd) {
+  mu = __fdiv_rn((float)s1, n);
+  const float ex2 = __fdiv_rn((float)s2, n);
+  float m2 = mu * mu;
+  asm volatile("" : "+v"(m2));
+  float var = ex2 - m2;
+  var = fmaxf(var, var_floor);
+  sd = sqrtf(var);
+}
+
 template <int PREC>
 __global__ __launch_bounds__(256) void pool_finalise_kernel(const PoolArgs a) {
   constexpr bool SPLIT = PrecXPlanes(PREC) == 2;
@@ -3641,14 +3657,8 @@
     s1 += (double)p[0];
     s2 += (double)p[a.ldp];
   }
-  const float n = (float)a.utt_count[b];
-  const float mu = __fdiv_rn((float)s1, n);
-  const float ex2 = __fdiv_rn((float)s2, n);
-  float m2 = mu * mu;
-  asm volatile("" : "+v"(m2));
-  float var = ex2 - m2;
-  var = fmaxf(var, a.var_floor);
-  const float sd = sqrtf(var);
+  float mu, sd;
+  pool_moments(s1, s2, (float)a.utt_count[b], a.var_floor, mu, sd);
   const long base = (long)b * a.ld;
   const uint16_t mh = to16<F16>(mu), sh = to16<F16>(sd);
   a.out_hi[base + col] = mh;
@@ -3667,6 +3677,213 @@
     case kPrecFp16: XV_LAUNCH(pool_finalise_kernel<kPrecFp16>, grid, block, 0, s, a); break;
     case kPrecFp16x3: XV_LAUNCH(pool_finalise_kernel<kPrecFp16x3>, grid, block, 0, s, a); break;
     default: return hipErrorInvalidValue;
+  }
+  return hipGetLastError();
+}
+
+constexpr int kPaPitch = kPoolAffineMaxSteps * kBK + 8;
+
+template <int PREC, int EPI>
+__global__ __launch_bounds__(256, 2) void tdnn_gemm_kernel_pool(const PoolAffineArgs a) {
+  constexpr bool F16 = PrecF16(PREC);
+  static_assert(PrecXPlanes(PREC) == 2 && PrecWPlanes(PREC) == 2, "three-pass arithmetic only");
+  __shared__ __attribute__((aligned(16))) uint16_t smem[2 * kPoolAffineRows * kPaPitch + 8];
+  uint16_t* xs_hi = smem;
+  uint16_t* xs_lo = smem + kPoolAffineRows * kPaPitch;
+  unsigned* last_flag = (unsigned*)(smem + 2 * kPoolAffineRows * kPaPitch);
+
+  const int tid = threadIdx.x;
+  const int lane = tid & 63;
+  const int wave = __builtin_amdgcn_readfirstlane(tid >> 6);
+  const int ks = blockIdx.x % a.g.ksplit;
+  const int mg = blockIdx.x / a.g.ksplit;
+  const int s_begin = ks * a.g.ksteps_per_slice;
+  const int S = min(a.g.total_ksteps, s_begin + a.g.ksteps_per_slice) - s_begin;
+  const int kw = a.g.ksteps_per_slice * kBK;
+  const int k0 = s_begin * kBK;
+  const int dim = a.pool.dim;
+  const int n_pad = a.g.n_tiles * kBN;
+
+  const int nitems = kPoolAffineRows * kw;
+  for (int i0 = 0; i0 < nitems; i0 += 256 * 8) {
+    const float* p[8];
+    int len[8], bb[8], kk[8];
+    bool want_sd[8];
+    int maxlen = 0;
+#pragma unroll
+    for (int c = 0; c < 8; ++c) {
+      const int idx = i0 + c * 256 + tid;
+      const int r = idx / kw, kl = idx - r * kw;
+      const int b = mg * kPoolAffineRows + r, k = k0 + kl;
+      const bool ok = idx < nitems && b < a.pool.B && k < 2 * dim;
+      bb[c] = ok ? b : -1;
+      kk[c] = k;
+      want_sd[c] = k >= dim;
+      len[c] = 0;
+      p[c] = a.pool.partial;
+      if (ok) {
+        const int g0 = a.pool.utt_grp0[b], g1 = a.pool.utt_grp1[b];
+        len[c] = g1 - g0;
+        p[c] = a.pool.partial + (long)g0 * 2 * a.pool.ldp + (want_sd[c] ? k - dim : k);
+      }
+      maxlen = max(maxlen, len[c]);
+    }
+    const long gstep = 2L * a.pool.ldp;
+    double s1[8], s2[8];
+#pragma unroll
+    for (int c = 0; c < 8; ++c) s1[c] = s2[c] = 0.0;
+    for (int g = 0; g < maxlen; g += 2) {
+      float v1[8][2], v2[8][2];
+#pragma unroll
+      for (int c = 0; c < 8; ++c)
+#pragma unroll
+        for (int u = 0; u < 2; ++u) {
+          const bool on = g + u < len[c];
+          v1[c][u] = on ? p[c][(g + u) * gstep] : 0.f;
+          v2[c][u] = (on && want_sd[c]) ? p[c][(g + u) * gstep + a.pool.ldp] : 0.f;
+        }
+#pragma unroll
+      for (int c = 0; c < 8; ++c)
+#pragma unroll
+        for (int u = 0; u < 2; ++u)
+          if (g + u < len[c]) {
+            s1[c] += (double)v1[c][u];
+            s2[c] += (double)v2[c][u];
+          }
+    }
+#pragma unroll
+    for (int c = 0; c < 8; ++c) {
+      const int idx = i0 + c * 256 + tid;
+      if (idx >= nitems) continue;
+      const int r = idx / kw, kl = idx - r * kw;
+      uint16_t h = 0, l = 0;
+      if (bb[c] >= 0) {
+        float mu, sd;
+        pool_moments(s1[c], s2[c], (float)a.pool.utt_count[bb[c]], a.pool.var_floor, mu, sd);
+        const float x = want_sd[c] ? sd : mu;
+        h = to16<F16>(x);
+        l = to16<F16>(x - from16<F16>(h));
+        const long o = (long)bb[c] * a.pool.ld + kk[c];
+        a.pool.out_hi[o] = h;
+        a.pool.out_lo[o] = l;
+      }
+      xs_hi[r * kPaPitch + kl] = h;
+      xs_lo[r * kPaPitch + kl] = l;
+    }
+  }
+  __syncthreads();
+
+  const int fr_i = lane & 15;
+  const int fr_g = lane >> 4;
+  float* ws = a.g.splitk_ws + (long)ks * a.ws_rows * n_pad + (long)(mg * kPoolAffineRows + fr_i) * n_pad;
+  for (int nb = 0; nb < n_pad; nb += 512) {
+    const int n0 = nb + wave * 128;
+    if (n0 >= n_pad) continue;
+    f32x4 acc[8];
+#pragma unroll
+    for (int f = 0; f < 8; ++f) acc[f] = f32x4{0.f, 0.f, 0.f, 0.f};
+    const uint16_t* wph = a.g.w_hi + (long)(n0 + fr_i) * a.g.ldw + k0 + fr_g * 8;
+    const uint16_t* wpl = a.g.w_lo + (long)(n0 + fr_i) * a.g.ldw + k0 + fr_g * 8;
+    const long wstep = 16L * a.g.ldw;
+#pragma unroll 1
+    for (int s = 0; s < S; ++s) {
+      const s16x8 xh = *(const s16x8*)(xs_hi + fr_i * kPaPitch + s * kBK + fr_g * 8);
+      const s16x8 xl = *(const s16x8*)(xs_lo + fr_i * kPaPitch + s * kBK + fr_g * 8);
+      s16x8 wh[8], wl[8];
+#pragma unroll
+      for (int f = 0; f < 8; ++f) {
+        wh[f] = *(const s16x8*)(wph + f * wstep + s * kBK);
+        wl[f] = *(const s16x8*)(wpl + f * wstep + s * kBK);
+      }
+#pragma unroll
+      for (int f = 0; f < 8; ++f) {
+        acc[f] = mfma16<F16>(wl[f], xh, acc[f]);
+        acc[f] = mfma16<F16>(wh[f], xl, acc[f]);
+        acc[f] = mfma16<F16>(wh[f], xh, acc[f]);
+      }
+    }
+#pragma unroll
+    for (int f = 0; f < 8; ++f) *(f32x4*)(ws + n0 + f * 16 + fr_g * 4) = acc[f];
+  }
+  for (int i = blockIdx.x * 256 + tid; i < a.n_zero_words; i += gridDim.x * 256) a.zero_words[i] = 0u;
+
+  asm volatile("s_waitcnt vmcnt(0)" ::: "memory");
+  __syncthreads();
+  if (tid == 0) {
+    __builtin_amdgcn_fence(__ATOMIC_RELEASE, "agent");
+    asm volatile("s_waitcnt vmcnt(0)" ::: "memory");
+    const unsigned ticket = __hip_atomic_fetch_add(a.tickets + mg, 1u, __ATOMIC_RELAXED, __HIP_MEMORY_SCOPE_AGENT);
+    const bool last = ticket == (unsigned)a.g.ksplit - 1u;
+    if (last) {
+      __hip_atomic_store(a.tickets + mg, 0u, __ATOMIC_RELAXED, __HIP_MEMORY_SCOPE_AGENT);
+      __builtin_amdgcn_fence(__ATOMIC_ACQUIRE, "agent");
+      asm volatile("s_waitcnt vmcnt(0)" ::: "memory");
+    }
+    *last_flag = last ? 1u : 0u;
+  }
+  __syncthreads();
+  if (*last_flag == 0u) return;
+
+  const long slab = (long)a.ws_rows * n_pad;
+  const int per_row = n_pad >> 2;
+  const int total = kPoolAffineRows * per_row;
+  for (int e0 = 0; e0 < total; e0 += 256 * 4) {
+    const float* src[4];
+    int row[4], col[4];
+    f32x4 v[4];
+#pragma unroll
+    for (int e = 0; e < 4; ++e) {
+      const int idx = min(e0 + e * 256 + tid, total - 1);
+      row[e] = mg * kPoolAffineRows + idx / per_row;
+      col[e] = (idx % per_row) * 4;
+      src[e] = a.g.splitk_ws + (long)row[e] * n_pad + col[e];
+      v[e] = f32x4{0.f, 0.f, 0.f, 0.f};
+    }
+    for (int k = 0; k < a.g.ksplit; k += 8) {
+      f32x4 t[4][8];
+#pragma unroll
+      for (int e = 0; e < 4; ++e)
+#pragma unroll
+        for (int j = 0; j < 8; ++j)
+          t[e][j] = (k + j < a.g.ksplit) ? *(const f32x4*)(src[e] + (k + j) * slab) : f32x4{0.f, 0.f, 0.f, 0.f};
+#pragma unroll
+      for (int e = 0; e < 4; ++e)
+#pragma unroll
+        for (int j = 0; j < 8; ++j)
+          if (k + j < a.g.ksplit) v[e] += t[e][j];
+    }
+#pragma unroll
+    for (int e = 0; e < 4; ++e)
+      if (e0 + e * 256 + tid < total) splitk_finish<PREC, EPI>(a.g, v[e], row[e], col[e]);
+  }
+}
+
+bool pool_affine_applicable(const PoolAffineArgs& a, int precision, int epilogue) {
+  const GemmArgs& g = a.g;
+  if (precision != kPrecFp16x3 && precision != kPrecBf16x3) return false;
+  if (epilogue != kEpiAct && epilogue != kEpiF32) return false;
+  if (g.ksplit < 2 || !g.splitk_ws || g.ksteps_per_slice < 1 || g.ksteps_per_slice > kPoolAffineMaxSteps) return false;
+  if (g.ksteps_per_slice != SplitKStepsPerSlice(g.total_ksteps) ||
+      g.ksplit != (g.total_ksteps + g.ksteps_per_slice - 1) / g.ksteps_per_slice)
+    return false;
+  if (a.pool.B < 1 || a.pool.dim < 1 || a.pool.ldp < a.pool.dim || a.pool.ld < 2 * a.pool.dim) return false;
+  if (g.total_ksteps != (2 * a.pool.dim + kBK - 1) / kBK || g.ldw < g.total_ksteps * kBK || g.n_tiles < 1) return false;
+  if (a.ws_rows < (a.pool.B + kPoolAffineRows - 1) / kPoolAffineRows * kPoolAffineRows || !a.tickets) return false;
+  if (!a.pool.partial || !a.pool.out_hi || !a.pool.out_lo || !g.w_hi || !g.w_lo || !g.bias) return false;
+  if (epilogue == kEpiF32 ? !g.out_f32 : (!g.out_hi || !g.out_lo)) return false;
+  return a.n_zero_words == 0 || a.zero_words;
+}
+
+hipError_t launch_pool_affine(const PoolAffineArgs& a, int precision, int epilogue, hipStream_t s) {
+  if (!pool_affine_applicable(a, precision, epilogue)) return hipErrorInvalidValue;
+  const dim3 grid((unsigned)((a.pool.B + kPoolAffineRows - 1) / kPoolAffineRows * a.g.ksplit)), block(256);
+  snprintf(g_last_kernel, sizeof g_last_kernel, "tdnn_gemm_kernel_pool<%s,%s>", prec_name(precision), epi_name(epilogue));
+  if (precision == kPrecFp16x3) {
+    if (epilogue == kEpiAct) XV_LAUNCH((tdnn_gemm_kernel_pool<kPrecFp16x3, kEpiAct>), grid, block, 0, s, a);
+    else XV_LAUNCH((tdnn_gemm_kernel_pool<kPrecFp16x3, kEpiF32>), grid, block, 0, s, a);
+  } else {
+    if (epilogue == kEpiAct) XV_LAUNCH((tdnn_gemm_kernel_pool<kPrecBf16x3, kEpiAct>), grid, block, 0, s, a);
+    else XV_LAUNCH((tdnn_gemm_kernel_pool<kPrecBf16x3, kEpiF32>), grid, block, 0, s, a);
   }
   return hipGetLastError();
 }
```

Result: slower. 339,500 utt/s (-5.3%).
